# mmp/pbrt-v3

Hardware: NVIDIA H100
Metric: Msamples/sec (higher is better)
Workload: dtype f32

## Files before the change

### include/pb2.h

```cpp
#ifndef PB2_H
#define PB2_H

#include <stddef.h>
#include <stdint.h>

#ifdef __cplusplus
extern "C" {
#endif

#define PB2_ABI_VERSION 10

typedef enum pb2_status {
    PB2_OK = 0,
    PB2_ERR_NO_DEVICE = 1,
    PB2_ERR_CUDA = 2,
    PB2_ERR_INVALID = 3,
    PB2_ERR_UNSUPPORTED = 4,
    PB2_ERR_NCCL = 5
} pb2_status;


typedef struct pb2_bvh_node {
    float bmin[3];
    float bmax[3];
// ... 95 lines not shown
} pb2_bvh;

typedef struct pb2_instance {
    float instance_to_world[16];
    float world_to_instance[16];
    int32_t bvh;
    int32_t lone_prim;
    int32_t pad[2];
} pb2_instance;

typedef struct pb2_scene_desc {
    int64_t n_vertices;
    const float *P;
    const float *N;
    const float *UV;
    const float *S;
    int64_t n_tris;
    const int32_t *tri_index;
    const int32_t *tri_mesh;
    int32_t n_meshes;
    const pb2_mesh *meshes;
    int32_t n_spheres;
    const pb2_sphere *spheres;

    int64_t n_prims;
    const uint8_t *prim_type;
    const int32_t *prim_index;
    const int32_t *prim_material;
    const int32_t *prim_light;

    int64_t n_nodes;
    const pb2_bvh_node *nodes;
    const int32_t *bvh_prims;

    int32_t n_materials;
    const pb2_material *materials;
    int32_t n_lights;
    const pb2_light *lights;

    int32_t light_strategy;
    int32_t spatial_max_voxels;

    int32_t n_instances;
    int32_t n_bvhs;
    const pb2_instance *instances;
    const pb2_bvh *bvhs;
    int64_t n_bvh_prims;
    const pb2_delta_light *delta_lights;
    int32_t n_textures;
    int32_t pad_textures;
    const pb2_texture *textures;
} pb2_scene_desc;

typedef struct pb2_camera {
    float camera_to_world[16];
    float world_to_camera[16];
    float screen_window[4];
    float fov;
    float lens_radius, focal_distance;
    float shutter_open, shutter_close;
    float raster_to_camera[16];
    float dx_camera[3], dy_camera[3];
} pb2_camera;

typedef struct pb2_film_desc {
    int32_t full_resolution[2];
    int32_t cropped_pixel_bounds[4];
    float filter_radius[2];
    float max_sample_luminance;
    float scale;
    int32_t filter_type;
    float filter_param[2];
    int32_t pad;
} pb2_film_desc;

typedef struct pb2_path_params {
    int32_t samples_per_pixel;
    int32_t sample_at_pixel_center;
    int32_t max_depth;
    float rr_threshold;
    int32_t pixel_bounds[4];
    int32_t tile_rank, tile_count;
    int32_t flags;
    int32_t sampler;
} pb2_path_params;

enum { PB2_SAMPLER_HALTON = 0, PB2_SAMPLER_SOBOL = 1 };

#define PB2_FLAG_COUNT_TRAVERSAL 1
#define PB2_FLAG_LINEAR_NODES 2
#define PB2_FLAG_WIDE4 4
#define PB2_FLAG_PLAIN_TRACE 8
#define PB2_FLAG_SMALL_STACK 16
#define PB2_FLAG_LD128 32
#define PB2_FLAG_LEAF_TMA 64
#define PB2_FLAG_POOL 128
#define PB2_FLAG_CHAIN 256

typedef struct pb2_ray {
    float o[3];
    float d[3];
    float t_max;
} pb2_ray;

typedef struct pb2_hit {
    int32_t prim;
    float t;
    float b[3];
    float p[3];
    float p_error[3];
    float n[3];
    float ns[3];
    float dpdu[3];
    float uv[2];
} pb2_hit;

typedef struct pb2_stats {
    uint64_t camera_rays;
    uint64_t regular_rays;
    uint64_t shadow_rays;
    uint64_t node_visits;
    uint64_t prim_tests;
    uint64_t kernel_launches;
    double render_ms;
    double h2d_ms, d2h_ms;
    double trace_ms;
} pb2_stats;

typedef struct pb2_scene pb2_scene;


int pb2_abi_version(void);
const char *pb2_last_error(void);

int pb2_init(int device_id);
int pb2_init_devices(int n_devices, const int *device_ids);
int pb2_device_count(void);
int pb2_shutdown(void);

#define PB2_DIST_ID_BYTES 128
int pb2_dist_unique_id(void *id);
int pb2_dist_init(int rank, int world, const void *id);
int pb2_dist_info(int *rank, int *world);
int pb2_dist_shutdown(void);

int pb2_work_items(const pb2_film_desc *film, const pb2_path_params *params, int64_t first, int64_t n, int32_t *out,
                   int64_t *n_items);

int pb2_host_alloc(size_t bytes, void **out);
int pb2_host_free(void *p);

int pb2_scene_create(const pb2_scene_desc *desc, pb2_scene **out);
int pb2_scene_destroy(pb2_scene *scene);

int pb2_intersect(pb2_scene *scene, const pb2_ray *rays, int64_t n, pb2_hit *hits);
int pb2_intersect_p(pb2_scene *scene, const pb2_ray *rays, int64_t n, uint8_t *occluded);

int pb2_render_path(pb2_scene *scene, const pb2_camera *camera, const pb2_film_desc *film,
                    const pb2_path_params *params, float *film_rgbw, pb2_stats *stats);

int pb2_render_path_device(pb2_scene *scene, const pb2_camera *camera, const pb2_film_desc *film,
                           const pb2_path_params *params, float *film_rgbw_device, int clear,
                           void *stream, pb2_stats *stats);

typedef struct pb2_wf_hit {
    int32_t found;
    int32_t leaf;
    int32_t prim;
    float t;
    float b[3];
    int32_t listed;
} pb2_wf_hit;
int pb2_trace_wavefront(pb2_scene *scene, const pb2_ray *rays, const uint8_t *any_hit, int64_t n, int32_t flags,
                        pb2_wf_hit *out);

int pb2_li_samples(pb2_scene *scene, const pb2_camera *camera, const pb2_film_desc *film,
                   const pb2_path_params *params, const int32_t *pixel_xy, const int64_t *sample_num,
                   int64_t n, float *out_rgb, float *out_pfilm);

int pb2_halton_samples(const pb2_film_desc *film, const pb2_path_params *params,
                       const int32_t *pixel_xy, const int64_t *sample_num, const int32_t *dim,
                       int64_t n, float *out);

int pb2_sobol_samples_host(const pb2_film_desc *film, const pb2_path_params *params, const int32_t *pixel_xy,
                           const int64_t *sample_num, const int32_t *dim, int64_t n, float *out, uint64_t *tables);

int pb2_light_distribution(pb2_scene *scene, const float *points_xyz, int64_t n, float *out);

int pb2_texture_pyramid(const pb2_texture *texture, int32_t level, int32_t *n_levels, int32_t *w, int32_t *h, float *out);

int pb2_texture_eval_host(const pb2_texture *textures, int32_t n_textures, int32_t id, int64_t n, const float *uv, const float *duv,
                          float *out);

int pb2_bsdf_eval_host(const pb2_material *material, int64_t n, const float *in, float *out);

int pb2_camera_differentials_host(const pb2_camera *camera, const pb2_film_desc *film, const pb2_path_params *params, int64_t n,
                                  const float *in, float *out);
int pb2_uv_differentials_host(int64_t n, const float *in, float *out);

int pb2_env_distribution(const pb2_texture *texture, int32_t *nu, int32_t *nv, float *out);

int pb2_texture_lookup(const pb2_texture *texture, int64_t n, const float *st, const float *dst, float *out);

typedef struct pb2_build_node {
    float bmin[3], bmax[3];
    int32_t child[2];
    int32_t split_axis;
    int32_t first_prim_offset;
    int32_t n_primitives;
} pb2_build_node;
int pb2_hlbvh_treelets(const float *prim_bounds, int64_t n, int32_t max_prims_in_node, pb2_build_node *pool,
                       int32_t *ordered_prims, int32_t *treelet_roots, int32_t *n_treelets, double *device_ms);

int pb2_hlbvh_build(const float *prim_bounds, int64_t n, int32_t max_prims_in_node, pb2_bvh_node *nodes, int64_t *n_nodes,
                    int32_t *ordered_prims, double *device_ms);

#ifdef __cplusplus
}
#endif
#endif
```

### pbrt_v3_b200/csrc/device/pb2_path.cuh

```cuda
#ifndef PB2_PATH_CUH
#define PB2_PATH_CUH

#include "pb2_shade.cuh"

namespace pb2 {

enum { LS_IDLE = 0, LS_PATH = 1, LS_SHADOW = 2, LS_MIS = 3, LS_DEFER = 4 };

struct DLane {
    int state;
    DRay ray;
    V3 L, beta;
    DSampler smp;
    int bounces;
    bool specularBounce;
    bool camRay;
    float etaScale;
    bool doNEE, hasMis, hasNext;
    int lightNum;
    float pick;
    V3 ldSum, ldLight, misTerm;
    V3 misO, misD;
    V3 nextO, nextD;
    V3 betaNext;
};

PB2_HD void laneStartPath(DLane &ln, const DRay &ray, const DSampler &smp) {
    ln.state = LS_PATH;
    ln.ray = ray;
    ln.L = mk3(0, 0, 0);
    ln.beta = mk3(1, 1, 1);
    ln.smp = smp;
    ln.bounces = 0;
    ln.specularBounce = false;
    ln.camRay = true;
    ln.etaScale = 1;
    ln.doNEE = ln.hasMis = ln.hasNext = false;
}

PB2_HD void finishVertex(DLane &ln) {
    if (ln.doNEE) {
        V3 Ld = mk3(0, 0, 0);
        if (ln.pick != 0) Ld = mk3(ln.ldSum.x / ln.pick, ln.ldSum.y / ln.pick, ln.ldSum.z / ln.pick);
        ln.L = ln.L + ln.beta * Ld;
    }
    if (ln.hasNext) {
        ln.beta = ln.betaNext;
        ln.ray.o = ln.nextO;
        ln.ray.d = ln.nextD;
        ln.ray.tMax = PB2_INFINITY;
        ln.bounces++;
        ln.state = LS_PATH;
    } else
        ln.state = LS_IDLE;
}

PB2_HD void startMisOrFinish(DLane &ln) {
    if (ln.hasMis) {
        ln.ray.o = ln.misO;
        ln.ray.d = ln.misD;
        ln.ray.tMax = PB2_INFINITY;
        ln.state = LS_MIS;
    } else
        finishVertex(ln);
}

struct DTexCtx {
    const DCamera *cam;
    V2 pFilm;
    float diffScale;
};

template <bool SPH, bool SPEC = true, bool LAZY = true, bool TEX = false>
PB2_HD void shadeVertex(const DScene &sc, const DHalton &h, const DPathParams &pp, DLane &ln, bool found, const DHit &hit,
                        float tMax, float *u, const DTexCtx *tc = nullptr) {
    const int dim0 = ln.smp.dim;
    if (found && ln.bounces < pp.maxDepth) haltonSampleBatch<TEX>(h, ln.smp.index, dim0, kSampleBatch, u);
    DInteraction isect;
    int li = -1;
    DTexGeom tg;
    DUvDiff uvDiff;
    uvDiff.dudx = uvDiff.dvdx = uvDiff.dudy = uvDiff.dvdy = 0;
    if (found) isect = hitInteraction<SPH>(sc, hit, ln.ray, tMax, &li, (TEX && tc) ? &tg : nullptr);
    if (TEX && tc && sc.textures) {
        if (found && ln.camRay) {
            V2 uLens = mk2(0, 0);
            if (tc->cam->lensRadius > 0) {
                DSampler ls = ln.smp;
                ls.dim = 3;
                uLens = get2D<TEX>(h, ls);
            }
            const DRayDiff rd = cameraRayDifferentials(*tc->cam, tc->pFilm, uLens, tc->diffScale, ln.ray.o, ln.ray.d);
            uvDiff = computeUvDifferentials(isect.p, isect.n, tg.dpdu, tg.dpdv, rd);
        }
        if (found && ln.bounces < pp.maxDepth) {
            const int m = sc.primMaterial[isect.prim];
            const int bump = m >= 0 ? sc.materials[m].tex[PB2_TEX_BUMP] : 0;
            if (bump) bumpShading(sc, bump - 1, tg, uvDiff, &isect);
        }
    }
    const float *lazyDistrib = nullptr;
    if (LAZY && sc.lightDist.slots && found && ln.bounces < pp.maxDepth) {
        lazyDistrib = lightDistLookup(sc.lightDist, isect.p);
        if (!lazyDistrib) {
            ln.state = LS_DEFER;
            return;
        }
    }
    if (ln.bounces == 0 || ln.specularBounce) {
        if (found) {
            if (li >= 0) ln.L = ln.L + ln.beta * lightL(sc.lights[li], isect.n, -ln.ray.d);
        } else {
            for (int k = 0; k < sc.nInfinite; ++k)
                ln.L = ln.L + ln.beta * infiniteLe(sc, sc.lights[sc.infinite[k]], sc.deltaLights[sc.infinite[k]], ln.ray.d);
        }
    }
    if (!found || ln.bounces >= pp.maxDepth) {
        ln.state = LS_IDLE;
        return;
    }
    if (TEX) ln.camRay = false;
    DBsdf bsdf;
    if (!makeBsdf<SPEC, TEX>(sc, isect, &bsdf, TEX ? &uvDiff : nullptr)) {
        ln.ray = spawnRay(isect, ln.ray.d);
        return;
    }
    const float *distrib = (LAZY && lazyDistrib) ? lazyDistrib : lightDistLookup(sc.lightDist, isect.p);
    DSampler &smp = ln.smp;

    ln.doNEE = bsdf.nLobes > 0;
    ln.hasMis = false;
    ln.pick = 0;
    ln.ldSum = mk3(0, 0, 0);
    bool hasShadow = false;
    DRay shadow;
    shadow.o = shadow.d = mk3(0, 0, 0);
    shadow.tMax = 0;
    if (ln.doNEE && sc.nLights > 0) {
        float lightPickPdf;
        int lightNum = sampleDiscrete(distrib, sc.nLights, get1D<TEX>(h, smp, u, dim0), &lightPickPdf);
        if (lightPickPdf != 0) {
            ln.pick = lightPickPdf;
            ln.lightNum = lightNum;
            const pb2_light light = sc.lights[lightNum];
            const TriRec lightRec = loadTriRec(sc.lightRecs, (size_t)lightNum);
            V2 uLight = get2D<TEX>(h, smp, u, dim0);
            V2 uScattering = get2D<TEX>(h, smp, u, dim0);
            DLightSample ls = sampleLight<SPH>(sc, lightNum, light, lightRec, isect, uLight);
            float lightPdf = ls.pdf, scatteringPdf = 0;
            if (lightPdf > 0 && !isBlack(ls.Li)) {
                V3 f = bsdfF<SPEC>(bsdf, isect.wo, ls.wi) * absDot(ls.wi, isect.ns);
                scatteringPdf = bsdfPdf<SPEC>(bsdf, isect.wo, ls.wi);
                if (!isBlack(f)) {
                    shadow = spawnRayTo(isect, ls.p, ls.pError, ls.n);
                    hasShadow = true;
                    float weight = ls.delta ? 1.f : powerHeuristic(lightPdf, scatteringPdf);
                    V3 fl = f * ls.Li * weight;
                    ln.ldLight = mk3(fl.x / lightPdf, fl.y / lightPdf, fl.z / lightPdf);
                }
            }
            V3 wi;
            V3 f = mk3(0, 0, 0);
            if (!ls.delta) {
                f = bsdfSampleF<SPEC>(bsdf, isect.wo, &wi, uScattering, &scatteringPdf, nullptr, true);
                if (scatteringPdf != 0) f = f * absDot(wi, isect.ns);
                else f = mk3(0, 0, 0);
            }
            if (!isBlack(f) && scatteringPdf > 0) {
                lightPdf = lightPdfLi<SPH>(sc, light, lightRec, isect, wi, lightNum);
                if (lightPdf != 0) {
                    float weight = powerHeuristic(scatteringPdf, lightPdf);
                    V3 Lmis = mk3(light.L[0], light.L[1], light.L[2]);
                    if (sc.deltaLights && light.type == PB2_LIGHT_INFINITE) Lmis = infiniteLe(sc, light, sc.deltaLights[lightNum], wi);
                    V3 fl = f * Lmis * weight;
                    ln.misTerm = mk3(fl.x / scatteringPdf, fl.y / scatteringPdf, fl.z / scatteringPdf);
                    DRay mr = spawnRay(isect, wi);
                    ln.misO = mr.o;
                    ln.misD = mr.d;
                    ln.hasMis = true;
                }
            }
        }
    }

    ln.hasNext = false;
    {
        V3 wo = -ln.ray.d, wi;
        float pdf;
        int sampled = 0;
        V3 f = bsdfSampleF<SPEC>(bsdf, wo, &wi, get2D<TEX>(h, smp, u, dim0), &pdf, &sampled);
        if (!(isBlack(f) || pdf == 0.f)) {
            V3 s = f * absDot(wi, isect.ns);
            V3 beta = ln.beta * mk3(s.x / pdf, s.y / pdf, s.z / pdf);
            ln.specularBounce = (sampled & BSDF_SAMPLED_SPECULAR) != 0;
            if ((sampled & BSDF_SAMPLED_SPECULAR) && (sampled & BSDF_SAMPLED_TRANSMISSION)) {
                float eta = bsdf.eta;
                ln.etaScale *= (dot(wo, isect.n) > 0) ? (eta * eta) : 1 / (eta * eta);
            }
            DRay nr = spawnRay(isect, wi);
            bool survive = true;
            V3 rrBeta = beta * ln.etaScale;
            if (maxComponentValue(rrBeta) < pp.rrThreshold && ln.bounces > 3) {
                float q = pmax(.05f, 1 - maxComponentValue(rrBeta));
                if (get1D<TEX>(h, smp, u, dim0) < q) survive = false;
                else {
                    float d = 1 - q;
                    beta = mk3(beta.x / d, beta.y / d, beta.z / d);
                }
            }
            if (survive) {
                ln.hasNext = true;
                ln.nextO = nr.o;
                ln.nextD = nr.d;
                ln.betaNext = beta;
            }
        }
    }

    if (hasShadow) {
        ln.ray = shadow;
        ln.state = LS_SHADOW;
    } else
        startMisOrFinish(ln);
}

template <bool SPH>
PB2_HD void lightAdvance(const DScene &sc, DLane &ln, bool found, const DHit &hit, float tMax) {
    if (ln.state == LS_SHADOW) {
        if (!found) ln.ldSum = ln.ldSum + ln.ldLight;
        startMisOrFinish(ln);
    } else {
        if (!found) {
            if (sc.deltaLights && sc.lights[ln.lightNum].type == PB2_LIGHT_INFINITE) ln.ldSum = ln.ldSum + ln.misTerm;
        } else if (!(sc.deltaLights && sc.lights[ln.lightNum].type == PB2_LIGHT_INFINITE)) {
            float4 b = ldg4(&sc.leafPrims[3 * (size_t)hit.leaf + 1]), c = ldg4(&sc.leafPrims[3 * (size_t)hit.leaf + 2]);
            int hitLight = asInt(c.w);
            if (SPH && (floatBits(b.w) & LEAF_SPHERE)) hitLight = sc.primLight[asInt(ldg4(&sc.leafPrims[3 * (size_t)hit.leaf]).w)];
            if (hitLight == ln.lightNum) {
                const pb2_light light = sc.lights[ln.lightNum];
                if (light.two_sided) ln.ldSum = ln.ldSum + ln.misTerm;
                else {
                    DInteraction lightIsect = hitInteraction<SPH>(sc, hit, ln.ray, tMax);
                    if (dot(lightIsect.n, -ln.ray.d) > 0) ln.ldSum = ln.ldSum + ln.misTerm;
                }
            }
        }
        finishVertex(ln);
    }
}

template <bool SPH, bool SPEC = true, bool TEX = false>
PB2_HD bool laneAdvance(const DScene &sc, const DHalton &h, const DPathParams &pp, DLane &ln, bool found, const DHit &hit,
                        float tMax, const DTexCtx *tc = nullptr) {
    if (ln.state == LS_PATH) {
        float u[kSampleBatch];
        shadeVertex<SPH, SPEC, true, TEX>(sc, h, pp, ln, found, hit, tMax, u, tc);
    } else
        lightAdvance<SPH>(sc, ln, found, hit, tMax);
    return ln.state == LS_IDLE;
}

PB2_HD bool traceLane(const DScene &sc, const DLane &ln, float *tMax, DHit *hit, DCounters *ctr) {
    *tMax = ln.ray.tMax;
    hit->leaf = -1;
    hit->b0 = hit->b1 = hit->b2 = 0;
    hit->inst = -1;
    return traverseAnyOrClosest(sc, ln.ray, ln.state == LS_SHADOW, tMax, hit, ctr);
}

}
#endif
```

### pbrt_v3_b200/csrc/device/pb2_shade.cuh

```cuda
#ifndef PB2_SHADE_CUH
#define PB2_SHADE_CUH

#include "pb2_sampler.cuh"
#include "pb2_scene.cuh"

namespace pb2 {

struct DInteraction {
    V3 p, pError, n;
    V3 wo;
    V3 ns;
    V3 dpdus;
    V2 uv;
    int prim;
};

struct DTexGeom { V3 dpdu, dpdv, dpdvs, dndus, dndvs; };

struct TriVerts { V3 p0, p1, p2; };

PB2_HD V3 ld3(const float *a, int64_t i) { return mk3(a[3 * i], a[3 * i + 1], a[3 * i + 2]); }

PB2_HD TriVerts triVerts(const DScene &sc, int tri) {
    TriVerts t;
// ... 69 lines not shown
        mesh = sc.meshes[sc.triMesh[tri]];
    }
    V2 uv[3];
    triUVs(sc, tri, mesh, uv);
    V3 dpdu, dpdv;
    triPartials(tv.p0, tv.p1, tv.p2, uv, &dpdu, &dpdv);
    if (tg) {
        tg->dpdu = dpdu;
        tg->dpdv = dpdv;
        tg->dpdvs = dpdv;
        tg->dndus = tg->dndvs = mk3(0, 0, 0);
    }
    float xAbsSum = (fabsf(b0 * tv.p0.x) + fabsf(b1 * tv.p1.x) + fabsf(b2 * tv.p2.x));
    float yAbsSum = (fabsf(b0 * tv.p0.y) + fabsf(b1 * tv.p1.y) + fabsf(b2 * tv.p2.y));
    float zAbsSum = (fabsf(b0 * tv.p0.z) + fabsf(b1 * tv.p1.z) + fabsf(b2 * tv.p2.z));
    it.pError = kGamma7 * mk3(xAbsSum, yAbsSum, zAbsSum);
    it.p = b0 * tv.p0 + b1 * tv.p1 + b2 * tv.p2;
    it.uv = mk2(b0 * uv[0].x + b1 * uv[1].x + b2 * uv[2].x, b0 * uv[0].y + b1 * uv[1].y + b2 * uv[2].y);
    it.wo = normalize(-rayD);
    it.prim = prim;
    V3 dp02 = tv.p0 - tv.p2, dp12 = tv.p1 - tv.p2;
    it.n = it.ns = normalize(cross(dp02, dp12));
    if ((mesh.reverse_orientation != 0) ^ (mesh.transform_swaps_handedness != 0)) it.n = it.ns = -it.n;
    it.dpdus = dpdu;
    if (mesh.has_n || mesh.has_s) {
        int64_t v0 = sc.triIndex[3 * (int64_t)tri], v1 = sc.triIndex[3 * (int64_t)tri + 1], v2 = sc.triIndex[3 * (int64_t)tri + 2];
        V3 ns;
        if (mesh.has_n) {
            ns = (b0 * ld3(sc.N, v0) + b1 * ld3(sc.N, v1) + b2 * ld3(sc.N, v2));
            if (lengthSquared(ns) > 0) ns = normalize(ns);
            else ns = it.n;
        } else
            ns = it.n;
        V3 ss;
        if (mesh.has_s) {
            ss = (b0 * ld3(sc.S, v0) + b1 * ld3(sc.S, v1) + b2 * ld3(sc.S, v2));
            if (lengthSquared(ss) > 0) ss = normalize(ss);
            else ss = normalize(dpdu);
        } else
            ss = normalize(dpdu);
        V3 ts = cross(ss, ns);
        if (lengthSquared(ts) > 0.f) {
            ts = normalize(ts);
            ss = cross(ts, ns);
        } else
            coordinateSystem(ns, &ss, &ts);
        if (mesh.reverse_orientation) ts = -ts;
        it.ns = normalize(cross(ss, ts));
        it.n = faceforward(it.n, it.ns);
        it.dpdus = ss;
        if (tg) {
            tg->dpdvs = ts;
            if (mesh.has_n) {
                const float duv02x = uv[0].x - uv[2].x, duv02y = uv[0].y - uv[2].y;
                const float duv12x = uv[1].x - uv[2].x, duv12y = uv[1].y - uv[2].y;
                const V3 n0 = ld3(sc.N, v0), n1 = ld3(sc.N, v1), n2 = ld3(sc.N, v2);
                const V3 dn1 = n0 - n2, dn2 = n1 - n2;
                const float determinant = duv02x * duv12y - duv02y * duv12x;
                if ((double)fabsf(determinant) < 1e-8) {
                    const V3 dn = cross(n2 - n0, n1 - n0);
                    if (lengthSquared(dn) == 0) tg->dndus = tg->dndvs = mk3(0, 0, 0);
                    else coordinateSystem(dn, &tg->dndus, &tg->dndvs);
                } else {
                    const float invDet = 1 / determinant;
                    tg->dndus = (duv12y * dn1 - duv02y * dn2) * invDet;
                    tg->dndvs = (-duv12x * dn1 + duv02x * dn2) * invDet;
                }
            }
        }
    }
    return it;
}

}

#include "pb2_sphere.cuh"

namespace pb2 {

template <bool SPH = true>
PB2_HD DInteraction hitInteraction(const DScene &sc, const DHit &hit, const DRay &ray, float tHit, int *light = nullptr, DTexGeom *tg = nullptr) {
    TriRec rec = loadTriRec(sc.leafPrims, (size_t)hit.leaf);
    const DInstance *inst = nullptr;
    DRay r = ray;
    if (hit.inst >= 0 && sc.instances) {
        inst = &sc.instances[hit.inst];
        r = xfRay(inst->w2i, ray, ray.tMax);
    }
    DInteraction it;
    if (SPH && (rec.flags & LEAF_SPHERE)) {
        if (light) *light = sc.primLight[rec.prim];
        it = sphereInteraction(sc, rec.prim, r, tHit, hit.b0, tg);
    } else {
        if (light) *light = rec.light;
        it = triangleInteraction(sc, rec, hit.b0, hit.b1, hit.b2, r.d, tg);
    }
    if (inst && !inst->identity) {
        V3 pError;
        it.p = xfPointErrIn(inst->i2w, it.p, it.pError, &pError);
        it.pError = pError;
        it.n = normalize(xfNormalInv(inst->w2i, it.n));
        it.wo = normalize(xfVector(inst->i2w, it.wo));
        it.ns = normalize(xfNormalInv(inst->w2i, it.ns));
        it.dpdus = xfVector(inst->i2w, it.dpdus);
        it.ns = faceforward(it.ns, it.n);
        if (tg) {
            tg->dpdu = xfVector(inst->i2w, tg->dpdu);
            tg->dpdv = xfVector(inst->i2w, tg->dpdv);
            tg->dpdvs = xfVector(inst->i2w, tg->dpdvs);
            tg->dndus = xfNormalInv(inst->w2i, tg->dndus);
            tg->dndvs = xfNormalInv(inst->w2i, tg->dndvs);
        }
    }
    return it;
}

PB2_HD DRay spawnRay(const DInteraction &it, V3 d) {
    DRay r;
    r.o = offsetRayOrigin(it.p, it.pError, it.n, d);
    r.d = d;
    r.tMax = PB2_INFINITY;
    return r;
}
PB2_HD DRay spawnRayTo(const DInteraction &from, V3 toP, V3 toPError, V3 toN) {
    DRay r;
    r.o = offsetRayOrigin(from.p, from.pError, from.n, toP - from.p);
    V3 target = offsetRayOrigin(toP, toPError, toN, r.o - toP);
    r.d = target - r.o;
    r.tMax = 1 - kShadowEpsilon;
    return r;
}

struct DBsdf {
    V3 ns, ng, ss, ts;
    int nLobes;
    int diffuseKind;
    V3 R;
    float A, B;
    int hasMicrofacet;
    V3 Ks;
    float alpha;
    int specKind;
    V3 specR, specT;
    float eta;
    int blend;
    float alphaX, alphaY;
    int general;
    int conductor;
    V3 T0;
    V3 condEta, condK;
    float e;
};
enum { BSDF_SAMPLED_SPECULAR = 1, BSDF_SAMPLED_TRANSMISSION = 2 };
enum { GEN_OPACITY = 1, GEN_LAMBERT = 2, GEN_MICROFACET = 4, GEN_SPEC_REFLECTION = 8, GEN_SPEC_TRANSMISSION = 16,
       GEN_MICRO_TRANSMISSION = 32,
       GEN_LOBES = 6, GEN_NON_SPECULAR = GEN_LAMBERT | GEN_MICROFACET | GEN_MICRO_TRANSMISSION };

PB2_HD V3 clampSpectrum(const float c[3]) {
    return mk3(clampf(c[0], 0.f, PB2_INFINITY), clampf(c[1], 0.f, PB2_INFINITY), clampf(c[2], 0.f, PB2_INFINITY));
}

PB2_HD float roughnessToAlpha(float roughness) {
    roughness = pmax(roughness, (float)1e-3);
    float x = plogf(roughness);
    return 1.62142f + 0.819955f * x + 0.1734f * x * x + 0.0171201f * x * x * x + 0.000640711f * x * x * x * x;
}

PB2_HDN void applyTextures(const DScene &sc, V2 uv, const DUvDiff &d, pb2_material *mat) {
    for (int k = 0; k < PB2_TEX_SLOTS; ++k) {
        const int id = mat->tex[k];
        if (!id) continue;
        const V3 v = texEvaluateNode(sc.textures, sc.texels, id - 1, uv, d);
        float *dst3 = nullptr;
        switch (k) {
        case PB2_TEX_KD: dst3 = mat->kd; break;
        case PB2_TEX_KS: dst3 = mat->ks; break;
        case PB2_TEX_KR: dst3 = mat->kr; break;
        case PB2_TEX_KT: dst3 = mat->kt; break;
        case PB2_TEX_OPACITY: dst3 = mat->opacity; break;
        case PB2_TEX_METAL_ETA: dst3 = mat->metal_eta; break;
        case PB2_TEX_METAL_K: dst3 = mat->metal_k; break;
        case PB2_TEX_SIGMA: mat->sigma = v.x; break;
        case PB2_TEX_ROUGHNESS: mat->roughness = v.x; break;
        case PB2_TEX_UROUGHNESS: mat->uroughness = v.x; break;
        case PB2_TEX_VROUGHNESS: mat->vroughness = v.x; break;
        case PB2_TEX_ETA: mat->eta = v.x; break;
        }
        if (dst3) {
            dst3[0] = v.x;
            dst3[1] = v.y;
            dst3[2] = v.z;
        }
    }
}

PB2_HDN void bumpShading(const DScene &sc, int tex, const DTexGeom &tg, const DUvDiff &d, DInteraction *it) {
    float du = .5f * (fabsf(d.dudx) + fabsf(d.dudy));
    if (du == 0) du = .0005f;
    const float uDisplace = texEvaluateNode(sc.textures, sc.texels, tex, mk2(it->uv.x + du, it->uv.y + 0.f), d).x;
    float dv = .5f * (fabsf(d.dvdx) + fabsf(d.dvdy));
    if (dv == 0) dv = .0005f;
    const float vDisplace = texEvaluateNode(sc.textures, sc.texels, tex, mk2(it->uv.x + 0.f, it->uv.y + dv), d).x;
    const float displace = texEvaluateNode(sc.textures, sc.texels, tex, it->uv, d).x;
    const V3 dpdu = it->dpdus + ((uDisplace - displace) / du) * it->ns + displace * tg.dndus;
    const V3 dpdv = tg.dpdvs + ((vDisplace - displace) / dv) * it->ns + displace * tg.dndvs;
    it->ns = faceforward(normalize(cross(dpdu, dpdv)), it->n);
    it->dpdus = dpdu;
}

template <bool SPEC = true, bool TEX = false>
PB2_HD bool makeBsdf(const DScene &sc, const DInteraction &it, DBsdf *bsdf, const DUvDiff *uvDiff = nullptr) {
    int m = sc.primMaterial[it.prim];
    if (m < 0) return false;
    pb2_material mat = sc.materials[m];
    if (mat.type == PB2_MAT_NONE) return false;
    if (TEX && sc.textures && uvDiff) applyTextures(sc, it.uv, *uvDiff, &mat);
    bsdf->ns = it.ns;
    bsdf->ng = it.n;
    bsdf->ss = normalize(it.dpdus);
    bsdf->ts = cross(bsdf->ns, bsdf->ss);
    bsdf->nLobes = 0;
    bsdf->diffuseKind = 0;
    bsdf->hasMicrofacet = 0;
    bsdf->R = mk3(0, 0, 0);
    bsdf->Ks = mk3(0, 0, 0);
    bsdf->A = bsdf->B = 0;
    bsdf->alpha = 0;
    bsdf->specKind = 0;
    bsdf->specR = bsdf->specT = mk3(0, 0, 0);
    bsdf->eta = 1;
    bsdf->blend = 0;
    bsdf->alphaX = bsdf->alphaY = 0;
    bsdf->general = 0;
    bsdf->conductor = 0;
    bsdf->T0 = bsdf->condEta = bsdf->condK = mk3(0, 0, 0);
    bsdf->e = 1;
    if (SPEC && mat.type == PB2_MAT_METAL) {
        float uRough = mat.uroughness, vRough = mat.vroughness;
        if (mat.remap_roughness) {
            uRough = roughnessToAlpha(uRough);
            vRough = roughnessToAlpha(vRough);
        }
        bsdf->Ks = mk3(1, 1, 1);
        bsdf->alphaX = pmax(0.001f, uRough);
        bsdf->alphaY = pmax(0.001f, vRough);
        bsdf->conductor = 1;
        bsdf->condEta = mk3(mat.metal_eta[0], mat.metal_eta[1], mat.metal_eta[2]);
        bsdf->condK = mk3(mat.metal_k[0], mat.metal_k[1], mat.metal_k[2]);
        bsdf->general = GEN_MICROFACET;
        bsdf->nLobes = 1;
        return true;
    }
    if (SPEC && mat.type == PB2_MAT_UBER) {
        const float e = mat.eta;
        V3 op = clampSpectrum(mat.opacity);
        V3 t = mk3(clampf(-op.x + 1.f, 0.f, PB2_INFINITY), clampf(-op.y + 1.f, 0.f, PB2_INFINITY), clampf(-op.z + 1.f, 0.f, PB2_INFINITY));
        bsdf->e = e;
        if (!isBlack(t)) {
            bsdf->T0 = t;
            bsdf->general |= GEN_OPACITY;
        } else
            bsdf->eta = e;
        V3 kd = op * clampSpectrum(mat.kd);
        if (!isBlack(kd)) {
            bsdf->R = kd;
            bsdf->diffuseKind = 1;
            bsdf->general |= GEN_LAMBERT;
            bsdf->nLobes++;
        }
        V3 ks = op * clampSpectrum(mat.ks);
        if (!isBlack(ks)) {
            float roughu = mat.uroughness, roughv = mat.vroughness;
            if (mat.remap_roughness) {
                roughu = roughnessToAlpha(roughu);
                roughv = roughnessToAlpha(roughv);
            }
            bsdf->Ks = ks;
            bsdf->alphaX = pmax(0.001f, roughu);
            bsdf->alphaY = pmax(0.001f, roughv);
            bsdf->general |= GEN_MICROFACET;
            bsdf->nLobes++;
        }
        V3 kr = op * clampSpectrum(mat.kr);
        if (!isBlack(kr)) {
            bsdf->specR = kr;
            bsdf->general |= GEN_SPEC_REFLECTION;
        }
        V3 kt = op * clampSpectrum(mat.kt);
        if (!isBlack(kt)) {
            bsdf->specT = kt;
            bsdf->general |= GEN_SPEC_TRANSMISSION;
        }
        return true;
    }
    if (SPEC && mat.type == PB2_MAT_SUBSTRATE) {
        V3 d = clampSpectrum(mat.kd), sp = clampSpectrum(mat.ks);
        if (!isBlack(d) || !isBlack(sp)) {
            float roughu = mat.uroughness, roughv = mat.vroughness;
            if (mat.remap_roughness) {
                roughu = roughnessToAlpha(roughu);
                roughv = roughnessToAlpha(roughv);
            }
            bsdf->R = d;
            bsdf->Ks = sp;
            bsdf->alphaX = pmax(0.001f, roughu);
            bsdf->alphaY = pmax(0.001f, roughv);
            bsdf->blend = 1;
            bsdf->nLobes = 1;
        }
        return true;
    }
    if (SPEC && mat.type == PB2_MAT_MIRROR) {
        V3 r = clampSpectrum(mat.kr);
        if (!isBlack(r)) {
            bsdf->specKind = 1;
            bsdf->specR = r;
        }
        return true;
    }
    if (SPEC && mat.type == PB2_MAT_GLASS && !(mat.uroughness == 0 && mat.vroughness == 0)) {
        V3 r = clampSpectrum(mat.kr), t = clampSpectrum(mat.kt);
        bsdf->eta = mat.eta;
        bsdf->e = mat.eta;
        if (isBlack(r) && isBlack(t)) return true;
        float urough = mat.uroughness, vrough = mat.vroughness;
        if (mat.remap_roughness) {
            urough = roughnessToAlpha(urough);
            vrough = roughnessToAlpha(vrough);
        }
        bsdf->alphaX = pmax(0.001f, urough);
        bsdf->alphaY = pmax(0.001f, vrough);
        if (!isBlack(r)) {
            bsdf->Ks = r;
            bsdf->general |= GEN_MICROFACET;
            bsdf->nLobes++;
        }
        if (!isBlack(t)) {
            bsdf->specT = t;
            bsdf->general |= GEN_MICRO_TRANSMISSION;
            bsdf->nLobes++;
        }
        return true;
    }
    if (SPEC && mat.type == PB2_MAT_GLASS) {
        V3 r = clampSpectrum(mat.kr), t = clampSpectrum(mat.kt);
        bsdf->eta = mat.eta;
        if (!(isBlack(r) && isBlack(t))) {
            bsdf->specKind = 2;
            bsdf->specR = r;
            bsdf->specT = t;
        }
        return true;
    }
    V3 kd = clampSpectrum(mat.kd);
    if (mat.type == PB2_MAT_MATTE) {
        float sig = clampf(mat.sigma, 0.f, 90.f);
        if (!isBlack(kd)) {
            bsdf->R = kd;
            if (sig == 0)
                bsdf->diffuseKind = 1;
            else {
                bsdf->diffuseKind = 2;
                float sigma = (kPi / 180) * sig;
                float sigma2 = sigma * sigma;
                bsdf->A = 1.f - (sigma2 / (2.f * (sigma2 + 0.33f)));
                bsdf->B = 0.45f * sigma2 / (sigma2 + 0.09f);
            }
            bsdf->nLobes = 1;
        }
    } else {
        if (!isBlack(kd)) {
            bsdf->R = kd;
            bsdf->diffuseKind = 1;
            bsdf->nLobes++;
        }
        V3 ks = clampSpectrum(mat.ks);
        if (!isBlack(ks)) {
            float rough = mat.roughness;
            if (mat.remap_roughness) rough = roughnessToAlpha(rough);
            bsdf->Ks = ks;
            bsdf->alpha = pmax(0.001f, rough);
            bsdf->hasMicrofacet = 1;
            bsdf->nLobes++;
        }
    }
    return true;
}

PB2_HD V3 worldToLocal(const DBsdf &b, V3 v) { return mk3(dot(v, b.ss), dot(v, b.ts), dot(v, b.ns)); }
PB2_HD V3 localToWorld(const DBsdf &b, V3 v) {
    return mk3(b.ss.x * v.x + b.ts.x * v.y + b.ns.x * v.z, b.ss.y * v.x + b.ts.y * v.y + b.ns.y * v.z,
               b.ss.z * v.x + b.ts.z * v.y + b.ns.z * v.z);
}

PB2_HD float cosTheta(V3 w) { return w.z; }
PB2_HD float cos2Theta(V3 w) { return w.z * w.z; }
PB2_HD float absCosTheta(V3 w) { return fabsf(w.z); }
PB2_HD float sin2Theta(V3 w) { return pmax(0.f, 1.f - cos2Theta(w)); }
PB2_HD float sinTheta(V3 w) { return sqrtf(sin2Theta(w)); }
PB2_HD float tanTheta(V3 w) { return sinTheta(w) / cosTheta(w); }
PB2_HD float tan2Theta(V3 w) { return sin2Theta(w) / cos2Theta(w); }
PB2_HD float cosPhi(V3 w) { float s = sinTheta(w); return (s == 0) ? 1 : clampf(w.x / s, -1.f, 1.f); }
PB2_HD float sinPhi(V3 w) { float s = sinTheta(w); return (s == 0) ? 0 : clampf(w.y / s, -1.f, 1.f); }
PB2_HD float cos2Phi(V3 w) { return cosPhi(w) * cosPhi(w); }
PB2_HD float sin2Phi(V3 w) { return sinPhi(w) * sinPhi(w); }
PB2_HD bool sameHemisphere(V3 w, V3 wp) { return w.z * wp.z > 0; }

PB2_HD float frDielectric(float cosThetaI, float etaI, float etaT) {
    cosThetaI = clampf(cosThetaI, -1.f, 1.f);
    bool entering = cosThetaI > 0.f;
    if (!entering) {
        float t = etaI; etaI = etaT; etaT = t;
        cosThetaI = fabsf(cosThetaI);
    }
    float sinThetaI = sqrtf(pmax(0.f, 1 - cosThetaI * cosThetaI));
    float sinThetaT = etaI / etaT * sinThetaI;
    if (sinThetaT >= 1) return 1;
    float cosThetaT = sqrtf(pmax(0.f, 1 - sinThetaT * sinThetaT));
    float Rparl = ((etaT * cosThetaI) - (etaI * cosThetaT)) / ((etaT * cosThetaI) + (etaI * cosThetaT));
    float Rperp = ((etaI * cosThetaI) - (etaT * cosThetaT)) / ((etaI * cosThetaI) + (etaT * cosThetaT));
    return (Rparl * Rparl + Rperp * Rperp) / 2;
}

PB2_HD float trD(float alpha, V3 wh) {
    float t2 = tan2Theta(wh);
    if (isinf(t2)) return 0.;
    const float cos4Theta = cos2Theta(wh) * cos2Theta(wh);
    float e = (cos2Phi(wh) / (alpha * alpha) + sin2Phi(wh) / (alpha * alpha)) * t2;
    return 1 / (kPi * alpha * alpha * cos4Theta * (1 + e) * (1 + e));
}
PB2_HD float trLambda(float alpha, V3 w) {
    float absTanTheta = fabsf(tanTheta(w));
    if (isinf(absTanTheta)) return 0.;
    float a = sqrtf(cos2Phi(w) * alpha * alpha + sin2Phi(w) * alpha * alpha);
    float alpha2Tan2Theta = (a * absTanTheta) * (a * absTanTheta);
    return (-1 + sqrtf(1.f + alpha2Tan2Theta)) / 2;
}
PB2_HD float trG1(float alpha, V3 w) { return 1 / (1 + trLambda(alpha, w)); }
PB2_HD float trG(float alpha, V3 wo, V3 wi) { return 1 / (1 + trLambda(alpha, wo) + trLambda(alpha, wi)); }
PB2_HD float trPdf(float alpha, V3 wo, V3 wh) {
    return trD(alpha, wh) * trG1(alpha, wo) * absDot(wo, wh) / absCosTheta(wo);
}

PB2_HDN void trSample11(float cosThetaV, float U1, float U2, float *slope_x, float *slope_y) {
    if ((double)cosThetaV > .9999) {
        float r = (float)sqrt((double)(U1 / (1 - U1)));
        float phi = (float)(6.28318530718 * (double)U2);
        double sPhi, cPhi;
        sincos((double)phi, &sPhi, &cPhi);
        *slope_x = (float)((double)r * cPhi);
        *slope_y = (float)((double)r * sPhi);
        return;
    }
    float sinThetaV = sqrtf(pmax(0.f, 1.f - cosThetaV * cosThetaV));
    float tanThetaV = sinThetaV / cosThetaV;
    float a = 1 / tanThetaV;
    float G1 = 2 / (1 + sqrtf(1.f + 1.f / (a * a)));
    float A = 2 * U1 / G1 - 1;
    float tmp = 1.f / (A * A - 1.f);
    if (tmp > 1e10) tmp = 1e10;
    float B = tanThetaV;
    float D = sqrtf(pmax((float)(B * B * tmp * tmp - (A * A - B * B) * tmp), 0.f));
    float slope_x_1 = B * tmp - D;
    float slope_x_2 = B * tmp + D;
    *slope_x = (A < 0 || slope_x_2 > 1.f / tanThetaV) ? slope_x_1 : slope_x_2;
    float S;
    if (U2 > 0.5f) {
        S = 1.f;
        U2 = 2.f * (U2 - .5f);
    } else {
        S = -1.f;
        U2 = 2.f * (.5f - U2);
    }
    float z = (U2 * (U2 * (U2 * 0.27385f - 0.73369f) + 0.46341f)) /
              (U2 * (U2 * (U2 * 0.093073f + 0.309420f) - 1.000000f) + 0.597999f);
    *slope_y = S * z * sqrtf(1.f + *slope_x * *slope_x);
}
PB2_HD V3 trSampleWh(float alpha, V3 wo, V2 u) {
    bool flip = wo.z < 0;
    V3 wi = flip ? -wo : wo;
    V3 wiStretched = normalize(mk3(alpha * wi.x, alpha * wi.y, wi.z));
    float slope_x, slope_y;
    trSample11(cosTheta(wiStretched), u.x, u.y, &slope_x, &slope_y);
    float tmp = cosPhi(wiStretched) * slope_x - sinPhi(wiStretched) * slope_y;
    slope_y = sinPhi(wiStretched) * slope_x + cosPhi(wiStretched) * slope_y;
    slope_x = tmp;
    slope_x = alpha * slope_x;
    slope_y = alpha * slope_y;
    V3 wh = normalize(mk3(-slope_x, -slope_y, 1.f));
    if (flip) wh = -wh;
    return wh;
}

PB2_HD float trD2(float ax, float ay, V3 wh) {
    float t2 = tan2Theta(wh);
    if (isinf(t2)) return 0.;
    const float cos4Theta = cos2Theta(wh) * cos2Theta(wh);
    float e = (cos2Phi(wh) / (ax * ax) + sin2Phi(wh) / (ay * ay)) * t2;
    return 1 / (kPi * ax * ay * cos4Theta * (1 + e) * (1 + e));
}
PB2_HD float trLambda2(float ax, float ay, V3 w) {
    float absTanTheta = fabsf(tanTheta(w));
    if (isinf(absTanTheta)) return 0.;
    float a = sqrtf(cos2Phi(w) * ax * ax + sin2Phi(w) * ay * ay);
    float alpha2Tan2Theta = (a * absTanTheta) * (a * absTanTheta);
    return (-1 + sqrtf(1.f + alpha2Tan2Theta)) / 2;
}
PB2_HD float trPdf2(float ax, float ay, V3 wo, V3 wh) {
    return trD2(ax, ay, wh) * (1 / (1 + trLambda2(ax, ay, wo))) * absDot(wo, wh) / absCosTheta(wo);
}
PB2_HD V3 trSampleWh2(float ax, float ay, V3 wo, V2 u) {
    bool flip = wo.z < 0;
    V3 wi = flip ? -wo : wo;
    V3 wiStretched = normalize(mk3(ax * wi.x, ay * wi.y, wi.z));
    float slope_x, slope_y;
    trSample11(cosTheta(wiStretched), u.x, u.y, &slope_x, &slope_y);
    float tmp = cosPhi(wiStretched) * slope_x - sinPhi(wiStretched) * slope_y;
    slope_y = sinPhi(wiStretched) * slope_x + cosPhi(wiStretched) * slope_y;
    slope_x = tmp;
    slope_x = ax * slope_x;
    slope_y = ay * slope_y;
    V3 wh = normalize(mk3(-slope_x, -slope_y, 1.f));
    if (flip) wh = -wh;
    return wh;
}
PB2_HD float pow5f(float v) { return (v * v) * (v * v) * v; }
PB2_HD V3 blendF(const DBsdf &b, V3 wo, V3 wi) {
    V3 one = mk3(1, 1, 1);
    V3 diffuse = (28.f / (23.f * kPi)) * b.R * (one - b.Ks) * (1 - pow5f(1 - .5f * absCosTheta(wi))) * (1 - pow5f(1 - .5f * absCosTheta(wo)));
    V3 wh = wi + wo;
    if (wh.x == 0 && wh.y == 0 && wh.z == 0) return mk3(0, 0, 0);
    wh = normalize(wh);
    float cosT = dot(wi, wh);
    V3 schlick = b.Ks + pow5f(1 - cosT) * (one - b.Ks);
    V3 specular = (trD2(b.alphaX, b.alphaY, wh) / (4 * absDot(wi, wh) * pmax(absCosTheta(wi), absCosTheta(wo)))) * schlick;
    return diffuse + specular;
}
PB2_HD float blendPdf(const DBsdf &b, V3 wo, V3 wi) {
    if (!sameHemisphere(wo, wi)) return 0;
    V3 wh = normalize(wo + wi);
    float pdf_wh = trPdf2(b.alphaX, b.alphaY, wo, wh);
    return .5f * (absCosTheta(wi) * kInvPi + pdf_wh / (4 * dot(wo, wh)));
}

PB2_HD V3 diffuseF(const DBsdf &b, V3 wo, V3 wi) {
    if (b.diffuseKind == 1) return b.R * kInvPi;
    float sinThetaI = sinTheta(wi), sinThetaO = sinTheta(wo);
    float maxCos = 0;
    if ((double)sinThetaI > 1e-4 && (double)sinThetaO > 1e-4) {
        float sinPhiI = sinPhi(wi), cosPhiI = cosPhi(wi);
        float sinPhiO = sinPhi(wo), cosPhiO = cosPhi(wo);
        float dCos = cosPhiI * cosPhiO + sinPhiI * sinPhiO;
        maxCos = pmax(0.f, dCos);
    }
    float sinAlpha, tanBeta;
    if (absCosTheta(wi) > absCosTheta(wo)) {
        sinAlpha = sinThetaO;
        tanBeta = sinThetaI / absCosTheta(wi);
    } else {
        sinAlpha = sinThetaI;
        tanBeta = sinThetaO / absCosTheta(wo);
    }
    return b.R * kInvPi * (b.A + b.B * maxCos * sinAlpha * tanBeta);
}
PB2_HD float diffusePdf(V3 wo, V3 wi) { return sameHemisphere(wo, wi) ? absCosTheta(wi) * kInvPi : 0; }

PB2_HD V3 microfacetF(const DBsdf &b, V3 wo, V3 wi) {
    float cosThetaO = absCosTheta(wo), cosThetaI = absCosTheta(wi);
    V3 wh = wi + wo;
    if (cosThetaI == 0 || cosThetaO == 0) return mk3(0, 0, 0);
    if (wh.x == 0 && wh.y == 0 && wh.z == 0) return mk3(0, 0, 0);
    wh = normalize(wh);
    float F = frDielectric(dot(wi, faceforward(wh, mk3(0, 0, 1))), 1.5f, 1.f);
    V3 num = b.Ks * trD(b.alpha, wh) * trG(b.alpha, wo, wi) * mk3(F, F, F);
    float den = (4 * cosThetaI * cosThetaO);
    return mk3(num.x / den, num.y / den, num.z / den);
}
PB2_HD float microfacetPdf(const DBsdf &b, V3 wo, V3 wi) {
    if (!sameHemisphere(wo, wi)) return 0;
    V3 wh = normalize(wo + wi);
    return trPdf(b.alpha, wo, wh) / (4 * dot(wo, wh));
}

PB2_HD float frConductor1(float cosThetaI, float cosThetaI2, float sinThetaI2, float etat, float k) {
    float eta = etat / 1.f, etak = k / 1.f;
    float eta2 = eta * eta, etak2 = etak * etak;
    float t0 = eta2 - etak2 - sinThetaI2;
    float a2plusb2 = sqrtf(t0 * t0 + 4 * eta2 * etak2);
    float t1 = a2plusb2 + cosThetaI2;
    float a = sqrtf(0.5f * (a2plusb2 + t0));
    float t2 = (2 * cosThetaI) * a;
    float Rs = (t1 - t2) / (t1 + t2);
    float t3 = cosThetaI2 * a2plusb2 + sinThetaI2 * sinThetaI2;
    float t4 = t2 * sinThetaI2;
    float Rp = Rs * (t3 - t4) / (t3 + t4);
    return 0.5f * (Rp + Rs);
}
PB2_HD V3 frConductor(float cosThetaI, V3 etat, V3 k) {
    cosThetaI = clampf(cosThetaI, -1.f, 1.f);
    float cosThetaI2 = cosThetaI * cosThetaI;
    float sinThetaI2 = (float)(1. - (double)cosThetaI2);
    return mk3(frConductor1(cosThetaI, cosThetaI2, sinThetaI2, etat.x, k.x), frConductor1(cosThetaI, cosThetaI2, sinThetaI2, etat.y, k.y),
               frConductor1(cosThetaI, cosThetaI2, sinThetaI2, etat.z, k.z));
}
PB2_HD V3 microfacetFGen(const DBsdf &b, V3 wo, V3 wi) {
    float cosThetaO = absCosTheta(wo), cosThetaI = absCosTheta(wi);
    V3 wh = wi + wo;
    if (cosThetaI == 0 || cosThetaO == 0) return mk3(0, 0, 0);
    if (wh.x == 0 && wh.y == 0 && wh.z == 0) return mk3(0, 0, 0);
    wh = normalize(wh);
    float c = dot(wi, faceforward(wh, mk3(0, 0, 1)));
    V3 F;
    if (b.conductor) F = frConductor(fabsf(c), b.condEta, b.condK);
    else {
        float Fd = frDielectric(c, 1.f, b.e);
        F = mk3(Fd, Fd, Fd);
    }
    float G = 1 / (1 + trLambda2(b.alphaX, b.alphaY, wo) + trLambda2(b.alphaX, b.alphaY, wi));
    V3 num = b.Ks * trD2(b.alphaX, b.alphaY, wh) * G * F;
    float den = (4 * cosThetaI * cosThetaO);
    return mk3(num.x / den, num.y / den, num.z / den);
}
PB2_HD float microfacetPdfGen(const DBsdf &b, V3 wo, V3 wi) {
    if (!sameHemisphere(wo, wi)) return 0;
    V3 wh = normalize(wo + wi);
    return trPdf2(b.alphaX, b.alphaY, wo, wh) / (4 * dot(wo, wh));
}
PB2_HD V3 microTransF(const DBsdf &b, V3 wo, V3 wi) {
    if (sameHemisphere(wo, wi)) return mk3(0, 0, 0);
    float cosThetaO = cosTheta(wo), cosThetaI = cosTheta(wi);
    if (cosThetaI == 0 || cosThetaO == 0) return mk3(0, 0, 0);
    float eta = cosTheta(wo) > 0 ? (b.e / 1.f) : (1.f / b.e);
    V3 wh = normalize(wo + wi * eta);
    if (wh.z < 0) wh = -wh;
    if (dot(wo, wh) * dot(wi, wh) > 0) return mk3(0, 0, 0);
    float F = frDielectric(dot(wo, wh), 1.f, b.e);
    float sqrtDenom = dot(wo, wh) + eta * dot(wi, wh);
    float factor = 1 / eta;
    float G = 1 / (1 + trLambda2(b.alphaX, b.alphaY, wo) + trLambda2(b.alphaX, b.alphaY, wi));
    float v = fabsf(trD2(b.alphaX, b.alphaY, wh) * G * eta * eta * absDot(wi, wh) * absDot(wo, wh) * factor * factor /
                    (cosThetaI * cosThetaO * sqrtDenom * sqrtDenom));
    return mk3(1.f - F, 1.f - F, 1.f - F) * b.specT * v;
}
PB2_HD float microTransPdf(const DBsdf &b, V3 wo, V3 wi) {
    if (sameHemisphere(wo, wi)) return 0;
    float eta = cosTheta(wo) > 0 ? (b.e / 1.f) : (1.f / b.e);
    V3 wh = normalize(wo + wi * eta);
    if (dot(wo, wh) * dot(wi, wh) > 0) return 0;
    float sqrtDenom = dot(wo, wh) + eta * dot(wi, wh);
    float dwh_dwi = fabsf((eta * eta * dot(wi, wh)) / (sqrtDenom * sqrtDenom));
    return trPdf2(b.alphaX, b.alphaY, wo, wh) * dwh_dwi;
}
PB2_HD V3 genF(const DBsdf &b, V3 wo, V3 wi, bool reflect) {
    V3 f = mk3(0, 0, 0);
    if (reflect) {
        if (b.general & GEN_LAMBERT) f = f + b.R * kInvPi;
        if (b.general & GEN_MICROFACET) f = f + microfacetFGen(b, wo, wi);
    } else if (b.general & GEN_MICRO_TRANSMISSION)
        f = f + microTransF(b, wo, wi);
    return f;
}

template <bool SPEC = true>
PB2_HD V3 bsdfF(const DBsdf &b, V3 woW, V3 wiW) {
    V3 wi = worldToLocal(b, wiW), wo = worldToLocal(b, woW);
    if (wo.z == 0) return mk3(0, 0, 0);
    bool reflect = dot(wiW, b.ng) * dot(woW, b.ng) > 0;
    V3 f = mk3(0, 0, 0);
    if (SPEC && b.blend) return reflect ? blendF(b, wo, wi) : f;
    if (SPEC && b.general) return genF(b, wo, wi, reflect);
    if (reflect) {
        if (b.diffuseKind) f = f + diffuseF(b, wo, wi);
        if (b.hasMicrofacet) f = f + microfacetF(b, wo, wi);
    }
    return f;
}
template <bool SPEC = true>
PB2_HD float bsdfPdf(const DBsdf &b, V3 woW, V3 wiW) {
    if (b.nLobes == 0) return 0.f;
    V3 wo = worldToLocal(b, woW), wi = worldToLocal(b, wiW);
    if (wo.z == 0) return 0.;
    if (SPEC && b.blend) return blendPdf(b, wo, wi);
    if (SPEC && b.general) {
        float pdf = 0.f;
        if (b.general & GEN_LAMBERT) pdf += diffusePdf(wo, wi);
        if (b.general & GEN_MICROFACET) pdf += microfacetPdfGen(b, wo, wi);
        if (b.general & GEN_MICRO_TRANSMISSION) pdf += microTransPdf(b, wo, wi);
        return pdf / b.nLobes;
    }
    float pdf = 0.f;
    if (b.diffuseKind) pdf += diffusePdf(wo, wi);
    if (b.hasMicrofacet) pdf += microfacetPdf(b, wo, wi);
    return pdf / b.nLobes;
}
PB2_HD bool refract(V3 wi, V3 n, float eta, V3 *wt) {
    float cosThetaI = dot(n, wi);
    float sin2ThetaI = pmax(0.f, 1 - cosThetaI * cosThetaI);
    float sin2ThetaT = eta * eta * sin2ThetaI;
    if (sin2ThetaT >= 1) return false;
    float cosThetaT = sqrtf(1 - sin2ThetaT);
    *wt = eta * (-wi) + (eta * cosThetaI - cosThetaT) * n;
    return true;
}

PB2_HDN V3 genSampleF(const DBsdf &b, V3 woW, V3 *wiW, V2 u, float *pdf, int *sampledFlags, bool nonSpecularOnly) {
    const int mask = nonSpecularOnly ? (b.general & GEN_NON_SPECULAR) : b.general;
    int matching = 0;
    for (int i = 0; i < GEN_LOBES; ++i) matching += (mask >> i) & 1;
    if (matching == 0) return mk3(0, 0, 0);
    int comp = (int)floorf(u.x * matching);
    if (comp > matching - 1) comp = matching - 1;
    int lobe = 0, count = comp;
    for (int i = 0; i < GEN_LOBES; ++i)
        if ((mask >> i) & 1) {
            if (count-- == 0) {
                lobe = 1 << i;
                break;
            }
        }
    V2 uRemapped = mk2(pmin(u.x * matching - comp, kOneMinusEpsilon), u.y);
    V3 wo = worldToLocal(b, woW), wi = mk3(0, 0, 0);
    if (wo.z == 0) return mk3(0, 0, 0);
    V3 f = mk3(0, 0, 0);
    int flags = 0;
    if (lobe == GEN_LAMBERT) {
        wi = cosineSampleHemisphere(uRemapped);
        if (wo.z < 0) wi.z *= -1;
        *pdf = diffusePdf(wo, wi);
    } else if (lobe == GEN_MICROFACET) {
        V3 wh = trSampleWh2(b.alphaX, b.alphaY, wo, uRemapped);
        if (dot(wo, wh) < 0) return mk3(0, 0, 0);
        wi = -wo + 2 * dot(wo, wh) * wh;
        if (!sameHemisphere(wo, wi)) return mk3(0, 0, 0);
        *pdf = trPdf2(b.alphaX, b.alphaY, wo, wh) / (4 * dot(wo, wh));
    } else if (lobe == GEN_MICRO_TRANSMISSION) {
        V3 wh = trSampleWh2(b.alphaX, b.alphaY, wo, uRemapped);
        if (dot(wo, wh) < 0) return mk3(0, 0, 0);
        float eta = cosTheta(wo) > 0 ? (1.f / b.e) : (b.e / 1.f);
        if (!refract(wo, wh, eta, &wi)) return mk3(0, 0, 0);
        *pdf = microTransPdf(b, wo, wi);
        flags = BSDF_SAMPLED_TRANSMISSION;
    } else if (lobe == GEN_SPEC_REFLECTION) {
        wi = mk3(-wo.x, -wo.y, wo.z);
        *pdf = 1;
        float F = frDielectric(cosTheta(wi), 1.f, b.e);
        V3 fr = mk3(F, F, F) * b.specR;
        f = mk3(fr.x / absCosTheta(wi), fr.y / absCosTheta(wi), fr.z / absCosTheta(wi));
        flags = BSDF_SAMPLED_SPECULAR;
    } else {
        const float etaA = 1.f, etaB = (lobe == GEN_OPACITY) ? 1.f : b.e;
        const V3 T = (lobe == GEN_OPACITY) ? b.T0 : b.specT;
        bool entering = cosTheta(wo) > 0;
        float etaI = entering ? etaA : etaB;
        float etaT = entering ? etaB : etaA;
        V3 nn = mk3(0, 0, 1);
        if (dot(nn, wo) < 0) nn = -nn;
        if (!refract(wo, nn, etaI / etaT, &wi)) return mk3(0, 0, 0);
        *pdf = 1;
        float F = frDielectric(cosTheta(wi), etaA, etaB);
        V3 ft = T * mk3(1.f - F, 1.f - F, 1.f - F);
        ft = ft * ((etaI * etaI) / (etaT * etaT));
        f = mk3(ft.x / absCosTheta(wi), ft.y / absCosTheta(wi), ft.z / absCosTheta(wi));
        flags = BSDF_SAMPLED_SPECULAR | BSDF_SAMPLED_TRANSMISSION;
    }
    if (*pdf == 0) return mk3(0, 0, 0);
    *wiW = localToWorld(b, wi);
    const bool specular = (lobe & GEN_NON_SPECULAR) == 0;
    if (!specular && matching > 1) {
        if (lobe != GEN_LAMBERT && (mask & GEN_LAMBERT)) *pdf += diffusePdf(wo, wi);
        if (lobe != GEN_MICROFACET && (mask & GEN_MICROFACET)) *pdf += microfacetPdfGen(b, wo, wi);
        if (lobe != GEN_MICRO_TRANSMISSION && (mask & GEN_MICRO_TRANSMISSION)) *pdf += microTransPdf(b, wo, wi);
    }
    if (matching > 1) *pdf /= matching;
    if (!specular) {
        bool reflect = dot(*wiW, b.ng) * dot(woW, b.ng) > 0;
        f = genF(b, wo, wi, reflect);
    }
    if (sampledFlags) *sampledFlags = flags;
    return f;
}

template <bool SPEC = true>
PB2_HD V3 bsdfSampleF(const DBsdf &b, V3 woW, V3 *wiW, V2 u, float *pdf, int *sampledFlags = nullptr, bool nonSpecularOnly = false) {
    *pdf = 0;
    if (sampledFlags) *sampledFlags = 0;
    if (SPEC && b.general) return genSampleF(b, woW, wiW, u, pdf, sampledFlags, nonSpecularOnly);
    if (SPEC && b.specKind) {
        V3 wo = worldToLocal(b, woW), wi;
        if (wo.z == 0) return mk3(0, 0, 0);
        V3 f;
        int flags = BSDF_SAMPLED_SPECULAR;
        if (b.specKind == 1) {
            wi = mk3(-wo.x, -wo.y, wo.z);
            *pdf = 1;
            f = mk3(b.specR.x / absCosTheta(wi), b.specR.y / absCosTheta(wi), b.specR.z / absCosTheta(wi));
        } else {
            float u0 = pmin(u.x, kOneMinusEpsilon);
            float F = frDielectric(cosTheta(wo), 1.f, b.eta);
            if (u0 < F) {
                wi = mk3(-wo.x, -wo.y, wo.z);
                *pdf = F;
                V3 fr = F * b.specR;
                f = mk3(fr.x / absCosTheta(wi), fr.y / absCosTheta(wi), fr.z / absCosTheta(wi));
            } else {
                bool entering = cosTheta(wo) > 0;
                float etaI = entering ? 1.f : b.eta;
                float etaT = entering ? b.eta : 1.f;
                V3 nn = mk3(0, 0, 1);
                if (dot(nn, wo) < 0) nn = -nn;
                if (!refract(wo, nn, etaI / etaT, &wi)) return mk3(0, 0, 0);
                V3 ft = b.specT * (1 - F);
                ft = ft * ((etaI * etaI) / (etaT * etaT));
                flags |= BSDF_SAMPLED_TRANSMISSION;
                *pdf = 1 - F;
                f = mk3(ft.x / absCosTheta(wi), ft.y / absCosTheta(wi), ft.z / absCosTheta(wi));
            }
        }
        if (*pdf == 0) return mk3(0, 0, 0);
        *wiW = localToWorld(b, wi);
        if (sampledFlags) *sampledFlags = flags;
        return f;
    }
    int matching = b.nLobes;
    if (matching == 0) return mk3(0, 0, 0);
    if (SPEC && b.blend) {
        V3 wo = worldToLocal(b, woW), wi;
        if (wo.z == 0) return mk3(0, 0, 0);
        V2 uu = mk2(pmin(u.x, kOneMinusEpsilon), u.y);
        if ((double)uu.x < .5) {
            uu.x = pmin(2 * uu.x, kOneMinusEpsilon);
            wi = cosineSampleHemisphere(uu);
            if (wo.z < 0) wi.z *= -1;
        } else {
            uu.x = pmin(2 * (uu.x - .5f), kOneMinusEpsilon);
            V3 wh = trSampleWh2(b.alphaX, b.alphaY, wo, uu);
            wi = -wo + 2 * dot(wo, wh) * wh;
            if (!sameHemisphere(wo, wi)) return mk3(0, 0, 0);
        }
        *pdf = blendPdf(b, wo, wi);
        if (*pdf == 0) return mk3(0, 0, 0);
        *wiW = localToWorld(b, wi);
        bool reflect = dot(*wiW, b.ng) * dot(woW, b.ng) > 0;
        return reflect ? blendF(b, wo, wi) : mk3(0, 0, 0);
    }
    int comp = (int)floorf(u.x * matching);
    if (comp > matching - 1) comp = matching - 1;
    bool sampleMicro = b.hasMicrofacet && (comp == matching - 1) && !(b.diffuseKind && comp == 0);
    V2 uRemapped = mk2(pmin(u.x * matching - comp, kOneMinusEpsilon), u.y);
    V3 wo = worldToLocal(b, woW), wi;
    if (wo.z == 0) return mk3(0, 0, 0);
    V3 f;
    if (!sampleMicro) {
        wi = cosineSampleHemisphere(uRemapped);
        if (wo.z < 0) wi.z *= -1;
        *pdf = diffusePdf(wo, wi);
        f = diffuseF(b, wo, wi);
    } else {
        V3 wh = trSampleWh(b.alpha, wo, uRemapped);
        if (dot(wo, wh) < 0) return mk3(0, 0, 0);
        wi = -wo + 2 * dot(wo, wh) * wh;
        if (!sameHemisphere(wo, wi)) return mk3(0, 0, 0);
        *pdf = trPdf(b.alpha, wo, wh) / (4 * dot(wo, wh));
        f = microfacetF(b, wo, wi);
    }
    if (*pdf == 0) return mk3(0, 0, 0);
    *wiW = localToWorld(b, wi);
    if (matching > 1) {
        if (sampleMicro) *pdf += diffusePdf(wo, wi);
        else *pdf += microfacetPdf(b, wo, wi);
        *pdf /= matching;
    }
    bool reflect = dot(*wiW, b.ng) * dot(woW, b.ng) > 0;
    f = mk3(0, 0, 0);
    if (reflect) {
        if (b.diffuseKind) f = f + diffuseF(b, wo, wi);
        if (b.hasMicrofacet) f = f + microfacetF(b, wo, wi);
    }
    return f;
}

struct DLightSample {
    V3 p, pError, n;
    V3 wi;
    V3 Li;
    float pdf;
    bool delta;
};

PB2_HD float triangleArea(const TriVerts &t) { return (float)(0.5 * (double)length(cross(t.p1 - t.p0, t.p2 - t.p0))); }

PB2_HD V3 lightL(const pb2_light &l, V3 n, V3 w) {
    return (l.two_sided || dot(n, w) > 0) ? mk3(l.L[0], l.L[1], l.L[2]) : mk3(0, 0, 0);
}

PB2_HD void sphereSampleArea(const pb2_sphere &s, V2 u, V3 *p, V3 *pError, V3 *n, float *pdf) {
    M44 o2w = loadM44(s.object_to_world), w2o = loadM44(s.world_to_object);
    V3 pObj = mk3(0, 0, 0) + s.radius * uniformSampleSphere(u);
    *n = normalize(xfNormalInv(w2o, pObj));
    if (s.reverse_orientation) *n = *n * -1.f;
    pObj = pObj * (s.radius / length(pObj));
    V3 pObjError = kGamma5 * vabs(pObj);
    *p = xfPointErrIn(o2w, pObj, pObjError, pError);
    *pdf = 1 / (s.phi_max * s.radius * (s.z_max - s.z_min));
}

PB2_HDN DLightSample sampleSphereLight(const DScene &sc, const pb2_light &l, const DInteraction &ref, V2 u) {
    DLightSample ls;
    const pb2_sphere s = sc.spheres[sc.primIndex[l.prim]];
    M44 o2w = loadM44(s.object_to_world);
    V3 pCenter = xfPoint(o2w, mk3(0, 0, 0));
    V3 pOrigin = offsetRayOrigin(ref.p, ref.pError, ref.n, pCenter - ref.p);
    if (lengthSquared(pOrigin - pCenter) <= s.radius * s.radius) {
        sphereSampleArea(s, u, &ls.p, &ls.pError, &ls.n, &ls.pdf);
        V3 wi = ls.p - ref.p;
        if (lengthSquared(wi) == 0)
            ls.pdf = 0;
        else {
            wi = normalize(wi);
            ls.pdf *= lengthSquared(ref.p - ls.p) / absDot(ls.n, -wi);
        }
        if (isinf(ls.pdf)) ls.pdf = 0.f;
    } else {
        float dc = length(ref.p - pCenter);
        float invDc = 1 / dc;
        V3 wc = (pCenter - ref.p) * invDc;
        V3 wcX, wcY;
        coordinateSystem(wc, &wcX, &wcY);
        float sinThetaMax = s.radius * invDc;
        float sinThetaMax2 = sinThetaMax * sinThetaMax;
        float invSinThetaMax = 1 / sinThetaMax;
        float cosThetaMax = sqrtf(pmax(0.f, 1 - sinThetaMax2));
        float cosThetaV = (cosThetaMax - 1) * u.x + 1;
        float sinTheta2 = 1 - cosThetaV * cosThetaV;
        if (sinThetaMax2 < 0.00068523f) {
            sinTheta2 = sinThetaMax2 * u.x;
            cosThetaV = sqrtf(1 - sinTheta2);
        }
        float cosAlpha = sinTheta2 * invSinThetaMax +
                         cosThetaV * sqrtf(pmax(0.f, 1.f - sinTheta2 * invSinThetaMax * invSinThetaMax));
        float sinAlpha = sqrtf(pmax(0.f, 1.f - cosAlpha * cosAlpha));
        float phi = u.y * 2 * kPi;
        float sinPhiS, cosPhiS;
        psincosf(phi, &sinPhiS, &cosPhiS);
        V3 nWorld = sinAlpha * cosPhiS * (-wcX) + sinAlpha * sinPhiS * (-wcY) + cosAlpha * (-wc);
        V3 pWorld = pCenter + s.radius * nWorld;
        ls.p = pWorld;
        ls.pError = kGamma5 * vabs(pWorld);
        ls.n = nWorld;
        if (s.reverse_orientation) ls.n = ls.n * -1.f;
        ls.pdf = 1 / (2 * kPi * (1 - cosThetaMax));
    }
    if (ls.pdf == 0 || lengthSquared(ls.p - ref.p) == 0) {
        ls.pdf = 0;
        ls.Li = mk3(0, 0, 0);
        ls.wi = mk3(0, 0, 0);
        return ls;
    }
    ls.wi = normalize(ls.p - ref.p);
    ls.Li = lightL(l, ls.n, -ls.wi);
    return ls;
}

PB2_HDN float sphereLightPdf(const DScene &sc, const pb2_light &l, const DInteraction &ref, V3 wi) {
    const pb2_sphere s = sc.spheres[sc.primIndex[l.prim]];
    M44 o2w = loadM44(s.object_to_world);
    V3 pCenter = xfPoint(o2w, mk3(0, 0, 0));
    V3 pOrigin = offsetRayOrigin(ref.p, ref.pError, ref.n, pCenter - ref.p);
    if (lengthSquared(pOrigin - pCenter) <= s.radius * s.radius) {
        DRay ray;
        ray.o = offsetRayOrigin(ref.p, ref.pError, ref.n, wi);
        ray.d = wi;
        ray.tMax = PB2_INFINITY;
        SphereRayHit h;
        if (!sphereTest(s, ray, ray.tMax, &h)) return 0;
        DInteraction li = sphereInteraction(sc, l.prim, ray, h.tHit, h.phi);
        float pdf = lengthSquared(ref.p - li.p) / (absDot(li.n, -wi) * (s.phi_max * s.radius * (s.z_max - s.z_min)));
        if (isinf(pdf)) pdf = 0.f;
        return pdf;
    }
    float sinThetaMax2 = s.radius * s.radius / lengthSquared(ref.p - pCenter);
    float cosThetaMax = sqrtf(pmax(0.f, 1 - sinThetaMax2));
    return 1 / (2 * kPi * (1 - cosThetaMax));
}

PB2_HD DLightSample sampleTriangleLight(const DScene &sc, const pb2_light &l, const TriRec &rec, V3 refP, V2 u) {
    DLightSample s;
    const TriVerts t = rec.tv;
    V2 b = uniformSampleTriangle(u);
    float b2 = (1 - b.x - b.y);
    s.p = b.x * t.p0 + b.y * t.p1 + b2 * t.p2;
    s.n = normalize(cross(t.p1 - t.p0, t.p2 - t.p0));
    bool hasN = false;
    if (rec.flags & LEAF_ATTR) {
        int tri = sc.primIndex[rec.prim];
        if (sc.meshes[sc.triMesh[tri]].has_n) {
            hasN = true;
            int64_t v0 = sc.triIndex[3 * (int64_t)tri], v1 = sc.triIndex[3 * (int64_t)tri + 1], v2 = sc.triIndex[3 * (int64_t)tri + 2];
            V3 ns = b.x * ld3(sc.N, v0) + b.y * ld3(sc.N, v1) + b2 * ld3(sc.N, v2);
            s.n = faceforward(s.n, ns);
        }
    }
    if (!hasN && (rec.flags & LEAF_FLIP)) s.n = s.n * -1.f;
    V3 pAbsSum = vabs(b.x * t.p0) + vabs(b.y * t.p1) + vabs(b2 * t.p2);
    s.pError = kGamma6 * pAbsSum;
    s.pdf = 1 / triangleArea(t);
    V3 wi = s.p - refP;
    if (lengthSquared(wi) == 0)
        s.pdf = 0;
    else {
        wi = normalize(wi);
        s.pdf *= lengthSquared(refP - s.p) / absDot(s.n, -wi);
        if (isinf(s.pdf)) s.pdf = 0.f;
    }
    if (s.pdf == 0 || lengthSquared(s.p - refP) == 0) {
        s.pdf = 0;
        s.Li = mk3(0, 0, 0);
        s.wi = mk3(0, 0, 0);
        return s;
    }
    s.wi = normalize(s.p - refP);
    s.Li = lightL(l, s.n, -s.wi);
    return s;
}

PB2_HDN DLightSample sampleDeltaLight(const pb2_light &l, const DDeltaLight &dl, V3 refP) {
    DLightSample s;
    s.delta = true;
    s.pError = s.n = mk3(0, 0, 0);
    s.pdf = 1.f;
    const V3 I = mk3(l.L[0], l.L[1], l.L[2]);
    if (l.type == PB2_LIGHT_DISTANT) {
        V3 wLight = mk3(dl.p[0], dl.p[1], dl.p[2]);
        s.wi = wLight;
        s.p = refP + wLight * (2 * dl.worldRadius);
        s.Li = I;
        return s;
    }
    V3 pLight = mk3(dl.p[0], dl.p[1], dl.p[2]);
    s.p = pLight;
    s.wi = normalize(pLight - refP);
    float d2 = lengthSquared(pLight - refP);
    if (l.type == PB2_LIGHT_POINT) {
        s.Li = mk3(I.x / d2, I.y / d2, I.z / d2);
        return s;
    }
    V3 w = -s.wi;
    const float *m = dl.worldToLight;
    V3 wl = normalize(mk3(m[0] * w.x + m[1] * w.y + m[2] * w.z, m[3] * w.x + m[4] * w.y + m[5] * w.z, m[6] * w.x + m[7] * w.y + m[8] * w.z));
    float cosT = wl.z, falloff;
    if (cosT < dl.cosTotalWidth) falloff = 0;
    else if (cosT >= dl.cosFalloffStart) falloff = 1;
    else {
        float delta = (cosT - dl.cosTotalWidth) / (dl.cosFalloffStart - dl.cosTotalWidth);
        falloff = (delta * delta) * (delta * delta);
    }
    V3 If = I * falloff;
    s.Li = mk3(If.x / d2, If.y / d2, If.z / d2);
    return s;
}

PB2_HD V3 infiniteLookup(const pb2_light &l, V2 st) {
    const V3 T = mk3(l.L[0], l.L[1], l.L[2]);
    const float s = st.x * 1 - 0.5f, t = st.y * 1 - 0.5f;
    const float s0 = floorf(s), t0 = floorf(t);
    const float ds = s - (float)(int)s0, dt = t - (float)(int)t0;
    return ((1 - ds) * (1 - dt)) * T + ((1 - ds) * dt) * T + (ds * (1 - dt)) * T + (ds * dt) * T;
}
PB2_HD float sampleContinuous1D(const float *rec, int n, float u, float *pdf, int *off) {
    const float *func = rec, *cdf = rec + n;
    const float funcInt = rec[2 * n + 1];
    int first = 0, len = n + 1;
    while (len > 0) {
        int half = len >> 1, middle = first + half;
        if (cdf[middle] <= u) {
            first = middle + 1;
            len -= half + 1;
        } else
            len = half;
    }
    int offset = first - 1;
    offset = offset < 0 ? 0 : (offset > n - 1 ? n - 1 : offset);
    *off = offset;
    float du = u - cdf[offset];
    if ((cdf[offset + 1] - cdf[offset]) > 0) du /= (cdf[offset + 1] - cdf[offset]);
    *pdf = (funcInt > 0) ? func[offset] / funcInt : 0;
    return (offset + du) / n;
}
PB2_HD V3 envLookup(const DScene &sc, const pb2_light &l, const DDeltaLight &dl, V2 st) {
    if (dl.envTex) return texTriangle(sc.textures[dl.envTex - 1], sc.texels, 0, st);
    return infiniteLookup(l, st);
}
PB2_HDN V3 infiniteLe(const DScene &sc, const pb2_light &l, const DDeltaLight &dl, V3 d) {
    const float *m = dl.worldToLight;
    const V3 w = normalize(mk3(m[0] * d.x + m[1] * d.y + m[2] * d.z, m[3] * d.x + m[4] * d.y + m[5] * d.z, m[6] * d.x + m[7] * d.y + m[8] * d.z));
    float phi = patan2f(w.y, w.x);
    if (phi < 0) phi = phi + 2 * kPi;
    const float theta = pacosf(clampf(w.z, -1.f, 1.f));
    return envLookup(sc, l, dl, mk2(phi * (0.5f * kInvPi), theta * kInvPi));
}
PB2_HDN DLightSample sampleInfiniteLight(const DScene &sc, const pb2_light &l, const DDeltaLight &dl, V3 refP, V2 u) {
    DLightSample s;
    s.delta = false;
    s.pError = s.n = mk3(0, 0, 0);
    s.p = refP;
    s.wi = mk3(0, 0, 1);
    s.pdf = 0;
    s.Li = mk3(0, 0, 0);
    float pdf1, pdf0;
    int v, uo;
    float d0, d1;
    if (dl.envTex) {
        const int nu = dl.envNu, nv = dl.envNv;
        d1 = sampleContinuous1D(dl.envDist + (size_t)nv * (2 * nu + 2), nv, u.y, &pdf1, &v);
        d0 = sampleContinuous1D(dl.envDist + (size_t)v * (2 * nu + 2), nu, u.x, &pdf0, &uo);
    } else {
        d1 = sampleContinuous1D(dl.dist + 12, 2, u.y, &pdf1, &v);
        d0 = sampleContinuous1D(dl.dist + 6 * v, 2, u.x, &pdf0, &uo);
    }
    const float mapPdf = pdf0 * pdf1;
    if (mapPdf == 0) return s;
    const float theta = d1 * kPi, phi = d0 * 2 * kPi;
    const float cosTheta = pcosf(theta), sinTheta = psinf(theta);
    const float sinPhi = psinf(phi), cosPhi = pcosf(phi);
    const V3 vl = mk3(sinTheta * cosPhi, sinTheta * sinPhi, cosTheta);
    const float *m = dl.lightToWorld;
    s.wi = mk3(m[0] * vl.x + m[1] * vl.y + m[2] * vl.z, m[3] * vl.x + m[4] * vl.y + m[5] * vl.z, m[6] * vl.x + m[7] * vl.y + m[8] * vl.z);
    s.pdf = mapPdf / (2 * kPi * kPi * sinTheta);
    if (sinTheta == 0) s.pdf = 0;
    s.p = refP + s.wi * (2 * dl.worldRadius);
    s.Li = envLookup(sc, l, dl, mk2(d0, d1));
    return s;
}
PB2_HDN float infinitePdfLi(const DDeltaLight &dl, V3 w) {
    const float *m = dl.worldToLight;
    const V3 wi = mk3(m[0] * w.x + m[1] * w.y + m[2] * w.z, m[3] * w.x + m[4] * w.y + m[5] * w.z, m[6] * w.x + m[7] * w.y + m[8] * w.z);
    const float theta = pacosf(clampf(wi.z, -1.f, 1.f));
    float phi = patan2f(wi.y, wi.x);
    if (phi < 0) phi = phi + 2 * kPi;
    const float sinTheta = psinf(theta);
    if (sinTheta == 0) return 0;
    const float px = phi * (0.5f * kInvPi), py = theta * kInvPi;
    if (dl.envTex) {
        const int nu = dl.envNu, nv = dl.envNv;
        int iu = (int)(px * nu), iv = (int)(py * nv);
        iu = iu < 0 ? 0 : (iu > nu - 1 ? nu - 1 : iu);
        iv = iv < 0 ? 0 : (iv > nv - 1 ? nv - 1 : iv);
        const float marginalInt = dl.envDist[(size_t)nv * (2 * nu + 2) + 2 * nv + 1];
        return (dl.envDist[(size_t)iv * (2 * nu + 2) + iu] / marginalInt) / (2 * kPi * kPi * sinTheta);
    }
    int iu = (int)(px * 2), iv = (int)(py * 2);
    iu = iu < 0 ? 0 : (iu > 1 ? 1 : iu);
    iv = iv < 0 ? 0 : (iv > 1 ? 1 : iv);
    return (dl.dist[6 * iv + iu] / dl.dist[12 + 5]) / (2 * kPi * kPi * sinTheta);
}

template <bool SPH = true>
PB2_HD DLightSample sampleLight(const DScene &sc, int lightNum, const pb2_light &l, const TriRec &rec, const DInteraction &ref, V2 u) {
    if (sc.deltaLights && l.type == PB2_LIGHT_INFINITE) return sampleInfiniteLight(sc, l, sc.deltaLights[lightNum], ref.p, u);
    if (sc.deltaLights && l.type != PB2_LIGHT_AREA) return sampleDeltaLight(l, sc.deltaLights[lightNum], ref.p);
    DLightSample s;
    if (SPH && (rec.flags & LEAF_SPHERE)) s = sampleSphereLight(sc, l, ref, u);
    else s = sampleTriangleLight(sc, l, rec, ref.p, u);
    s.delta = false;
    return s;
}

template <bool SPH = true>
PB2_HD float lightPdfLi(const DScene &sc, const pb2_light &l, const TriRec &rec, const DInteraction &ref, V3 wi, int lightNum = -1) {
    if (sc.deltaLights && l.type == PB2_LIGHT_INFINITE) return infinitePdfLi(sc.deltaLights[lightNum], wi);
    if (SPH && (rec.flags & LEAF_SPHERE)) return sphereLightPdf(sc, l, ref, wi);
    DRay ray = spawnRay(ref, wi);
    const TriVerts t = rec.tv;
    DRaySetup rs = setupRay(ray.o, ray.d);
    float tHit, b0, b1, b2;
    if (!triangleTest(t.p0, t.p1, t.p2, rs, ray.tMax, &tHit, &b0, &b1, &b2)) return 0;
    if (rec.flags & LEAF_DEGENERATE) return 0;
    DInteraction li = triangleInteraction(sc, rec, b0, b1, b2, ray.d);
    float pdf = lengthSquared(ref.p - li.p) / (absDot(li.n, -wi) * triangleArea(t));
    if (isinf(pdf)) pdf = 0.f;
    return pdf;
}

PB2_HD const float *lightDistLookup(const DLightDist &ld, V3 p) {
    if (ld.strategy != PB2_LIGHTDIST_SPATIAL) return ld.table;
    V3 o = p - ld.boundsMin;
    if (ld.boundsMax.x > ld.boundsMin.x) o.x /= ld.boundsMax.x - ld.boundsMin.x;
    if (ld.boundsMax.y > ld.boundsMin.y) o.y /= ld.boundsMax.y - ld.boundsMin.y;
    if (ld.boundsMax.z > ld.boundsMin.z) o.z /= ld.boundsMax.z - ld.boundsMin.z;
    int pi[3];
    float of[3] = {o.x, o.y, o.z};
    for (int i = 0; i < 3; ++i) {
        float v = of[i] * ld.nVoxels[i];
        int iv = (v != v) ? 0 : (v >= 2147483648.f ? ld.nVoxels[i] - 1 : (v <= -2147483648.f ? 0 : (int)v));
        pi[i] = iv < 0 ? 0 : (iv > ld.nVoxels[i] - 1 ? ld.nVoxels[i] - 1 : iv);
    }
    int64_t voxel = ((int64_t)pi[0] * ld.nVoxels[1] + pi[1]) * ld.nVoxels[2] + pi[2];
    if (!ld.slots) return ld.table + voxel * ld.stride;
#if defined(__CUDA_ARCH__)
    int s = ld.slots[voxel];
    if (s >= 0) return ld.table + (size_t)s * ld.stride;
    if (s == LD_ABSENT && atomicCAS(&ld.slots[voxel], (int)LD_ABSENT, (int)LD_REQUESTED) == LD_ABSENT)
        ld.requests[atomicAdd(&ld.counters[0], 1)] = (int)voxel;
#endif
    return nullptr;
}

struct DVoxelBounds { V3 vMin, vMax; };
PB2_HD DVoxelBounds voxelBounds(const DLightDist &ld, int px, int py, int pz) {
    V3 p0 = mk3((float)px / (float)ld.nVoxels[0], (float)py / (float)ld.nVoxels[1], (float)pz / (float)ld.nVoxels[2]);
    V3 p1 = mk3((float)(px + 1) / (float)ld.nVoxels[0], (float)(py + 1) / (float)ld.nVoxels[1], (float)(pz + 1) / (float)ld.nVoxels[2]);
    V3 a = mk3(lerpf(p0.x, ld.boundsMin.x, ld.boundsMax.x), lerpf(p0.y, ld.boundsMin.y, ld.boundsMax.y), lerpf(p0.z, ld.boundsMin.z, ld.boundsMax.z));
    V3 b = mk3(lerpf(p1.x, ld.boundsMin.x, ld.boundsMax.x), lerpf(p1.y, ld.boundsMin.y, ld.boundsMax.y), lerpf(p1.z, ld.boundsMin.z, ld.boundsMax.z));
    DVoxelBounds vb;
    vb.vMin = mk3(pmin(a.x, b.x), pmin(a.y, b.y), pmin(a.z, b.z));
    vb.vMax = mk3(pmax(a.x, b.x), pmax(a.y, b.y), pmax(a.z, b.z));
    return vb;
}
constexpr int kVoxelSamples = 128;
PB2_HD float voxelLightContribution(const DScene &sc, const DHalton &h, const DVoxelBounds &vb, int j) {
    const pb2_light light = sc.lights[j];
    const TriRec rec = loadTriRec(sc.lightRecs, (size_t)j);
    float contrib = 0;
    for (int i = 0; i < kVoxelSamples; ++i) {
        V3 t = mk3(radicalInverse(h, 0, i), radicalInverse(h, 1, i), radicalInverse(h, 2, i));
        DInteraction intr;
        intr.p = mk3(lerpf(t.x, vb.vMin.x, vb.vMax.x), lerpf(t.y, vb.vMin.y, vb.vMax.y), lerpf(t.z, vb.vMin.z, vb.vMax.z));
        intr.pError = mk3(0, 0, 0);
        intr.n = mk3(0, 0, 0);
        intr.wo = mk3(1, 0, 0);
        intr.ns = mk3(0, 0, 0);
        intr.dpdus = mk3(0, 0, 0);
        intr.uv = mk2(0, 0);
        intr.prim = -1;
        V2 u = mk2(radicalInverse(h, 3, i), radicalInverse(h, 4, i));
        DLightSample ls = sampleLight(sc, j, light, rec, intr, u);
        if (ls.pdf > 0) contrib += luminance(ls.Li) / ls.pdf;
    }
    return contrib;
}
PB2_HD void finishVoxelDistribution(int n, float *rec) {
    float sumContrib = 0;
    for (int j = 0; j < n; ++j) sumContrib += rec[j];
    float avgContrib = sumContrib / (kVoxelSamples * n);
    float minContrib = (avgContrib > 0) ? (float)(.001 * (double)avgContrib) : 1;
    for (int j = 0; j < n; ++j) rec[j] = pmax(rec[j], minContrib);
    float *cdf = rec + n;
    cdf[0] = 0;
    for (int i = 1; i < n + 1; ++i) cdf[i] = cdf[i - 1] + rec[i - 1] / n;
    float funcInt = cdf[n];
    if (funcInt == 0) {
        for (int i = 1; i < n + 1; ++i) cdf[i] = (float)i / (float)n;
    } else {
        for (int i = 1; i < n + 1; ++i) cdf[i] /= funcInt;
    }
    rec[2 * n + 1] = funcInt;
}
PB2_HD void computeVoxelDistribution(const DScene &sc, const DHalton &h, const DLightDist &ld, int px, int py, int pz,
                                     float *rec) {
    const DVoxelBounds vb = voxelBounds(ld, px, py, pz);
    for (int j = 0; j < sc.nLights; ++j) rec[j] = voxelLightContribution(sc, h, vb, j);
    finishVoxelDistribution(sc.nLights, rec);
}

struct DCamera {
    M44 rasterToCamera, cameraToWorld;
    float lensRadius, focalDistance;
    V3 dxCamera, dyCamera;
};

struct DRayDiff { V3 rxo, rxd, ryo, ryd; };

PB2_HD DRayDiff cameraRayDifferentials(const DCamera &cam, V2 pFilm, V2 uLens, float scale, V3 o, V3 d) {
    V3 pCamera = xfPoint(cam.rasterToCamera, mk3(pFilm.x, pFilm.y, 0));
    V3 rxo = mk3(0, 0, 0), ryo = mk3(0, 0, 0), rxd, ryd;
    if (cam.lensRadius > 0) {
        V2 dsk = concentricSampleDisk(uLens);
        V2 pLens = mk2(cam.lensRadius * dsk.x, cam.lensRadius * dsk.y);
        V3 dx = normalize(pCamera + cam.dxCamera);
        float ft = cam.focalDistance / dx.z;
        V3 pFocus = mk3(0, 0, 0) + (ft * dx);
        rxo = mk3(pLens.x, pLens.y, 0);
        rxd = normalize(pFocus - rxo);
        V3 dy = normalize(pCamera + cam.dyCamera);
        ft = cam.focalDistance / dy.z;
        pFocus = mk3(0, 0, 0) + (ft * dy);
        ryo = mk3(pLens.x, pLens.y, 0);
        ryd = normalize(pFocus - ryo);
    } else {
        rxd = normalize(pCamera + cam.dxCamera);
        ryd = normalize(pCamera + cam.dyCamera);
    }
    DRayDiff r;
    r.rxo = xfPoint(cam.cameraToWorld, rxo);
    r.ryo = xfPoint(cam.cameraToWorld, ryo);
    r.rxd = xfVector(cam.cameraToWorld, rxd);
    r.ryd = xfVector(cam.cameraToWorld, ryd);
    r.rxo = o + (r.rxo - o) * scale;
    r.ryo = o + (r.ryo - o) * scale;
    r.rxd = d + (r.rxd - d) * scale;
    r.ryd = d + (r.ryd - d) * scale;
    return r;
}

PB2_HD DUvDiff computeUvDifferentials(V3 p, V3 n, V3 dpdu, V3 dpdv, const DRayDiff &rd) {
    DUvDiff z;
    z.dudx = z.dvdx = z.dudy = z.dvdy = 0;
    float dd = dot(n, p);
    float tx = -(dot(n, rd.rxo) - dd) / dot(n, rd.rxd);
    if (isinf(tx) || tx != tx) return z;
    V3 px = rd.rxo + tx * rd.rxd;
    float ty = -(dot(n, rd.ryo) - dd) / dot(n, rd.ryd);
    if (isinf(ty) || ty != ty) return z;
    V3 py = rd.ryo + ty * rd.ryd;
    int d0, d1;
    if (fabsf(n.x) > fabsf(n.y) && fabsf(n.x) > fabsf(n.z)) {
        d0 = 1;
        d1 = 2;
    } else if (fabsf(n.y) > fabsf(n.z)) {
        d0 = 0;
        d1 = 2;
    } else {
        d0 = 0;
// ... 78 lines not shown
```

### pbrt_v3_b200/csrc/pb2_cuda.cu

```cuda
#include <cuda_runtime.h>
#include <cub/device/device_radix_sort.cuh>
#include <dlfcn.h>
#include <nccl.h>

#include <algorithm>
#include <mutex>
#include <chrono>
#include <cstddef>
#include <cstdio>
#include <cstdlib>
#include <cstring>
#include <string>
#include <thread>
#include <vector>

#include "device/pb2_path.cuh"
#include "device/pb2_wide4.cuh"
#include "host/core.h"
#include "pb2.h"

using namespace pb2;

static thread_local std::string g_lastError;
static int setError(int code, const std::string &msg) {
// ... 172 lines not shown
    extendedGCD(b, a % b, &xp, &yp);
    *x = yp;
    *y = xp - (d * yp);
}
static uint64_t multiplicativeInverse(int64_t a, int64_t n) {
    int64_t x, y;
    extendedGCD(a, n, &x, &y);
    int64_t r = x - (x / n) * n;
    return (uint64_t)(r < 0 ? r + n : r);
}

struct SampleBounds { int x0, y0, x1, y1; };
static SampleBounds filmSampleBounds(const pb2_film_desc *f) {
    SampleBounds b;
    b.x0 = (int)std::floor((float)f->cropped_pixel_bounds[0] + 0.5f - f->filter_radius[0]);
    b.y0 = (int)std::floor((float)f->cropped_pixel_bounds[1] + 0.5f - f->filter_radius[1]);
    b.x1 = (int)std::ceil((float)f->cropped_pixel_bounds[2] - 0.5f + f->filter_radius[0]);
    b.y1 = (int)std::ceil((float)f->cropped_pixel_bounds[3] - 0.5f + f->filter_radius[1]);
    return b;
}

static DHalton makeHalton(const pb2_film_desc *film, const pb2_path_params *pp) {
    DHalton h;
    SampleBounds sb = filmSampleBounds(film);
    int res[2] = {sb.x1 - sb.x0, sb.y1 - sb.y0};
    for (int i = 0; i < 2; ++i) {
        int base = (i == 0) ? 2 : 3;
        int scale = 1, exp = 0;
        while (scale < std::min(res[i], kMaxResolution)) {
            scale *= base;
            ++exp;
        }
        h.baseScales[i] = scale;
        h.baseExponents[i] = exp;
    }
    h.sampleStride = h.baseScales[0] * h.baseScales[1];
    h.multInverse[0] = (int)multiplicativeInverse(h.baseScales[1], h.baseScales[0]);
    h.multInverse[1] = (int)multiplicativeInverse(h.baseScales[0], h.baseScales[1]);
    h.sampleAtPixelCenter = pp->sample_at_pixel_center;
    h.samplesPerPixel = pp->samples_per_pixel;
    h.perms = cur().perms;
    h.primes = cur().primes;
    h.primeSums = cur().primeSums;
    h.dimRecs = cur().dimRecs;
    h.dimTabs = envInt("PB2_HALTON_LOOP", 0) ? nullptr : cur().dimTabs;
    h.digitTab = cur().digitTab;
    h.sobol = nullptr;
    h.sobolVdc = nullptr;
    h.sobolLog2Res = h.sobolRes = 0;
    h.sbx0 = sb.x0;
    h.sby0 = sb.y0;
    return h;
}

static std::vector<uint32_t> g_sobolMatrices;
static std::mutex g_sobolMutex;
static int loadSobolMatrices() {
    std::lock_guard<std::mutex> lock(g_sobolMutex);
    if (!g_sobolMatrices.empty()) return PB2_OK;
    Dl_info info;
    std::string dir = ".";
    if (dladdr((void *)&loadSobolMatrices, &info) && info.dli_fname) {
        dir = info.dli_fname;
        size_t slash = dir.find_last_of('/');
        dir = slash == std::string::npos ? "." : dir.substr(0, slash);
    }
    const std::string path = dir + "/sobol_matrices32.bin";
    FILE *f = fopen(path.c_str(), "rb");
    std::vector<uint32_t> m((size_t)kSobolDims * kSobolMatrixSize);
    if (!f || fread(m.data(), sizeof(uint32_t), m.size(), f) != m.size()) {
        if (f) fclose(f);
        return setError(PB2_ERR_UNSUPPORTED, "SobolSampler: cannot read " + path + " (run tools/make_sobol_tables.py or __graft_entry__.build())");
    }
    fclose(f);
    for (int k = 0; k < 32; ++k)
        if (m[k] != (0x80000000u >> k) || !(m[kSobolMatrixSize + k] & 0x80000000u))
            return setError(PB2_ERR_INVALID, "SobolSampler: " + path + " does not hold Sobol' generator matrices");
    g_sobolMatrices.swap(m);
    return PB2_OK;
}
static uint64_t sobolPixelColumn(int k, int m) {
    const uint64_t c0 = g_sobolMatrices[k], c1 = g_sobolMatrices[kSobolMatrixSize + k];
    return ((c0 >> (32 - m)) << m) | (c1 >> (32 - m));
}
static void sobolIntervalTables(int m, uint64_t out[2 * kSobolMatrixSize]) {
    memset(out, 0, 2 * kSobolMatrixSize * sizeof(uint64_t));
    if (m <= 0) return;
    const int n = 2 * m;
    for (int c = 0; c + n < kSobolMatrixSize; ++c) out[c] = sobolPixelColumn(n + c, m);
    std::vector<uint64_t> a((size_t)n, 0), id((size_t)n);
    for (int r = 0; r < n; ++r) {
        for (int k = 0; k < n; ++k)
            if ((sobolPixelColumn(k, m) >> r) & 1) a[r] |= 1ull << k;
        id[r] = 1ull << r;
    }
    for (int k = 0, rr = 0; k < n; ++k, ++rr) {
        int p = rr;
        while (p < n && !((a[p] >> k) & 1)) ++p;
        if (p == n) return;
        std::swap(a[rr], a[p]);
        std::swap(id[rr], id[p]);
        for (int r = 0; r < n; ++r)
            if (r != rr && ((a[r] >> k) & 1)) {
                a[r] ^= a[rr];
                id[r] ^= id[rr];
            }
    }
    for (int c = 0; c < n; ++c) {
        uint64_t v = 0;
        for (int k = 0; k < n; ++k)
            if ((id[k] >> c) & 1) v |= 1ull << k;
        out[kSobolMatrixSize + c] = v;
    }
}
static int attachSobol(DHalton *h, const pb2_film_desc *film) {
    int rc = loadSobolMatrices();
    if (rc) return rc;
    DeviceState &dev = cur();
    if (!dev.sobol) {
        CUDA_TRY(cudaMalloc((void **)&dev.sobol, g_sobolMatrices.size() * sizeof(uint32_t)));
        CUDA_TRY(cudaMemcpy(dev.sobol, g_sobolMatrices.data(), g_sobolMatrices.size() * sizeof(uint32_t), cudaMemcpyHostToDevice));
    }
    if (!dev.sobolVdc) CUDA_TRY(cudaMalloc((void **)&dev.sobolVdc, 2 * kSobolMatrixSize * sizeof(uint64_t)));
    SampleBounds sb = filmSampleBounds(film);
    int extent = std::max(sb.x1 - sb.x0, sb.y1 - sb.y0), res = 1, log2Res = 0;
    while (res < extent) {
        res <<= 1;
        ++log2Res;
    }
    if (log2Res > 26) return setError(PB2_ERR_UNSUPPORTED, "SobolSampler: sample bounds beyond 2^26 pixels in one direction");
    uint64_t tables[2 * kSobolMatrixSize];
    sobolIntervalTables(log2Res, tables);
    CUDA_TRY(cudaMemcpy(dev.sobolVdc, tables, sizeof(tables), cudaMemcpyHostToDevice));
    h->sobol = dev.sobol;
    h->sobolVdc = dev.sobolVdc;
    h->sobolLog2Res = log2Res;
    h->sobolRes = res;
    h->sampleAtPixelCenter = 0;
    return PB2_OK;
}

struct pb2_scene {
    DScene d;
    std::vector<void *> allocations;
    float *film = nullptr;
    float *filterTable = nullptr;
    size_t filmFloats = 0;
    unsigned long long *counters = nullptr;
    int64_t nPrims = 0;
    int nLights = 0;
    int bvhDepth = 0;
    int instDepth = 0;
    bool hasSpecular = false;
    int devIndex = 0;
    std::vector<pb2_scene *> replicas;
    bool lazyLightDist = false;
    int *ldHostCounters = nullptr;
    void *wfCtx = nullptr;
    int *wfQueues = nullptr;
    unsigned *wfCounts = nullptr;
    unsigned *wfHostCounts = nullptr;
    int wfCapacity = 0;
    std::vector<cudaEvent_t> traceEvents;
    int2 *wfSpill = nullptr;
    void *paramBuf = nullptr;
    cudaStream_t pipeStreams[4] = {nullptr, nullptr, nullptr, nullptr};
    cudaEvent_t forkEvent = nullptr, joinEvents[4] = {nullptr, nullptr, nullptr, nullptr};
};

template <typename T>
static int upload(pb2_scene *s, const T *host, size_t count, const T **dev) {
    *dev = nullptr;
    if (count == 0 || host == nullptr) return PB2_OK;
    void *p = nullptr;
    CUDA_TRY(cudaMalloc(&p, count * sizeof(T)));
    s->allocations.push_back(p);
    CUDA_TRY(cudaMemcpy(p, host, count * sizeof(T), cudaMemcpyHostToDevice));
    *dev = (const T *)p;
    return PB2_OK;
}
template <typename T>
static int allocate(pb2_scene *s, size_t count, T **dev) {
    void *p = nullptr;
    CUDA_TRY(cudaMalloc(&p, std::max<size_t>(count, 1) * sizeof(T)));
    s->allocations.push_back(p);
    *dev = (T *)p;
    return PB2_OK;
}

__global__ void k_build_leaf_records(DScene sc, const int32_t *prims, int64_t n, float4 *out) {
    int64_t j = blockIdx.x * (int64_t)blockDim.x + threadIdx.x;
    if (j >= n) return;
    int prim = prims[j];
    float4 a, b, c;
    if (sc.primType[prim] == PB2_PRIM_SPHERE) {
        a = make_float4(0, 0, 0, __int_as_float(prim));
        b = make_float4(0, 0, 0, __uint_as_float(LEAF_SPHERE));
        c = make_float4(0, 0, 0, __int_as_float(sc.primIndex[prim]));
    } else if (sc.primType[prim] == PB2_PRIM_INSTANCE) {
        a = make_float4(0, 0, 0, __int_as_float(prim));
        b = make_float4(0, 0, 0, __uint_as_float(LEAF_INSTANCE));
        c = make_float4(0, 0, 0, __int_as_float(sc.primIndex[prim]));
    } else {
        int tri = sc.primIndex[prim];
        TriVerts t = triVerts(sc, tri);
        uint32_t flags = 0;
        V2 uv[3];
        const pb2_mesh mesh = sc.meshes[sc.triMesh[tri]];
        triUVs(sc, tri, mesh, uv);
        V3 dpdu, dpdv;
        if (!triPartials(t.p0, t.p1, t.p2, uv, &dpdu, &dpdv)) flags |= LEAF_DEGENERATE;
        if ((mesh.reverse_orientation != 0) ^ (mesh.transform_swaps_handedness != 0)) flags |= LEAF_FLIP;
        if (mesh.has_n || mesh.has_s || mesh.has_uv) flags |= LEAF_ATTR;
        if (mesh.alpha_tex || mesh.shadow_alpha_tex) flags |= LEAF_ALPHA;
        a = make_float4(t.p0.x, t.p0.y, t.p0.z, __int_as_float(prim));
        b = make_float4(t.p1.x, t.p1.y, t.p1.z, __uint_as_float(flags));
        c = make_float4(t.p2.x, t.p2.y, t.p2.z, __int_as_float(sc.primLight[prim]));
    }
    out[3 * j] = a;
    out[3 * j + 1] = b;
    out[3 * j + 2] = c;
}

__global__ void k_spatial_light_dist(DScene sc, DHalton h, float *table) {
    int64_t v = blockIdx.x * (int64_t)blockDim.x + threadIdx.x;
    const DLightDist &ld = sc.lightDist;
    int64_t total = (int64_t)ld.nVoxels[0] * ld.nVoxels[1] * ld.nVoxels[2];
    if (v >= total) return;
    int pz = (int)(v % ld.nVoxels[2]);
    int py = (int)((v / ld.nVoxels[2]) % ld.nVoxels[1]);
    int px = (int)(v / ((int64_t)ld.nVoxels[2] * ld.nVoxels[1]));
    computeVoxelDistribution(sc, h, ld, px, py, pz, table + v * ld.stride);
}

__global__ void k_intersect(DScene sc, const pb2_ray *rays, int64_t n, pb2_hit *hits) {
    int64_t i = blockIdx.x * (int64_t)blockDim.x + threadIdx.x;
    if (i >= n) return;
    DRay r;
    r.o = mk3(rays[i].o[0], rays[i].o[1], rays[i].o[2]);
    r.d = mk3(rays[i].d[0], rays[i].d[1], rays[i].d[2]);
    r.tMax = rays[i].t_max;
    DHit h;
    h.leaf = -1;
    h.b0 = h.b1 = h.b2 = 0;
    h.inst = -1;
    float tMax = r.tMax;
    bool found = traverse<false>(sc, r, &tMax, &h, nullptr);
    pb2_hit out;
    memset(&out, 0, sizeof(out));
    out.prim = -1;
    out.t = tMax;
    if (found) {
        DInteraction it = hitInteraction<true>(sc, h, r, tMax);
        out.prim = it.prim;
        out.b[0] = h.b0; out.b[1] = h.b1; out.b[2] = h.b2;
        out.p[0] = it.p.x; out.p[1] = it.p.y; out.p[2] = it.p.z;
        out.p_error[0] = it.pError.x; out.p_error[1] = it.pError.y; out.p_error[2] = it.pError.z;
        out.n[0] = it.n.x; out.n[1] = it.n.y; out.n[2] = it.n.z;
        out.ns[0] = it.ns.x; out.ns[1] = it.ns.y; out.ns[2] = it.ns.z;
        out.dpdu[0] = it.dpdus.x; out.dpdu[1] = it.dpdus.y; out.dpdu[2] = it.dpdus.z;
        out.uv[0] = it.uv.x; out.uv[1] = it.uv.y;
    }
    hits[i] = out;
}

__global__ void k_intersect_p(DScene sc, const pb2_ray *rays, int64_t n, uint8_t *occluded) {
    int64_t i = blockIdx.x * (int64_t)blockDim.x + threadIdx.x;
    if (i >= n) return;
    DRay r;
    r.o = mk3(rays[i].o[0], rays[i].o[1], rays[i].o[2]);
    r.d = mk3(rays[i].d[0], rays[i].d[1], rays[i].d[2]);
    r.tMax = rays[i].t_max;
    DHit h;
    h.leaf = -1;
    h.inst = -1;
    float tMax = r.tMax;
    occluded[i] = traverse<true>(sc, r, &tMax, &h, nullptr) ? 1 : 0;
}

struct DRenderParams {
    DCamera cam;
    DHalton halton;
    DPathParams path;
    int sbx0, sby0, sbx1, sby1;
    int pbx0, pby0, pbx1, pby1;
    int cx0, cy0, cx1, cy1;
    float filterRadiusX, filterRadiusY;
    float invFilterRadiusX, invFilterRadiusY;
    const float *filterTable;
    float maxSampleLuminance;
    int nTilesX, nTilesY;
    int tileRank, tileCount;
    long long nOwnedTiles;
    long long nWorkItems;
    int spp;
    float diffScale;
};

enum { CTR_WORK = 0, CTR_CAMERA = 1, CTR_REGULAR = 2, CTR_SHADOW = 3, CTR_NODES = 4, CTR_PRIMS = 5, CTR_COUNT = 8 };

PB2_HD int compact1by1(unsigned x) {
    x &= 0x55555555u;
    x = (x ^ (x >> 1)) & 0x33333333u;
    x = (x ^ (x >> 2)) & 0x0f0f0f0fu;
    x = (x ^ (x >> 4)) & 0x00ff00ffu;
    return (int)x;
// ... 272 lines not shown
    rp.maxSampleLuminance = film->max_sample_luminance;
    rp.nTilesX = (sb.x1 - sb.x0 + 15) / 16;
    rp.nTilesY = (sb.y1 - sb.y0 + 15) / 16;
    rp.tileCount = std::max(1, pp->tile_count);
    rp.tileRank = pp->tile_rank;
    long long nTiles = (long long)std::max(0, rp.nTilesX) * std::max(0, rp.nTilesY);
    rp.nOwnedTiles = nTiles > rp.tileRank ? (nTiles - rp.tileRank + rp.tileCount - 1) / rp.tileCount : 0;
    rp.spp = pp->samples_per_pixel;
    rp.nWorkItems = rp.nOwnedTiles * 256LL * rp.spp;
    return rp;
}

static int validateRenderArgs(const pb2_scene *scene, const pb2_camera *cam, const pb2_film_desc *film, const pb2_path_params *pp) {
    if (!scene || !cam || !film || !pp) return setError(PB2_ERR_INVALID, "null argument");
    if (pp->samples_per_pixel <= 0 || pp->max_depth < 0) return setError(PB2_ERR_INVALID, "bad samples_per_pixel / max_depth");
    if (5 + 8 * ((long long)pp->max_depth + 1) > kMaxHaltonDims)
        return setError(PB2_ERR_UNSUPPORTED, "maxdepth above 123: HaltonSampler can only sample 1000 dimensions");
    if (pp->tile_count < 0 || pp->tile_rank < 0 || (pp->tile_count > 0 && pp->tile_rank >= pp->tile_count))
        return setError(PB2_ERR_INVALID, "bad tile_rank / tile_count");
    if (pp->sampler != PB2_SAMPLER_HALTON && pp->sampler != PB2_SAMPLER_SOBOL) return setError(PB2_ERR_INVALID, "unknown sampler");
    if (pp->sampler == PB2_SAMPLER_SOBOL && (pp->samples_per_pixel & (pp->samples_per_pixel - 1)))
        return setError(PB2_ERR_INVALID, "SobolSampler: samples_per_pixel must be the power of two its constructor rounds up to (sobol.h:52)");
    if (film->cropped_pixel_bounds[2] < film->cropped_pixel_bounds[0] || film->cropped_pixel_bounds[3] < film->cropped_pixel_bounds[1])
        return setError(PB2_ERR_INVALID, "bad cropped pixel bounds");
    if (!(film->filter_radius[0] > 0) || !(film->filter_radius[1] > 0)) return setError(PB2_ERR_INVALID, "bad filter radius");
    if (film->filter_type < PB2_FILTER_BOX || film->filter_type > PB2_FILTER_TRIANGLE) return setError(PB2_ERR_INVALID, "unknown filter type");
    return PB2_OK;
}

enum { kMaxPipes = 4 };
typedef void (*TraceKernel)(DScene, WfPool, int, WfChain);
typedef void (*AdvanceKernel)(const DScene *, const DRenderParams *, WfPool, int, int, int, float4 *, unsigned long long *);

struct TraceLaunch {
    TraceKernel fn = nullptr;
    int block = 128;
    size_t smem = 0;
    int grid = 0;
    bool chain = false;
    const char *name = "";
};

static int selectTraceKernel(pb2_scene *scene, int flags, TraceLaunch *out, bool allowChain = false) {
    TraceLaunch t;
    const bool wantChain = allowChain && (flags & PB2_FLAG_CHAIN) != 0;
    const bool spheres = scene->d.spheres != nullptr;
    const bool instanced = scene->d.instances != nullptr;
    const bool records = scene->d.wide4 != nullptr && !(flags & PB2_FLAG_LINEAR_NODES);
    const bool small = (flags & PB2_FLAG_SMALL_STACK) != 0;
    const bool linearFits = !instanced || scene->bvhDepth + 3 + scene->instDepth <= 64;
    if (flags & PB2_FLAG_COUNT_TRAVERSAL) { t.fn = k_wf_trace_plain<true>; t.name = "k_wf_trace_plain<count>"; }
    else if ((flags & PB2_FLAG_PLAIN_TRACE) || (!records && !linearFits)) { t.fn = k_wf_trace_plain<false>; t.name = "k_wf_trace_plain"; }
    else if (scene->d.hasAlpha) {
        if (!records) { t.fn = k_wf_trace_plain<false>; t.name = "k_wf_trace_plain"; }
        else {
            t.name = "k_wf_trace_w<2,alpha>";
            if (instanced) t.fn = k_wf_trace_w<2, 1, 8, 4, 16, 6, true, true, true, false, true>;
            else if (spheres) t.fn = k_wf_trace_w<2, 1, 8, 4, 16, 6, true, false, true, false, true>;
            else t.fn = k_wf_trace_w<2, 1, 8, 4, 16, 6, false, false, true, false, true>;
        }
    } else if (records && (flags & PB2_FLAG_POOL) && !spheres && !instanced) {
        t.name = "k_wf_trace_pool";
        if (!scene->wfSpill)
            CUDA_TRY(cudaMalloc((void **)&scene->wfSpill, (size_t)kMaxPipes * g_numSMs * 8 * 4 * PL_R * PL_SPILL * sizeof(int2)));
        t.fn = k_wf_trace_pool<4, 8, 16, 12, 48, 8>;
        t.smem = 4 * sizeof(PoolWarp<48, 8>);
        CUDA_TRY(cudaFuncSetAttribute(t.fn, cudaFuncAttributeMaxDynamicSharedMemorySize, (int)t.smem));
    } else if (records && (flags & PB2_FLAG_WIDE4)) {
        t.name = "k_wf_trace_w<4>";
        if (flags & PB2_FLAG_LD128) {
            if (instanced) t.fn = small ? k_wf_trace_w<4, 1, 8, 4, 4, 5, true, true> : k_wf_trace_w<4, 1, 8, 4, 16, 5, true, true>;
            else if (spheres) t.fn = small ? k_wf_trace_w<4, 1, 8, 4, 4, 5, true> : k_wf_trace_w<4, 1, 8, 4, 16, 5, true>;
            else t.fn = small ? k_wf_trace_w<4, 1, 8, 4, 4, 7> : k_wf_trace_w<4, 1, 8, 4, 16, 7>;
        } else {
            if (instanced) t.fn = small ? k_wf_trace_w<4, 1, 8, 4, 4, 5, true, true, true> : k_wf_trace_w<4, 1, 8, 4, 16, 5, true, true, true>;
            else if (spheres) t.fn = small ? k_wf_trace_w<4, 1, 8, 4, 4, 5, true, false, true> : k_wf_trace_w<4, 1, 8, 4, 16, 5, true, false, true>;
            else t.fn = small ? k_wf_trace_w<4, 1, 8, 4, 4, 7, false, false, true> : k_wf_trace_w<4, 1, 8, 4, 16, 7, false, false, true>;
        }
    } else if (records) {
        t.name = "k_wf_trace_w<2>";
        if (flags & PB2_FLAG_LD128) {
            if (instanced) t.fn = small ? k_wf_trace_w<2, 1, 8, 4, 4, 6, true, true> : k_wf_trace_w<2, 1, 8, 4, 16, 6, true, true>;
            else if (spheres) t.fn = small ? k_wf_trace_w<2, 1, 8, 4, 4, 6, true> : k_wf_trace_w<2, 1, 8, 4, 16, 6, true>;
            else t.fn = small ? k_wf_trace_w<2, 1, 8, 4, 4, 9> : k_wf_trace_w<2, 1, 8, 4, 16, 9>;
        } else {
            if (instanced) t.fn = small ? k_wf_trace_w<2, 1, 8, 4, 4, 6, true, true, true> : k_wf_trace_w<2, 1, 8, 4, 16, 6, true, true, true>;
            else if (spheres) t.fn = small ? k_wf_trace_w<2, 1, 8, 4, 4, 6, true, false, true> : k_wf_trace_w<2, 1, 8, 4, 16, 6, true, false, true>;
            else if (flags & PB2_FLAG_LEAF_TMA) t.fn = k_wf_trace_w<2, 1, 8, 4, 16, 5, false, false, true, true>;
            else t.fn = small ? k_wf_trace_w<2, 1, 8, 4, 4, 9, false, false, true> : k_wf_trace_w<2, 1, 8, 4, 16, 9, false, false, true>;
            if (wantChain && !small && !(flags & PB2_FLAG_LEAF_TMA)) {
                t.chain = true;
                t.name = "k_wf_trace_w<2,chain>";
                if (instanced) t.fn = k_wf_trace_w<2, 1, 8, 4, 16, 6, true, true, true, false, false, true>;
                else if (spheres) t.fn = k_wf_trace_w<2, 1, 8, 4, 16, 6, true, false, true, false, false, true>;
                else t.fn = k_wf_trace_w<2, 1, 8, 4, 16, 9, false, false, true, false, false, true>;
            }
        }
    } else {
        t.name = "k_wf_trace";
        if (instanced) t.fn = k_wf_trace<8, 8, 2, 32, true, true, 6, true>;
        else if (spheres) t.fn = k_wf_trace<8, 8, 2, 32, true, true, 6>;
        else if (scene->bvhDepth > 32) t.fn = k_wf_trace<12, 8, 4, 32, true, false, 8>;
        else t.fn = k_wf_trace<12, 8, 4, 32, false, false, 8>;
    }
    if (t.name[10] == 'p') {
        *out = t;
        return PB2_OK;
    }
    int blocksPerSM = 1;
    CUDA_TRY(cudaOccupancyMaxActiveBlocksPerMultiprocessor(&blocksPerSM, t.fn, t.block, t.smem));
    blocksPerSM = std::max(1, std::min(blocksPerSM, 8));
    cudaFuncAttributes fa;
    CUDA_TRY(cudaFuncGetAttributes(&fa, t.fn));
    size_t need = (size_t)blocksPerSM * (fa.sharedSizeBytes + t.smem + 1024);
    int pct = (int)std::min<size_t>(100, (need * 100 + 233471) / 233472);
    CUDA_TRY(cudaFuncSetAttribute(t.fn, cudaFuncAttributePreferredSharedMemoryCarveout, pct));
    static const int verbose = envInt("PB2_VERBOSE", 0);
    if (verbose)
        fprintf(stderr, "pb2: trace kernel %s: %d regs, %zu B smem, %d blocks/SM, carve-out %d %%, BVH depth %d\n", t.name, fa.numRegs,
                fa.sharedSizeBytes + t.smem, blocksPerSM, pct, scene->bvhDepth);
    t.grid = g_numSMs * blocksPerSM;
    *out = t;
    return PB2_OK;
}

static int ensurePool(pb2_scene *scene, int capacity) {
    if (scene->wfCapacity < capacity) {
        if (scene->wfCtx) cudaFree(scene->wfCtx);
        if (scene->wfQueues) cudaFree(scene->wfQueues);
        scene->wfCtx = nullptr;
        scene->wfQueues = nullptr;
        scene->wfCapacity = 0;
        CUDA_TRY(cudaMalloc(&scene->wfCtx, (size_t)capacity * sizeof(WfCtx)));
        CUDA_TRY(cudaMalloc((void **)&scene->wfQueues, (size_t)capacity * WQ_COUNT * sizeof(int)));
        scene->wfCapacity = capacity;
    }
    if (!scene->wfCounts) CUDA_TRY(cudaMalloc((void **)&scene->wfCounts, kMaxPipes * WQ_COUNT * sizeof(unsigned)));
    if (!scene->wfHostCounts) CUDA_TRY(cudaMallocHost((void **)&scene->wfHostCounts, (kMaxPipes * WQ_COUNT + 2) * sizeof(unsigned long long)));
    return PB2_OK;
}

static WfPool poolOf(const pb2_scene *scene, int capacity, int pipe = 0, int nPipes = 1) {
    WfPool pool;
    const int cap = capacity / nPipes;
    pool.capacity = cap;
    pool.ctx = (WfCtx *)scene->wfCtx + (size_t)pipe * cap;
    for (int q = 0; q < WQ_COUNT; ++q) pool.queue[q] = scene->wfQueues + ((size_t)pipe * WQ_COUNT + q) * cap;
    pool.counts = scene->wfCounts + (size_t)pipe * WQ_COUNT;
    pool.ctr = scene->counters;
    pool.spill = scene->wfSpill ? scene->wfSpill + (size_t)pipe * g_numSMs * 8 * 4 * PL_R * PL_SPILL : nullptr;
    return pool;
}

static int renderWavefront(pb2_scene *scene, const DRenderParams &rp, float4 *film, cudaStream_t stream, int flags,
                           bool timeTrace, unsigned long long *launches, double *traceMs) {
    const bool lazyLights = scene->lazyLightDist;
    static const int maxCapacity = envInt("PB2_POOL", 1 << 22);
    long long want = std::min<long long>(maxCapacity, std::max<long long>(rp.nWorkItems, 1024));
    int capacity = (int)((want + 255) / 256 * 256);
    int rc = ensurePool(scene, capacity);
    if (rc) return rc;
    TraceLaunch trace;
    if ((rc = selectTraceKernel(scene, flags, &trace, true))) return rc;
    if (!scene->paramBuf) CUDA_TRY(cudaMalloc(&scene->paramBuf, sizeof(DScene) + sizeof(DRenderParams)));
    const DScene *dSc = reinterpret_cast<const DScene *>(scene->paramBuf);
    const DRenderParams *dRp = reinterpret_cast<const DRenderParams *>((char *)scene->paramBuf + sizeof(DScene));
    CUDA_TRY(cudaMemcpyAsync((void *)dSc, &scene->d, sizeof(DScene), cudaMemcpyHostToDevice, stream));
    CUDA_TRY(cudaMemcpyAsync((void *)dRp, &rp, sizeof(DRenderParams), cudaMemcpyHostToDevice, stream));
    WfChain chain;
    memset(&chain, 0, sizeof(chain));
    if (trace.chain) {
        chain.sc = dSc;
        chain.rp = dRp;
        chain.film = film;
    }
    const bool spheres = scene->d.spheres != nullptr;
    AdvanceKernel advLight = spheres ? k_wf_advance<false, true, 7> : k_wf_advance<false, false, 7>;
    AdvanceKernel advShade = scene->hasSpecular ? (spheres ? k_wf_advance<true, true, 4, true> : k_wf_advance<true, false, 4, true>)
                             : spheres ? k_wf_advance<true, true, 4>
                                       : k_wf_advance<true, false, 4>;
    if (scene->lazyLightDist)
        advShade = scene->hasSpecular ? (spheres ? k_wf_advance<true, true, 4, true, true> : k_wf_advance<true, false, 4, true, true>)
                   : spheres ? k_wf_advance<true, true, 4, false, true>
                             : k_wf_advance<true, false, 4, false, true>;
    const bool sobol = rp.halton.sobol != nullptr;
    const bool textured = scene->d.nTextures > 0 || sobol;
    if (textured) advShade = k_wf_advance<true, true, 3, true, true, true>;
    typedef void (*FinishKernel)(const DScene *, const DRenderParams *, WfPool, int, unsigned, float4 *);
    FinishKernel finish = scene->hasSpecular ? (spheres ? k_wf_finish<true, true> : k_wf_finish<false, true>)
                                             : (spheres ? k_wf_finish<true, false> : k_wf_finish<false, false>);
    static const int finishPerSM = envInt("PB2_FINISH", 256);
    const unsigned finishThreshold = ((flags & PB2_FLAG_COUNT_TRAVERSAL) || lazyLights || textured) ? 0u : (unsigned)(g_numSMs * std::max(0, finishPerSM));
    const int finishBlocks = std::max(1, (int)((finishThreshold + 127) / 128));
    static const int syncEvery = std::max(1, envInt("PB2_SYNC_EVERY", 8));
    static const int pipesEnv = envInt("PB2_PIPES", 0);
    const int pipesWanted = std::min((int)kMaxPipes, pipesEnv > 0 ? pipesEnv : 2);
    const int nPipes = (lazyLights || capacity < 65536) ? 1 : pipesWanted;
    cudaStream_t streams[kMaxPipes] = {stream, stream, stream, stream};
    if (nPipes > 1) {
        if (!scene->forkEvent) CUDA_TRY(cudaEventCreateWithFlags(&scene->forkEvent, cudaEventDisableTiming));
        CUDA_TRY(cudaEventRecord(scene->forkEvent, stream));
        for (int p = 1; p < nPipes; ++p) {
            if (!scene->pipeStreams[p]) CUDA_TRY(cudaStreamCreateWithFlags(&scene->pipeStreams[p], cudaStreamNonBlocking));
            if (!scene->joinEvents[p]) CUDA_TRY(cudaEventCreateWithFlags(&scene->joinEvents[p], cudaEventDisableTiming));
            streams[p] = scene->pipeStreams[p];
            CUDA_TRY(cudaStreamWaitEvent(streams[p], scene->forkEvent, 0));
        }
    }
    WfPool pools[kMaxPipes];
    for (int p = 0; p < nPipes; ++p) pools[p] = poolOf(scene, capacity / nPipes * nPipes, p, nPipes);
    const int capP = pools[0].capacity;
    const int blocks128 = std::min((capP + 127) / 128, g_numSMs * 32);
    for (int p = 0; p < nPipes; ++p) k_wf_init<<<(capP + 255) / 256, 256, 0, streams[p]>>>(pools[p]);
    unsigned long long nLaunch = nPipes;
    size_t nEvents = 0;
    int cur = 0;
    volatile unsigned *hc = scene->wfHostCounts;
    unsigned long long *hWork = reinterpret_cast<unsigned long long *>(scene->wfHostCounts + kMaxPipes * WQ_COUNT);
    for (long long round = 0;; ++round) {
        int next = 1 - cur;
        for (int p = 0; p < nPipes; ++p) {
            const WfPool &pool = pools[p];
            cudaStream_t st = streams[p];
            if (sobol) k_wf_gen<true><<<blocks128, 128, 0, st>>>(dRp, pool, WQ_FREE0 + cur, WQ_TRACE0 + cur);
            else k_wf_gen<false><<<blocks128, 128, 0, st>>>(dRp, pool, WQ_FREE0 + cur, WQ_TRACE0 + cur);
            if (timeTrace) {
                if (scene->traceEvents.size() < nEvents + 2) {
                    cudaEvent_t e0, e1;
                    CUDA_TRY(cudaEventCreate(&e0));
                    CUDA_TRY(cudaEventCreate(&e1));
                    scene->traceEvents.push_back(e0);
                    scene->traceEvents.push_back(e1);
                }
                CUDA_TRY(cudaEventRecord(scene->traceEvents[nEvents], st));
            }
            chain.freeQ = WQ_FREE0 + next;
            trace.fn<<<trace.grid ? trace.grid : blocks128, trace.block, trace.smem, st>>>(scene->d, pool, WQ_TRACE0 + cur, chain);
            if (timeTrace) {
                CUDA_TRY(cudaEventRecord(scene->traceEvents[nEvents + 1], st));
                nEvents += 2;
            }
            if (!trace.chain) advLight<<<blocks128, 128, 0, st>>>(dSc, dRp, pool, WQ_LIGHT, WQ_TRACE0 + next, WQ_FREE0 + next, film, scene->counters);
            else --nLaunch;
            advShade<<<blocks128, 128, 0, st>>>(dSc, dRp, pool, WQ_SHADE, WQ_TRACE0 + next, WQ_FREE0 + next, film, scene->counters);
            if (lazyLights) {
                launchLightDistBuild(scene, st);
                advShade<<<blocks128, 128, 0, st>>>(dSc, dRp, pool, WQ_RETRY, WQ_TRACE0 + next, WQ_FREE0 + next, film, scene->counters);
                nLaunch += 3;
            }
            if (finishThreshold) finish<<<finishBlocks, 128, 0, st>>>(dSc, dRp, pool, WQ_TRACE0 + next, finishThreshold, film);
            k_wf_reset<<<1, 32, 0, st>>>(pool, WQ_FREE0 + cur, WQ_TRACE0 + cur, WQ_TRACE0 + next, finishThreshold);
            nLaunch += finishThreshold ? 6 : 5;
        }
        cur = next;
        if ((round + 1) % syncEvery != 0) continue;
        for (int p = 0; p < nPipes; ++p)
            CUDA_TRY(cudaMemcpyAsync((void *)(scene->wfHostCounts + p * WQ_COUNT), pools[p].counts, WQ_COUNT * sizeof(unsigned), cudaMemcpyDeviceToHost, streams[p]));
        for (int p = 1; p < nPipes; ++p) CUDA_TRY(cudaStreamSynchronize(streams[p]));
        CUDA_TRY(cudaMemcpyAsync(hWork, &scene->counters[CTR_WORK], sizeof(unsigned long long), cudaMemcpyDeviceToHost, stream));
        CUDA_TRY(cudaStreamSynchronize(stream));
        bool overflowed = false;
        if ((rc = lightDistOverflowed(scene, stream, &overflowed))) return rc;
        if (overflowed) return lightDistOverflowError();
        const bool workLeft = (long long)*hWork < rp.nWorkItems;
        bool done = true;
        for (int p = 0; p < nPipes; ++p) {
            const unsigned traceNext = hc[p * WQ_COUNT + WQ_TRACE0 + cur], freeNext = hc[p * WQ_COUNT + WQ_FREE0 + cur];
            if (!(traceNext == 0 && !(workLeft && freeNext > 0))) done = false;
        }
        if (done) break;
        if (round > 100000000LL) return setError(PB2_ERR_CUDA, "wavefront did not terminate");
    }
    if (nPipes > 1) {
        for (int p = 1; p < nPipes; ++p) {
            CUDA_TRY(cudaEventRecord(scene->joinEvents[p], streams[p]));
            CUDA_TRY(cudaStreamWaitEvent(stream, scene->joinEvents[p], 0));
        }
    }
    CUDA_TRY(cudaGetLastError());
    *launches = nLaunch;
    *traceMs = 0;
    for (size_t e = 0; e + 1 < nEvents; e += 2) {
        float ms = 0;
        CUDA_TRY(cudaEventElapsedTime(&ms, scene->traceEvents[e], scene->traceEvents[e + 1]));
        *traceMs += ms;
    }
    return PB2_OK;
}

extern "C" {

int pb2_abi_version(void) { return PB2_ABI_VERSION; }
const char *pb2_last_error(void) { return g_lastError.c_str(); }

static void freeDeviceTables() {
    for (DeviceState &d : g_devs) {
        cudaSetDevice(d.id);
        cudaFree(d.primes);
        cudaFree(d.primeSums);
        cudaFree(d.perms);
        cudaFree(d.dimRecs);
        cudaFree(d.dimTabs);
        cudaFree(d.digitTab);
        cudaFree(d.sobol);
        cudaFree(d.sobolVdc);
    }
    g_devs.clear();
    g_initialised = false;
}

int pb2_init_devices(int n, const int *device_ids) {
    int count = 0;
    cudaError_t e = cudaGetDeviceCount(&count);
    if (e != cudaSuccess || count == 0) {
        cudaGetLastError();
        return setError(PB2_ERR_NO_DEVICE, std::string("no CUDA device available (") +
                                               (e != cudaSuccess ? cudaGetErrorString(e) : "device count is 0") +
                                               "); the path-tracing hot path has no CPU fallback");
    }
    std::vector<int> ids;
    if (n <= 0) for (int i = 0; i < count; ++i) ids.push_back(i);
    else {
        if (!device_ids) return setError(PB2_ERR_INVALID, "null device list");
        ids.assign(device_ids, device_ids + n);
    }
    for (size_t i = 0; i < ids.size(); ++i) {
        if (ids[i] < 0 || ids[i] >= count) return setError(PB2_ERR_INVALID, "device id out of range");
        for (size_t j = 0; j < i; ++j)
            if (ids[j] == ids[i]) return setError(PB2_ERR_INVALID, "device listed twice");
    }
    if (g_initialised && g_devs.size() == ids.size()) {
        bool same = true;
        for (size_t i = 0; i < ids.size(); ++i) same &= g_devs[i].id == ids[i];
        if (same) return PB2_OK;
    }
    if (g_dist.comm) return setError(PB2_ERR_INVALID, "pb2_init: shut the communicator down (pb2_dist_shutdown) before rebinding devices");
    freeDeviceTables();
    buildHaltonHostTables();
    t_dev = 0;
    for (int id : ids) {
        CUDA_TRY(cudaSetDevice(id));
        cudaDeviceProp prop;
        CUDA_TRY(cudaGetDeviceProperties(&prop, id));
// ... 91 lines not shown
        if (dim0[i] < 0 || dim0[i] + kSampleBatch > kMaxHaltonDims) return setError(PB2_ERR_INVALID, "dimension out of range");
    DHalton h = makeHalton(film, pp);
    if (pp->sampler == PB2_SAMPLER_SOBOL && (rc = attachSobol(&h, film))) return rc;
    int32_t *dXY = nullptr, *dDim = nullptr;
    int64_t *dS = nullptr;
    float *dOut = nullptr;
    cudaError_t e = cudaMalloc((void **)&dXY, n * 2 * sizeof(int32_t));
    if (e == cudaSuccess) e = cudaMalloc((void **)&dS, n * sizeof(int64_t));
    if (e == cudaSuccess) e = cudaMalloc((void **)&dDim, n * sizeof(int32_t));
    if (e == cudaSuccess) e = cudaMalloc((void **)&dOut, n * kSampleBatch * sizeof(float));
    if (e == cudaSuccess) e = cudaMemcpy(dXY, pixel_xy, n * 2 * sizeof(int32_t), cudaMemcpyHostToDevice);
    if (e == cudaSuccess) e = cudaMemcpy(dS, sample_num, n * sizeof(int64_t), cudaMemcpyHostToDevice);
    if (e == cudaSuccess) e = cudaMemcpy(dDim, dim0, n * sizeof(int32_t), cudaMemcpyHostToDevice);
    if (e == cudaSuccess) {
        k_halton_batch<<<(unsigned)((n + 127) / 128), 128>>>(h, dXY, dS, dDim, n, dOut);
        e = cudaGetLastError();
    }
    if (e == cudaSuccess) e = cudaMemcpy(out, dOut, n * kSampleBatch * sizeof(float), cudaMemcpyDeviceToHost);
    cudaFree(dXY);
    cudaFree(dS);
    cudaFree(dDim);
    cudaFree(dOut);
    if (e != cudaSuccess) return setError(PB2_ERR_CUDA, std::string("pb2_debug_halton_batch_device: ") + cudaGetErrorString(e));
    return PB2_OK;
}

int pb2_work_items(const pb2_film_desc *film, const pb2_path_params *pp, int64_t first, int64_t n, int32_t *out, int64_t *n_items) {
    if (!film || !pp) return setError(PB2_ERR_INVALID, "null argument");
    if (pp->samples_per_pixel <= 0 || pp->tile_count < 0 || pp->tile_rank < 0 || (pp->tile_count > 0 && pp->tile_rank >= pp->tile_count))
        return setError(PB2_ERR_INVALID, "bad samples_per_pixel / tile_rank / tile_count");
    pb2_camera cam;
    memset(&cam, 0, sizeof(cam));
    const DRenderParams rp = makeRenderParams(&cam, film, pp);
    if (n_items) *n_items = rp.nWorkItems;
    for (int64_t i = 0; i < n && out; ++i) {
        int px = -1, py = -1, sample = -1;
        const bool inside = first + i >= 0 && first + i < rp.nWorkItems && decodeWork(rp, first + i, &px, &py, &sample);
        out[3 * i] = inside ? px : -1;
        out[3 * i + 1] = inside ? py : -1;
        out[3 * i + 2] = inside ? sample : -1;
    }
    return PB2_OK;
}

int pb2_dist_unique_id(void *id128) {
    if (!id128) return setError(PB2_ERR_INVALID, "null argument");
    int rc = loadNccl();
    if (rc) return rc;
    static_assert(sizeof(ncclUniqueId) == PB2_DIST_ID_BYTES, "ncclUniqueId is 128 bytes");
    ncclUniqueId id;
    NCCL_TRY(g_nccl.GetUniqueId(&id));
    memcpy(id128, &id, sizeof(id));
    return PB2_OK;
}

int pb2_dist_init(int rank, int world, const void *id128) {
    int rc = requireDevice();
    if (rc) return rc;
    if (world < 1 || rank < 0 || rank >= world || (world > 1 && !id128)) return setError(PB2_ERR_INVALID, "bad rank / world / id");
    if (g_dist.comm) return setError(PB2_ERR_INVALID, "pb2_dist_init: a communicator already exists (call pb2_dist_shutdown first)");
    g_dist.rank = rank;
    g_dist.world = world;
    if (world == 1) return PB2_OK;
    if ((rc = loadNccl())) return rc;
    ncclUniqueId id;
    memcpy(&id, id128, sizeof(id));
    if (g_devs.size() != 1) return setError(PB2_ERR_INVALID, "pb2_dist_init: one device per process (pb2_init), not a local device group");
    CUDA_TRY(cudaSetDevice(g_devs[0].id));
    NCCL_TRY(g_nccl.CommInitRank(&g_dist.comm, world, id, rank));
    return PB2_OK;
}

int pb2_dist_info(int *rank, int *world) {
    if (rank) *rank = g_dist.rank;
    if (world) *world = g_dist.world;
    return PB2_OK;
}

int pb2_dist_shutdown(void) {
    if (g_dist.comm) g_nccl.CommDestroy(g_dist.comm);
    g_dist.comm = nullptr;
    g_dist.rank = 0;
    g_dist.world = 1;
    return PB2_OK;
}

int pb2_host_alloc(size_t bytes, void **out) {
    if (!out) return setError(PB2_ERR_INVALID, "null argument");
    *out = nullptr;
    int rc = requireDevice();
    if (rc) return rc;
    CUDA_TRY(cudaMallocHost(out, std::max<size_t>(bytes, 1)));
    return PB2_OK;
}

int pb2_host_free(void *p) {
    if (p) cudaFreeHost(p);
    return PB2_OK;
}

int pb2_scene_destroy(pb2_scene *s) {
    if (!s) return PB2_OK;
    for (pb2_scene *r : s->replicas) pb2_scene_destroy(r);
    s->replicas.clear();
    if (g_initialised && (size_t)s->devIndex < g_devs.size()) cudaSetDevice(g_devs[(size_t)s->devIndex].id);
    for (void *p : s->allocations) cudaFree(p);
    if (s->film) cudaFree(s->film);
    if (s->filterTable) cudaFree(s->filterTable);
    if (s->wfCtx) cudaFree(s->wfCtx);
    if (s->wfQueues) cudaFree(s->wfQueues);
    if (s->wfCounts) cudaFree(s->wfCounts);
    if (s->wfHostCounts) cudaFreeHost(s->wfHostCounts);
    if (s->ldHostCounters) cudaFreeHost(s->ldHostCounters);
    for (cudaEvent_t e : s->traceEvents) cudaEventDestroy(e);
    if (s->wfSpill) cudaFree(s->wfSpill);
    if (s->paramBuf) cudaFree(s->paramBuf);
    for (int p = 0; p < 4; ++p) {
        if (s->pipeStreams[p]) cudaStreamDestroy(s->pipeStreams[p]);
        if (s->joinEvents[p]) cudaEventDestroy(s->joinEvents[p]);
    }
    if (s->forkEvent) cudaEventDestroy(s->forkEvent);
    delete s;
    if (g_initialised) cudaSetDevice(g_devs[0].id);
    return PB2_OK;
}

static int createSceneOnCurrentDevice(const pb2_scene_desc *d, pb2_scene **out);

int pb2_scene_create(const pb2_scene_desc *d, pb2_scene **out) {
    if (!d || !out) return setError(PB2_ERR_INVALID, "null argument");
    *out = nullptr;
    int rc = requireDevice();
    if (rc) return rc;
    t_dev = 0;
    CUDA_TRY(cudaSetDevice(g_devs[0].id));
    pb2_scene *primary = nullptr;
    if ((rc = createSceneOnCurrentDevice(d, &primary))) return rc;
    for (size_t i = 1; i < g_devs.size() && rc == PB2_OK; ++i) {
        t_dev = (int)i;
        pb2_scene *rep = nullptr;
        if (cudaSetDevice(g_devs[i].id) != cudaSuccess) rc = setError(PB2_ERR_CUDA, "cudaSetDevice failed");
        else if ((rc = createSceneOnCurrentDevice(d, &rep)) == PB2_OK) {
            rep->devIndex = (int)i;
            primary->replicas.push_back(rep);
        }
    }
    t_dev = 0;
    cudaSetDevice(g_devs[0].id);
    if (rc) {
        pb2_scene_destroy(primary);
        return rc;
    }
    *out = primary;
    return PB2_OK;
}

static float texLanczos(float x) {
    const float tau = 2;
    x = std::abs(x);
    if (x < 1e-5f) return 1;
    if (x > 1.f) return 0;
    x *= 3.14159265358979323846f;
    float sv = std::sin(x * tau) / (x * tau);
    float lanczos = std::sin(x) / x;
    return sv * lanczos;
}
struct TexResampleWeight {
    int firstTexel;
    float weight[4];
};
static std::vector<TexResampleWeight> texResampleWeights(int oldRes, int newRes) {
    std::vector<TexResampleWeight> wt((size_t)newRes);
    const float filterwidth = 2.f;
    for (int i = 0; i < newRes; ++i) {
        float center = (i + .5f) * oldRes / newRes;
        wt[i].firstTexel = (int)std::floor((center - filterwidth) + 0.5f);
        for (int j = 0; j < 4; ++j) {
            float pos = wt[i].firstTexel + j + .5f;
            wt[i].weight[j] = texLanczos((pos - center) / filterwidth);
        }
        float invSumWts = 1 / (wt[i].weight[0] + wt[i].weight[1] + wt[i].weight[2] + wt[i].weight[3]);
        for (int j = 0; j < 4; ++j) wt[i].weight[j] *= invSumWts;
    }
    return wt;
}
static int texWrapIndex(int i, int n, int wrap) {
    if (wrap == PB2_WRAP_REPEAT) return texMod(i, n);
    if (wrap == PB2_WRAP_CLAMP) return i < 0 ? 0 : (i > n - 1 ? n - 1 : i);
    return (i >= 0 && i < n) ? i : -1;
}
static int buildTexturePyramid(const pb2_texture &in, std::vector<float> &pool, DTexture *out) {
    if (in.kind != PB2_TEXKIND_IMAGE) return setError(PB2_ERR_INVALID, "texture: not an image (a constant or a combinator has no pyramid)");
    if ((in.channels != 1 && in.channels != 3) || in.width <= 0 || in.height <= 0 || !in.texels)
        return setError(PB2_ERR_INVALID, "texture: channels must be 1 or 3, the resolution positive, texels not null");
    if (in.wrap < PB2_WRAP_REPEAT || in.wrap > PB2_WRAP_CLAMP) return setError(PB2_ERR_INVALID, "texture: unknown wrap mode");
    if (in.width > 32768 || in.height > 32768) return setError(PB2_ERR_UNSUPPORTED, "texture larger than 32768 in one direction");
    const int C = in.channels;
    int rw = in.width, rh = in.height;
    std::vector<float> level0;
    auto isPow2 = [](int v) { return v && !(v & (v - 1)); };
    auto roundUpPow2 = [](int v) { int p = 1; while (p < v) p <<= 1; return p; };
    if (!isPow2(rw) || !isPow2(rh)) {
        const int pw = roundUpPow2(rw), ph = roundUpPow2(rh);
        std::vector<float> img((size_t)pw * ph * C, 0.f);
        std::vector<TexResampleWeight> sW = texResampleWeights(rw, pw);
        for (int t = 0; t < rh; ++t)
            for (int sx = 0; sx < pw; ++sx)
                for (int c = 0; c < C; ++c) {
                    float v = 0.f;
                    for (int j = 0; j < 4; ++j) {
                        int origS = texWrapIndex(sW[sx].firstTexel + j, rw, in.wrap);
                        if (origS >= 0 && origS < rw) v += sW[sx].weight[j] * in.texels[((size_t)t * rw + origS) * C + c];
                    }
                    img[((size_t)t * pw + sx) * C + c] = v;
                }
        std::vector<TexResampleWeight> tW = texResampleWeights(rh, ph);
        std::vector<float> work((size_t)ph);
        for (int sx = 0; sx < pw; ++sx)
            for (int c = 0; c < C; ++c) {
                for (int t = 0; t < ph; ++t) {
                    float v = 0.f;
                    for (int j = 0; j < 4; ++j) {
                        int offset = texWrapIndex(tW[t].firstTexel + j, rh, in.wrap);
                        if (offset >= 0 && offset < rh) v += tW[t].weight[j] * img[((size_t)offset * pw + sx) * C + c];
                    }
                    work[t] = v;
                }
                for (int t = 0; t < ph; ++t) img[((size_t)t * pw + sx) * C + c] = work[t] < 0.f ? 0.f : work[t];
            }
        level0.swap(img);
        rw = pw;
        rh = ph;
    } else
        level0.assign(in.texels, in.texels + (size_t)rw * rh * C);
    int nLevels = 1;
    for (int m = std::max(rw, rh); m > 1; m >>= 1) ++nLevels;
    memset(out, 0, sizeof(*out));
    out->channels = C;
    out->nLevels = nLevels;
    out->w = rw;
    out->h = rh;
    out->wrap = in.wrap;
    out->doTrilinear = in.do_trilinear != 0;
    out->maxAniso = in.max_anisotropy;
    out->su = in.su; out->sv = in.sv; out->du = in.du; out->dv = in.dv;
    out->levelOfs[0] = (long long)pool.size();
    pool.insert(pool.end(), level0.begin(), level0.end());
    int pw = rw, ph = rh;
    for (int i = 1; i < nLevels; ++i) {
        const int sRes = std::max(1, pw / 2), tRes = std::max(1, ph / 2);
        const size_t prev = (size_t)out->levelOfs[i - 1];
        out->levelOfs[i] = (long long)pool.size();
        pool.resize(pool.size() + (size_t)sRes * tRes * C);
        float *dst = pool.data() + out->levelOfs[i];
        const float *src = pool.data() + prev;
        auto texel = [&](int sx, int t, int c) -> float {
            sx = texWrapIndex(sx, pw, in.wrap);
            t = texWrapIndex(t, ph, in.wrap);
            if (sx < 0 || t < 0) return 0.f;
            return src[((size_t)t * pw + sx) * C + c];
        };
        for (int t = 0; t < tRes; ++t)
            for (int sx = 0; sx < sRes; ++sx)
                for (int c = 0; c < C; ++c)
                    dst[((size_t)t * sRes + sx) * C + c] =
                        .25f * (texel(2 * sx, 2 * t, c) + texel(2 * sx + 1, 2 * t, c) + texel(2 * sx, 2 * t + 1, c) + texel(2 * sx + 1, 2 * t + 1, c));
        pw = sRes;
        ph = tRes;
    }
    return PB2_OK;
}

static void texWeightLut(std::vector<float> &pool);
struct HostTextures {
    std::vector<float> pool;
    std::vector<DTexture> tex;
};
static int buildHostTextures(const pb2_scene_desc *d, HostTextures *host);
static int uploadTextures(pb2_scene *s, const pb2_scene_desc *d, HostTextures *host) {
    DScene &sc = s->d;
    if (d->n_textures <= 0) return PB2_OK;
    int rc = buildHostTextures(d, host);
    if (rc) return rc;
    if ((rc = upload(s, host->tex.data(), host->tex.size(), &sc.textures))) return rc;
    if ((rc = upload(s, host->pool.data(), host->pool.size(), &sc.texels))) return rc;
    sc.nTextures = d->n_textures;
    return PB2_OK;
}
static int buildHostTextures(const pb2_scene_desc *d, HostTextures *host) {
    if (!d->textures) return setError(PB2_ERR_INVALID, "n_textures > 0 but textures is null");
    std::vector<float> &pool = host->pool;
    texWeightLut(pool);
    std::vector<DTexture> &tex = host->tex;
    tex.resize((size_t)d->n_textures);
    std::vector<int> depth((size_t)d->n_textures, 0);
    for (int i = 0; i < d->n_textures; ++i) {
        const pb2_texture &in = d->textures[i];
        if (in.kind == PB2_TEXKIND_IMAGE) {
            int rc = buildTexturePyramid(in, pool, &tex[i]);
            if (rc) return rc;
            continue;
        }
        DTexture &t = tex[i];
        memset(&t, 0, sizeof(t));
        if (in.channels != 1 && in.channels != 3) return setError(PB2_ERR_INVALID, "texture: channels must be 1 or 3");
        t.channels = in.channels;
        t.kind = in.kind;
        for (int c = 0; c < 3; ++c) t.value[c] = in.value[in.channels == 3 ? c : 0];
        if (in.kind == PB2_TEXKIND_CONSTANT) continue;
        t.su = in.su; t.sv = in.sv; t.du = in.du; t.dv = in.dv;
        if (in.kind == PB2_TEXKIND_UV) {
            if (in.channels != 3) return setError(PB2_ERR_INVALID, "texture: a uv texture has three channels");
            continue;
        }
        if (in.kind == PB2_TEXKIND_CHECKERBOARD) t.value[0] = in.value[0];
        else if (in.kind != PB2_TEXKIND_SCALE && in.kind != PB2_TEXKIND_MIX) return setError(PB2_ERR_INVALID, "texture: unknown kind");
        const int nChildren = in.kind == PB2_TEXKIND_MIX ? 3 : 2;
        for (int c = 0; c < nChildren; ++c) {
            const int id = in.child[c];
            if (id < 1 || id > i) return setError(PB2_ERR_INVALID, "texture combinator: a child must precede its parent in the texture array");
            const int want = (in.kind == PB2_TEXKIND_MIX && c == 2) ? 1 : in.channels;
            if (d->textures[id - 1].channels != want) return setError(PB2_ERR_INVALID, "texture combinator: child with the wrong number of channels");
            t.child[c] = id;
            depth[i] = std::max(depth[i], depth[(size_t)id - 1] + 1);
        }
        if (depth[i] > TEX_MAX_DEPTH) return setError(PB2_ERR_UNSUPPORTED, "texture combinators nested more than three levels deep");
    }
    return PB2_OK;
}

extern "C" int pb2_texture_eval_host(const pb2_texture *textures, int32_t n_textures, int32_t id, int64_t n, const float *uv,
                                     const float *duv, float *out) {
    if (!textures || n_textures <= 0 || id < 0 || id >= n_textures || (n > 0 && (!uv || !duv || !out))) return setError(PB2_ERR_INVALID, "bad argument");
    pb2_scene_desc d;
    memset(&d, 0, sizeof(d));
    d.n_textures = n_textures;
    d.textures = textures;
    HostTextures host;
    int rc = buildHostTextures(&d, &host);
    if (rc) return rc;
    for (int64_t i = 0; i < n; ++i) {
        DUvDiff dd;
        dd.dudx = duv[4 * i];
        dd.dvdx = duv[4 * i + 1];
        dd.dudy = duv[4 * i + 2];
        dd.dvdy = duv[4 * i + 3];
        const V3 v = texEvaluateNode(host.tex.data(), host.pool.data(), id, mk2(uv[2 * i], uv[2 * i + 1]), dd);
        out[3 * i] = v.x;
        out[3 * i + 1] = v.y;
        out[3 * i + 2] = v.z;
    }
    return PB2_OK;
}

static void texWeightLut(std::vector<float> &pool) {
    pool.assign((size_t)TEX_LUT_SIZE, 0.f);
    for (int i = 0; i < TEX_LUT_SIZE; ++i) {
        float alpha = 2;
        float r2 = float(i) / float(TEX_LUT_SIZE - 1);
        pool[i] = std::exp(-alpha * r2) - std::exp(-alpha);
    }
}

extern "C" int pb2_texture_pyramid(const pb2_texture *texture, int32_t level, int32_t *n_levels, int32_t *w, int32_t *h, float *out) {
    if (!texture || !n_levels || !w || !h) return setError(PB2_ERR_INVALID, "null argument");
    std::vector<float> pool;
    DTexture t;
    int rc = buildTexturePyramid(*texture, pool, &t);
    if (rc) return rc;
    if (level < 0 || level >= t.nLevels) return setError(PB2_ERR_INVALID, "texture level out of range");
    *n_levels = t.nLevels;
    *w = std::max(1, t.w >> level);
    *h = std::max(1, t.h >> level);
    if (out) memcpy(out, pool.data() + t.levelOfs[level], (size_t)*w * *h * t.channels * sizeof(float));
    return PB2_OK;
}

__global__ void k_texture_lookup(DTexture tx, const float *pool, int64_t n, const float *st, const float *dst, float *out) {
    int64_t i = blockIdx.x * (int64_t)blockDim.x + threadIdx.x;
    if (i >= n) return;
    V3 v = texLookup(tx, pool, mk2(st[2 * i], st[2 * i + 1]), mk2(dst[4 * i], dst[4 * i + 1]), mk2(dst[4 * i + 2], dst[4 * i + 3]));
    out[3 * i] = v.x;
    out[3 * i + 1] = v.y;
    out[3 * i + 2] = v.z;
}

extern "C" int pb2_texture_lookup(const pb2_texture *texture, int64_t n, const float *st, const float *dst, float *out) {
    if (!g_initialised) return setError(PB2_ERR_NO_DEVICE, "pb2_init was not called or failed (no CUDA device: this library has no CPU fallback)");
    if (!texture || n < 0 || (n > 0 && (!st || !dst || !out))) return setError(PB2_ERR_INVALID, "null argument");
    std::vector<float> pool;
    texWeightLut(pool);
    DTexture t;
    int rc = buildTexturePyramid(*texture, pool, &t);
    if (rc || n == 0) return rc;
    float *dPool = nullptr, *dSt = nullptr, *dDst = nullptr, *dOut = nullptr;
    cudaError_t e = cudaMalloc((void **)&dPool, pool.size() * sizeof(float));
    if (e == cudaSuccess) e = cudaMalloc((void **)&dSt, (size_t)n * 2 * sizeof(float));
    if (e == cudaSuccess) e = cudaMalloc((void **)&dDst, (size_t)n * 4 * sizeof(float));
    if (e == cudaSuccess) e = cudaMalloc((void **)&dOut, (size_t)n * 3 * sizeof(float));
    if (e == cudaSuccess) e = cudaMemcpy(dPool, pool.data(), pool.size() * sizeof(float), cudaMemcpyHostToDevice);
    if (e == cudaSuccess) e = cudaMemcpy(dSt, st, (size_t)n * 2 * sizeof(float), cudaMemcpyHostToDevice);
    if (e == cudaSuccess) e = cudaMemcpy(dDst, dst, (size_t)n * 4 * sizeof(float), cudaMemcpyHostToDevice);
    if (e == cudaSuccess) {
        k_texture_lookup<<<(unsigned)((n + 127) / 128), 128>>>(t, dPool, n, dSt, dDst, dOut);
        e = cudaGetLastError();
    }
    if (e == cudaSuccess) e = cudaMemcpy(out, dOut, (size_t)n * 3 * sizeof(float), cudaMemcpyDeviceToHost);
    cudaFree(dPool);
    cudaFree(dSt);
    cudaFree(dDst);
    cudaFree(dOut);
    if (e != cudaSuccess) return setError(PB2_ERR_CUDA, cudaGetErrorString(e));
    return PB2_OK;
}

static int buildEnvDistribution(const DTexture &tx, const float *pool, std::vector<float> *out) {
    const int width = 2 * tx.w, height = 2 * tx.h;
    if ((size_t)width * height > ((size_t)1 << 27)) return setError(PB2_ERR_UNSUPPORTED, "environment map too large for its sampling table");
    const size_t rowStride = 2 * (size_t)width + 2;
    std::vector<float> &table = *out;
    table.assign((size_t)height * rowStride + 2 * (size_t)height + 2, 0.f);
    const float fwidth = 0.5f / std::min(width, height);
    for (int v = 0; v < height; ++v) {
        const float vp = (v + .5f) / (float)height;
        const float sinTheta = std::sin(3.14159265358979323846f * (v + .5f) / height);
        float *row = table.data() + (size_t)v * rowStride;
        for (int u = 0; u < width; ++u) {
            const float up = (u + .5f) / (float)width;
            const V3 c = texLookupWidth(tx, pool, mk2(up, vp), fwidth);
            row[u] = 0.212671f * c.x + 0.715160f * c.y + 0.072169f * c.z;
            row[u] *= sinTheta;
        }
        finishVoxelDistribution(width, row);
    }
    float *marginal = table.data() + (size_t)height * rowStride;
    for (int v = 0; v < height; ++v) marginal[v] = table[(size_t)v * rowStride + 2 * (size_t)width + 1];
    finishVoxelDistribution(height, marginal);
    return PB2_OK;
}

extern "C" int pb2_env_distribution(const pb2_texture *texture, int32_t *nu, int32_t *nv, float *out) {
    if (!texture || !nu || !nv) return setError(PB2_ERR_INVALID, "null argument");
    std::vector<float> pool;
    texWeightLut(pool);
    DTexture t;
    int rc = buildTexturePyramid(*texture, pool, &t);
    if (rc) return rc;
    *nu = 2 * t.w;
    *nv = 2 * t.h;
    if (!out) return PB2_OK;
    std::vector<float> table;
    if ((rc = buildEnvDistribution(t, pool.data(), &table))) return rc;
    memcpy(out, table.data(), table.size() * sizeof(float));
    return PB2_OK;
}

static int createSceneOnCurrentDevice(const pb2_scene_desc *d, pb2_scene **out) {
    int rc = PB2_OK;
    if (d->n_prims <= 0 || d->n_nodes <= 0 || !d->nodes || !d->bvh_prims || !d->prim_type || !d->prim_index)
        return setError(PB2_ERR_INVALID, "scene has no primitives / BVH");
    if (d->n_prims > 0x7fffffffLL || d->n_nodes > 0x7fffffffLL) return setError(PB2_ERR_UNSUPPORTED, "more than 2^31 primitives/nodes");
    for (int i = 0; i < d->n_materials; ++i)
        if (d->materials[i].type < PB2_MAT_NONE || d->materials[i].type > PB2_MAT_UBER)
            return setError(PB2_ERR_UNSUPPORTED, "material type outside the path's scope (matte, plastic, substrate, metal, uber, mirror, glass)");
    for (int i = 0; i < d->n_materials; ++i)
        for (int k = 0; k < PB2_TEX_SLOTS; ++k) {
            const int id = d->materials[i].tex[k];
            if (!id) continue;
            if (id < 0 || id > d->n_textures || !d->textures) return setError(PB2_ERR_INVALID, "material texture index out of range");
            const bool spectrum = k == PB2_TEX_KD || k == PB2_TEX_KS || k == PB2_TEX_KR || k == PB2_TEX_KT || k == PB2_TEX_OPACITY ||
                                  k == PB2_TEX_METAL_ETA || k == PB2_TEX_METAL_K;
            if (d->textures[id - 1].channels != (spectrum ? 3 : 1))
                return setError(PB2_ERR_INVALID, "material texture has the wrong number of channels for its parameter");
        }
    bool hasAlpha = false;
    for (int i = 0; i < d->n_meshes; ++i)
        for (int id : {d->meshes[i].alpha_tex, d->meshes[i].shadow_alpha_tex}) {
            if (!id) continue;
            if (id < 0 || id > d->n_textures || !d->textures || d->textures[id - 1].channels != 1)
                return setError(PB2_ERR_INVALID, "mesh alpha texture: index out of range or not a one-channel texture");
            hasAlpha = true;
        }
    struct Guard {
        pb2_scene *s;
        ~Guard() { if (s) pb2_scene_destroy(s); }
    } guard{new pb2_scene()};
    pb2_scene *s = guard.s;
    s->devIndex = t_dev;
    for (int i = 0; i < d->n_materials; ++i)
        if (d->materials[i].type == PB2_MAT_MIRROR || d->materials[i].type == PB2_MAT_GLASS || d->materials[i].type == PB2_MAT_SUBSTRATE ||
            d->materials[i].type == PB2_MAT_METAL || d->materials[i].type == PB2_MAT_UBER)
            s->hasSpecular = true;
    DScene &sc = s->d;
    memset(&sc, 0, sizeof(sc));
    sc.nNodes = d->n_nodes;
    sc.nPrims = d->n_prims;
    sc.nTris = d->n_tris;
    sc.nLights = d->n_lights;
    s->nPrims = d->n_prims;
    s->nLights = d->n_lights;
    std::vector<pb2_bvh> bvhs;
    int64_t nBvhPrims = d->n_prims;
    if (d->n_bvhs >= 1) {
        if (!d->bvhs) return setError(PB2_ERR_INVALID, "n_bvhs > 0 but bvhs is null");
        bvhs.assign(d->bvhs, d->bvhs + d->n_bvhs);
        nBvhPrims = d->n_bvh_prims;
        if (nBvhPrims <= 0 || nBvhPrims > d->n_prims) return setError(PB2_ERR_INVALID, "bad n_bvh_prims");
    } else
        bvhs.push_back(pb2_bvh{0, d->n_nodes, 0, d->n_prims});
    if (d->n_instances < 0 || (d->n_instances > 0 && !d->instances)) return setError(PB2_ERR_INVALID, "bad instances");
    for (const pb2_bvh &b : bvhs)
        if (b.node_offset < 0 || b.n_nodes <= 0 || b.node_offset + b.n_nodes > d->n_nodes || b.prim_offset < 0 || b.n_prims <= 0 ||
            b.prim_offset + b.n_prims > nBvhPrims)
            return setError(PB2_ERR_INVALID, "BVH range out of bounds");
    std::vector<pb2_bvh_node> rebased;
    if (bvhs.size() > 1) rebased.assign(d->nodes, d->nodes + d->n_nodes);
    s->bvhDepth = 0;
    for (size_t k = 0; k < bvhs.size(); ++k) {
        const pb2_bvh &b = bvhs[k];
        std::vector<std::pair<int64_t, int>> todo{{0, 0}};
        int depth = 0;
        while (!todo.empty()) {
            std::pair<int64_t, int> nd = todo.back();
            todo.pop_back();
            if (nd.first < 0 || nd.first >= b.n_nodes) return setError(PB2_ERR_INVALID, "BVH child index out of range");
            depth = std::max(depth, nd.second);
            const pb2_bvh_node &node = d->nodes[b.node_offset + nd.first];
            if (node.n_prims == 0) {
                if (nd.second > 4096) return setError(PB2_ERR_INVALID, "BVH is not a tree");
                todo.push_back({nd.first + 1, nd.second + 1});
                todo.push_back({(int64_t)node.offset, nd.second + 1});
                if (!rebased.empty()) rebased[b.node_offset + nd.first].offset = (int32_t)(node.offset + b.node_offset);
            } else {
                if ((int64_t)node.offset + node.n_prims > b.n_prims || node.offset < 0)
                    return setError(PB2_ERR_INVALID, "BVH leaf range out of bounds");
                if (!rebased.empty()) rebased[b.node_offset + nd.first].offset = (int32_t)(node.offset + b.prim_offset);
            }
        }
        if (depth > 64) return setError(PB2_ERR_UNSUPPORTED, "BVH deeper than the reference's 64-entry traversal stack (bvh.cpp:671)");
        if (k == 0) s->bvhDepth = depth;
        else s->instDepth = std::max(s->instDepth, depth);
    }
    for (int64_t j = 0; j < nBvhPrims; ++j)
        if (d->bvh_prims[j] < 0 || d->bvh_prims[j] >= d->n_prims) return setError(PB2_ERR_INVALID, "bvh_prims entry out of range");
    for (int64_t i = 0; i < d->n_prims; ++i) {
        if (d->prim_type[i] == PB2_PRIM_INSTANCE) {
            if (d->prim_index[i] < 0 || d->prim_index[i] >= d->n_instances) return setError(PB2_ERR_INVALID, "instance index out of range");
        } else if (d->prim_type[i] != PB2_PRIM_TRIANGLE && d->prim_type[i] != PB2_PRIM_SPHERE)
            return setError(PB2_ERR_UNSUPPORTED, "primitive type outside the path's scope");
    }
    const pb2_bvh_node *nodes;
    if ((rc = upload(s, rebased.empty() ? d->nodes : rebased.data(), (size_t)d->n_nodes, &nodes))) return rc;
    sc.instances = nullptr;
    sc.nInstances = d->n_instances;
    std::vector<DInstance> inst((size_t)std::max(0, d->n_instances));
    if (d->n_instances > 0) {
        const float identity[16] = {1, 0, 0, 0, 0, 1, 0, 0, 0, 0, 1, 0, 0, 0, 0, 1};
        for (int i = 0; i < d->n_instances; ++i) {
            const pb2_instance &pi = d->instances[i];
            memcpy(inst[i].i2w.m, pi.instance_to_world, sizeof(float) * 16);
            memcpy(inst[i].w2i.m, pi.world_to_instance, sizeof(float) * 16);
            inst[i].identity = memcmp(pi.instance_to_world, identity, sizeof(identity)) == 0;
            inst[i].wroot = pi.bvh >= 0 ? pi.bvh : -1;
            inst[i].wroot4 = -1;
            if (pi.bvh >= 0) {
                if (pi.bvh == 0 || pi.bvh >= (int)bvhs.size()) return setError(PB2_ERR_INVALID, "instance BVH out of range");
                inst[i].root = (int)bvhs[pi.bvh].node_offset;
                inst[i].lone = -1;
            } else {
                if (pi.lone_prim < 0 || pi.lone_prim >= nBvhPrims) return setError(PB2_ERR_INVALID, "instance primitive out of range");
                if (d->prim_type[d->bvh_prims[pi.lone_prim]] == PB2_PRIM_INSTANCE) return setError(PB2_ERR_INVALID, "instance of an instance");
                inst[i].root = -1;
                inst[i].lone = pi.lone_prim;
            }
        }
        for (size_t k = 1; k < bvhs.size(); ++k)
            for (int64_t j = 0; j < bvhs[k].n_prims; ++j)
                if (d->prim_type[d->bvh_prims[bvhs[k].prim_offset + j]] == PB2_PRIM_INSTANCE)
                    return setError(PB2_ERR_INVALID, "instance inside an object BVH (api.cpp:1554-1557 forbids it)");
    }
    sc.nodes = reinterpret_cast<const float4 *>(nodes);
    sc.wide = nullptr;
    sc.wide4 = nullptr;
    if (d->n_nodes > 0 && d->n_prims < (int64_t)WIDE_MAX_PRIMS) {
        const pb2_bvh_node *src = rebased.empty() ? d->nodes : rebased.data();
        const int32_t nBvh = (int32_t)bvhs.size();
        std::vector<int32_t> wideOf((size_t)d->n_nodes, -1);
        int32_t nWide = nBvh;
        bool fits = true;
        for (int64_t i = 0; i < d->n_nodes; ++i) {
            if (src[i].n_prims == 0) wideOf[i] = nWide++;
            else if (src[i].n_prims > WIDE_MAX_LEAF) fits = false;
        }
        if (fits) {
            struct WideRec { float b[12]; uint32_t ref0, ref1, meta, pad; };
            static_assert(sizeof(WideRec) == 64, "wide record is 64 bytes");
            std::vector<WideRec> wide((size_t)nWide);
            auto childRef = [&](int64_t i) -> uint32_t {
                const pb2_bvh_node &n = src[i];
                return n.n_prims == 0 ? (uint32_t)wideOf[i] : (WIDE_LEAF | ((uint32_t)(n.n_prims - 1) << WIDE_LEAF_COUNT_SHIFT) | (uint32_t)n.offset);
            };
            auto putBox = [&](float *dst, const pb2_bvh_node &n) {
                dst[0] = n.bmin[0]; dst[1] = n.bmin[1]; dst[2] = n.bmin[2];
                dst[3] = n.bmax[0]; dst[4] = n.bmax[1]; dst[5] = n.bmax[2];
            };
            memset(wide.data(), 0, wide.size() * sizeof(WideRec));
            for (int32_t k = 0; k < nBvh; ++k) {
                const int64_t root = bvhs[(size_t)k].node_offset;
                putBox(wide[(size_t)k].b, src[root]);
                putBox(wide[(size_t)k].b + 6, src[root]);
                wide[(size_t)k].ref0 = wide[(size_t)k].ref1 = childRef(root);
                wide[(size_t)k].meta = WIDE_SINGLE;
            }
            for (int64_t i = 0; i < d->n_nodes; ++i) {
                const pb2_bvh_node &n = src[i];
                if (n.n_prims != 0) continue;
                WideRec &w = wide[(size_t)wideOf[i]];
                putBox(w.b, src[i + 1]);
                putBox(w.b + 6, src[n.offset]);
                w.ref0 = childRef(i + 1);
                w.ref1 = childRef(n.offset);
                w.meta = (uint32_t)n.axis & 3u;
            }
            const WideRec *dWide;
            if ((rc = upload(s, wide.data(), wide.size(), &dWide))) return rc;
            sc.wide = reinterpret_cast<const float4 *>(dWide);
            std::vector<int64_t> roots(bvhs.size());
            for (size_t k = 0; k < bvhs.size(); ++k) roots[k] = bvhs[k].node_offset;
            std::vector<int32_t> rootRecord(bvhs.size(), 0);
            const std::vector<float4> wide4 = buildWide4Records(src, roots.data(), roots.size(), rootRecord.data());
            const float4 *dWide4;
            if ((rc = upload(s, wide4.data(), wide4.size(), &dWide4))) return rc;
            sc.wide4 = dWide4;
            for (int i = 0; i < d->n_instances; ++i)
                inst[(size_t)i].wroot4 = d->instances[i].bvh >= 0 ? rootRecord[(size_t)d->instances[i].bvh] : -1;
        }
    }
    if (d->n_instances > 0) {
        const DInstance *dInst;
        if ((rc = upload(s, inst.data(), inst.size(), &dInst))) return rc;
        sc.instances = dInst;
    }
    if ((rc = upload(s, d->P, 3 * (size_t)d->n_vertices, &sc.P))) return rc;
    if ((rc = upload(s, d->N, d->N ? 3 * (size_t)d->n_vertices : 0, &sc.N))) return rc;
    if ((rc = upload(s, d->UV, d->UV ? 2 * (size_t)d->n_vertices : 0, &sc.UV))) return rc;
// ... 1240 lines not shown
```

### pbrt_v3_b200/csrc/pb2_wavefront.cuh

```cuda
#ifndef PB2_WAVEFRONT_CUH
#define PB2_WAVEFRONT_CUH

struct alignas(32) WfCtx {
    DLane ln;
    alignas(16) float4 hit;
    float tHit;
    int found;
    V2 pFilm;
};
static_assert(offsetof(WfCtx, ln) == 0 && offsetof(DLane, state) == 0 && offsetof(DLane, ray) == 4 && sizeof(DRay) == 28,
              "the trace kernels read the first 32 bytes of a context as {state, o, d, tMax}");
static_assert(offsetof(WfCtx, tHit) % 8 == 0 && offsetof(WfCtx, found) == offsetof(WfCtx, tHit) + 4, "tHit/found are stored as one float2");
static_assert(sizeof(DLane) == 192 && offsetof(WfCtx, hit) == 192 && offsetof(WfCtx, tHit) == 208 && offsetof(WfCtx, pFilm) == 216 &&
                  sizeof(WfCtx) == 224 && sizeof(WfCtx) % 32 == 0,
              "a context is seven whole 32-byte sectors: the lane (six), then hit, tHit / found and pFilm (one)");

struct WfSlot {
    DLane ln;
    float hit[4];
    float tHit;
    int found;
    V2 pFilm;
    int pad[2];
};
static_assert(offsetof(WfSlot, hit) == offsetof(WfCtx, hit) && offsetof(WfSlot, tHit) == offsetof(WfCtx, tHit) &&
                  offsetof(WfSlot, found) == offsetof(WfCtx, found) && offsetof(WfSlot, pFilm) == offsetof(WfCtx, pFilm) &&
                  sizeof(WfSlot) == 232 && alignof(WfSlot) == 8,
              "a slot holds a context's bytes at the context's offsets, 8-byte aligned, 58 words apart");

enum { WF_OUT_START = 96, WF_OUT_LIGHT = 128, WF_OUT_SHADE = (int)sizeof(DLane) };
static_assert(offsetof(DLane, lightNum) == 88 && offsetof(DLane, pick) == 92 && offsetof(DLane, ldSum) == 96 && offsetof(DLane, ldLight) == 108 &&
                  offsetof(DLane, bounces) < 96 && offsetof(DLane, misTerm) == 120,
              "the written-back prefixes above cover the fields their kernels change");

__device__ __forceinline__ int wfLaneId() {
    int lane;
    asm volatile("mov.u32 %0, %%laneid;" : "=r"(lane));
    return lane;
}

__device__ __forceinline__ void wfStageIn(const WfCtx *ctx, WfSlot *warpSlots, int c) {
    constexpr int CHUNKS = sizeof(WfCtx) / 16, BATCH = CHUNKS / 2;
    const int lane = wfLaneId();
    __syncwarp();
#pragma unroll
    for (int b = 0; b < 2; ++b) {
        uint4 v[BATCH];
        int cs[BATCH];
#pragma unroll
        for (int it = 0; it < BATCH; ++it) {
            const int q = (b * BATCH + it) * 32 + lane, j = q / CHUNKS, k = q % CHUNKS;
            cs[it] = __shfl_sync(0xffffffffu, c, j);
            if (cs[it] >= 0) v[it] = __ldcs(reinterpret_cast<const uint4 *>(ctx + cs[it]) + k);
        }
#pragma unroll
        for (int it = 0; it < BATCH; ++it) {
            const int q = (b * BATCH + it) * 32 + lane, j = q / CHUNKS, k = q % CHUNKS;
            if (cs[it] >= 0) {
                uint2 *s = reinterpret_cast<uint2 *>(reinterpret_cast<char *>(&warpSlots[j]) + 16 * k);
                s[0] = make_uint2(v[it].x, v[it].y);
                s[1] = make_uint2(v[it].z, v[it].w);
            }
        }
    }
    __syncwarp();
}

template <int BYTES>
__device__ __forceinline__ void wfStageOut(WfCtx *ctx, const WfSlot *warpSlots, int c) {
    static_assert(BYTES % 32 == 0 && BYTES <= (int)sizeof(DLane), "whole sectors of the lane");
    constexpr int CHUNKS = BYTES / 16;
    const int lane = wfLaneId();
    __syncwarp();
#pragma unroll
    for (int it = 0; it < CHUNKS; ++it) {
        const int q = it * 32 + lane, j = q / CHUNKS, k = q % CHUNKS;
        const int cj = __shfl_sync(0xffffffffu, c, j);
        if (cj >= 0) {
            const uint2 *s = reinterpret_cast<const uint2 *>(reinterpret_cast<const char *>(&warpSlots[j]) + 16 * k);
            const uint2 lo = s[0], hi = s[1];
            __stcs(reinterpret_cast<uint4 *>(ctx + cj) + k, make_uint4(lo.x, lo.y, hi.x, hi.y));
        }
    }
    __syncwarp();
}

enum { WQ_TRACE0 = 0, WQ_TRACE1 = 1, WQ_SHADE = 2, WQ_LIGHT = 3, WQ_FREE0 = 4, WQ_FREE1 = 5, WQ_CURSOR = 6, WQ_RETRY = 7, WQ_COUNT = 8 };
enum { WQ_FINISH = WQ_RETRY, WF_FINISH_WAIT = 1, WF_FINISH_GO = 2 };

struct WfPool {
    int capacity;
    WfCtx *ctx;
    int *queue[WQ_COUNT];
    unsigned *counts;
    unsigned long long *ctr;
    int2 *spill;
};

__device__ __forceinline__ int *wfQueue(const WfPool &pool, int q) {
    int *list = pool.queue[0];
#pragma unroll
    for (int k = 1; k < WQ_COUNT; ++k) {
        int *entry = pool.queue[k];
        asm("" : "+l"(entry));
        list = q == k ? entry : list;
    }
    return list;
}

__device__ __forceinline__ void wfPush(int *queue, unsigned *counter, int value, bool participate) {
    unsigned mask = __ballot_sync(0xffffffffu, participate);
    if (!mask) return;
    int lane = threadIdx.x & 31;
    int leader = __ffs(mask) - 1;
    unsigned base = 0;
    if (lane == leader) base = atomicAdd(counter, (unsigned)__popc(mask));
    base = __shfl_sync(0xffffffffu, base, leader);
    if (participate) queue[base + __popc(mask & ((1u << lane) - 1u))] = value;
}

__device__ __forceinline__ void wfCountRays(unsigned long long *counters, unsigned regular, unsigned shadow) {
    for (int o = 16; o > 0; o >>= 1) {
        regular += __shfl_down_sync(0xffffffffu, regular, o);
        shadow += __shfl_down_sync(0xffffffffu, shadow, o);
    }
    if ((threadIdx.x & 31) == 0) {
        if (regular) atomicAdd(&counters[CTR_REGULAR], (unsigned long long)regular);
        if (shadow) atomicAdd(&counters[CTR_SHADOW], (unsigned long long)shadow);
    }
}

struct WfChain {
    const DScene *sc;
    const DRenderParams *rp;
    float4 *film;
    int freeQ;
    int pad;
};

template <bool SPH>
__device__ __noinline__ int wfChainLight(const WfChain &ch, WfCtx *cx, bool found) {
    DLane &ln = cx->ln;
    const float4 h4 = cx->hit;
    const int foundCode = cx->found;
    DHit hit;
    hit.leaf = __float_as_int(h4.x);
    hit.b0 = h4.y;
    hit.b1 = h4.z;
    hit.b2 = h4.w;
    hit.inst = foundCode >= 2 ? foundCode - 2 : -1;
    lightAdvance<SPH>(*ch.sc, ln, found, hit, cx->tHit);
    if (ln.state == LS_IDLE) addSample(*ch.rp, ch.film, cx->pFilm, guardRadiance(ln.L));
    return ln.state;
}

template <bool GENERAL>
__device__ __forceinline__ bool wfStartSample(const DRenderParams &rp, const WfPool &pool, WfSlot &slot, bool want, unsigned *cameraRays) {
    bool started = false;
    while (__any_sync(0xffffffffu, want && !started)) {
        const bool draw = want && !started;
        const unsigned mask = __ballot_sync(0xffffffffu, draw);
        const int lane = threadIdx.x & 31, leader = __ffs(mask) - 1;
        unsigned long long w0 = 0;
        if (lane == leader) w0 = atomicAdd(&pool.ctr[CTR_WORK], (unsigned long long)__popc(mask));
        w0 = __shfl_sync(0xffffffffu, w0, leader);
        if (draw) {
            const long long item = (long long)w0 + __popc(mask & ((1u << lane) - 1u));
            if (item >= rp.nWorkItems) {
                want = false;
            } else {
                int px, py, sample;
                if (decodeWork(rp, item, &px, &py, &sample)) {
                    DSampler smp;
                    smp.index = sampleIndex<GENERAL>(rp.halton, px, py, sample);
                    smp.dim = 0;
                    V2 pFilm;
                    DRay ray = generateCameraRay<GENERAL>(rp.cam, rp.halton, smp, px, py, &pFilm);
                    laneStartPath(slot.ln, ray, smp);
                    slot.pFilm = pFilm;
                    ++*cameraRays;
                    started = true;
                }
            }
        }
    }
    return started;
}

template <bool GENERAL>
__global__ void __launch_bounds__(128) k_wf_gen(const DRenderParams *__restrict__ rpp, WfPool pool, int freeQ, int traceQ) {
    __shared__ WfSlot stage[128];
    WfSlot &slot = stage[threadIdx.x];
    WfSlot *warpSlots = stage + (threadIdx.x & ~31u);
    const DRenderParams &rp = *rpp;
    const int *freeList = wfQueue(pool, freeQ);
    int *traceList = wfQueue(pool, traceQ);
    const unsigned n = pool.counts[freeQ];
    unsigned stride = gridDim.x * blockDim.x;
    unsigned cameraRays = 0;
    for (unsigned base = blockIdx.x * blockDim.x; base < n; base += stride) {
        unsigned i = base + threadIdx.x;
        const bool have = i < n;
        const int c = have ? freeList[i] : -1;
        const bool started = wfStartSample<GENERAL>(rp, pool, slot, have, &cameraRays);
        if (started) {
            slot.ln.lightNum = 0;
            slot.ln.pick = 0;
            __stcs(reinterpret_cast<float2 *>(&pool.ctx[c].pFilm), make_float2(slot.pFilm.x, slot.pFilm.y));
        }
        wfStageOut<WF_OUT_START>(pool.ctx, warpSlots, started ? c : -1);
// ... 703 lines not shown
                    state = (fl & 1) ? LS_SHADOW : __ldcs(&cx.ln.state);
                    __stcs(reinterpret_cast<float2 *>(&cx.tHit), make_float2(pw.f[6][s], __int_as_float((fl & 2) ? 1 : 0)));
                }
                wfPush(pool.queue[WQ_SHADE], &pool.counts[WQ_SHADE], c, flush && state == LS_PATH);
                wfPush(pool.queue[WQ_LIGHT], &pool.counts[WQ_LIGHT], c, flush && state != LS_PATH);
                bool want = (flush || mode == PL_EMPTY) && !exhausted;
                const unsigned wantMask = __ballot_sync(FULL, want);
                int newFlags = 0;
                if (wantMask) {
                    const int leader = __ffs(wantMask) - 1;
                    unsigned base = 0;
                    if (lane == leader) base = atomicAdd(&pool.counts[WQ_CURSOR], (unsigned)__popc(wantMask));
                    base = __shfl_sync(FULL, base, leader);
                    const unsigned idx = base + __popc(wantMask & ltMask);
                    if (want && idx < n) {
                        c = pool.queue[traceQ][idx];
                        const float4 *p = reinterpret_cast<const float4 *>(&pool.ctx[c]);
                        const float4 ra = __ldcs(p), rb = __ldcs(p + 1);
                        const DRaySetup rs = setupRay(mk3(ra.y, ra.z, ra.w), mk3(rb.x, rb.y, rb.z));
                        pw.f[0][s] = rs.o.x; pw.f[1][s] = rs.o.y; pw.f[2][s] = rs.o.z;
                        pw.f[3][s] = rs.invDir.x; pw.f[4][s] = rs.invDir.y; pw.f[5][s] = rs.invDir.z;
                        pw.f[6][s] = rb.w;
                        pw.f[7][s] = rs.Sx; pw.f[8][s] = rs.Sy; pw.f[9][s] = rs.Sz;
                        pw.i[0][s] = 0;
                        pw.i[1][s] = 0;
                        pw.i[2][s] = c;
                        newFlags = ((__float_as_int(ra.x) == LS_SHADOW) ? 1 : 0) | (rs.neg0 << 2) | (rs.neg1 << 3) | (rs.neg2 << 4) | (rs.kx << 5) |
                                   (rs.ky << 7) | (rs.kz << 9) | (rs.slow << 11) | (PL_NODE << 12);
                    }
                    if (__any_sync(FULL, want && idx >= n)) exhausted = true;
                }
                if (flush || want) pw.i[3][s] = newFlags;
            }
            __syncwarp();
            continue;
        }

        const unsigned b0 = phase == PL_NODE ? bN0 : bL0, b1 = phase == PL_NODE ? bN1 : bL1;
        const int c0 = __popc(b0);
        if (b0 & (1u << lane)) pw.list[__popc(b0 & ltMask)] = lane;
        if (b1 & (1u << lane)) pw.list[c0 + __popc(b1 & ltMask)] = lane + 32;
        __syncwarp();
        const int nSel = min(c0 + __popc(b1), 32);
        const bool active = lane < nSel;
        const int s = active ? pw.list[lane] : 0;
        __syncwarp();

        if (phase == PL_NODE) {
            DRaySetup rs;
            rs.o = mk3(pw.f[0][s], pw.f[1][s], pw.f[2][s]);
            rs.invDir = mk3(pw.f[3][s], pw.f[4][s], pw.f[5][s]);
            float tMax = pw.f[6][s];
            int cur = pw.i[0][s], sp = pw.i[1][s];
            int fl = pw.i[3][s];
            rs.neg0 = (fl >> 2) & 1; rs.neg1 = (fl >> 3) & 1; rs.neg2 = (fl >> 4) & 1;
            rs.kx = rs.ky = rs.kz = 0;
            rs.Sx = rs.Sy = rs.Sz = 0;
            rs.slow = (fl >> 11) & 1;
            int mode = active ? (int)PL_NODE : (int)PL_EMPTY;
            int leafFirst = 0, leafN = 0;
            const bool warpSlow = __any_sync(FULL, active && rs.slow != 0);
#pragma unroll
            for (int sub = 0; sub < NSUB; ++sub) {
                {
                    const bool need = (mode == PL_NODE) & (cur < 0);
                    const bool empty = need & (sp == 0);
                    const bool pop = need & !empty;
                    int2 e = make_int2(0, 0);
                    if (pop) e = stGet(s, sp - 1);
                    sp = pop ? sp - 1 : sp;
                    const bool take = pop & (__int_as_float(e.y) < tMax);
                    const bool leafRef = take & (e.x < 0);
                    leafFirst = leafRef ? (e.x & (int)WIDE_LEAF_OFFSET_MASK) : leafFirst;
                    leafN = leafRef ? (((e.x >> WIDE_LEAF_COUNT_SHIFT) & 0xf) + 1) : leafN;
                    cur = (take & !leafRef) ? e.x : cur;
                    mode = leafRef ? (int)PL_LEAF : mode;
                    if (empty) mode = PL_DONE;
                }
                if (mode == PL_NODE && cur >= 0) {
                    const float4 *w = &sc.wide[4 * (size_t)cur];
                    float4 q0, q1, q2, q3;
                    ldg256(w, q0, q1);
                    ldg256(w + 2, q2, q3);
                    float t0, t1;
                    bool p0, p1;
                    if (warpSlow) slabTestPair(q0, q1, q2, rs, tMax, &p0, &p1, &t0, &t1);
                    else slabTestPairFast(q0, q1, q2, rs, tMax, &p0, &p1, &t0, &t1);
                    const uint32_t meta = floatBits(q3.z);
                    if (meta & WIDE_SINGLE) p1 = false;
                    const int axis = (int)(meta & 3u);
                    const bool isNeg = (axis == 0 ? rs.neg0 : (axis == 1 ? rs.neg1 : rs.neg2)) != 0;
                    const int ref0 = asInt(q3.x), ref1 = asInt(q3.y);
                    const bool both = p0 & p1;
                    if (both) stPut(s, sp, make_int2(isNeg ? ref0 : ref1, __float_as_int(isNeg ? t0 : t1)));
                    sp += both ? 1 : 0;
                    const int ref = (both ? isNeg : !p0) ? ref1 : ref0;
                    const bool have = p0 | p1;
                    const bool isLeaf = have & (ref < 0);
                    leafFirst = isLeaf ? (ref & (int)WIDE_LEAF_OFFSET_MASK) : leafFirst;
                    leafN = isLeaf ? (((ref >> WIDE_LEAF_COUNT_SHIFT) & 0xf) + 1) : leafN;
                    mode = isLeaf ? (int)PL_LEAF : (int)PL_NODE;
                    cur = (have & !isLeaf) ? ref : -1;
                }
            }
            if (active) {
                pw.i[0][s] = cur;
                pw.i[1][s] = sp;
                pw.i[3][s] = (fl & 0xfff) | (mode << 12);
                pw.i[4][s] = leafFirst;
                pw.i[5][s] = leafN;
            }
        } else {
            if (active) {
                DRaySetup rs;
                rs.o = mk3(pw.f[0][s], pw.f[1][s], pw.f[2][s]);
                rs.invDir = mk3(0, 0, 0);
                float tMax = pw.f[6][s];
                rs.Sx = pw.f[7][s]; rs.Sy = pw.f[8][s]; rs.Sz = pw.f[9][s];
                int fl = pw.i[3][s];
                rs.neg0 = rs.neg1 = rs.neg2 = 0;
                rs.kx = (fl >> 5) & 3; rs.ky = (fl >> 7) & 3; rs.kz = (fl >> 9) & 3;
                rs.slow = 0;
                const int c = pw.i[2][s];
                int leafFirst = pw.i[4][s], leafN = pw.i[5][s];
                const bool any = (fl & 1) != 0;
                bool finished = false;
                while (leafN > 0) {
                    const int idx = leafFirst;
                    ++leafFirst;
                    --leafN;
                    const float4 *rec = &sc.leafPrims[3 * (size_t)idx];
                    const float4 a = ldg4(rec), b = ldg4(rec + 1), c4 = ldg4(rec + 2);
                    const uint32_t pf = floatBits(b.w);
                    float t, b0, b1, b2;
                    if (triangleTest(mk3(a.x, a.y, a.z), mk3(b.x, b.y, b.z), mk3(c4.x, c4.y, c4.z), rs, tMax, &t, &b0, &b1, &b2)) {
                        if (any) { fl |= 2; finished = true; break; }
                        if (pf & LEAF_DEGENERATE) continue;
                        fl |= 2;
                        tMax = t;
                        __stcs(reinterpret_cast<float4 *>(&pool.ctx[c].hit), make_float4(__int_as_float(idx), b0, b1, b2));
                    }
                }
                const int sp = pw.i[1][s];
                const int mode = (finished || sp == 0) ? (int)PL_DONE : (int)PL_NODE;
                pw.f[6][s] = tMax;
                pw.i[0][s] = -1;
                pw.i[3][s] = (fl & 0xfff) | (mode << 12);
            }
        }
        __syncwarp();
    }
}

template <bool SHADE, bool SPH, int MINB, bool SPEC = false, bool LAZY = false, bool TEX = false>
__global__ void __launch_bounds__(128, MINB) k_wf_advance(const DScene *__restrict__ scp, const DRenderParams *__restrict__ rpp, WfPool pool,
                                                          int srcQ, int traceQ, int freeQ, float4 *film, unsigned long long *counters) {
    __shared__ WfSlot stage[128];
    __shared__ float sampleRows[SHADE ? 128 * (kSampleBatch + 1) : 1];
    WfSlot &slot = stage[threadIdx.x];
    WfSlot *warpSlots = stage + (threadIdx.x & ~31u);
    float *u = sampleRows + (SHADE ? threadIdx.x * (kSampleBatch + 1) : 0);
    const DScene &sc = *scp;
    const DRenderParams &rp = *rpp;
    const int *srcList = wfQueue(pool, srcQ);
    int *traceList = wfQueue(pool, traceQ), *freeList = wfQueue(pool, freeQ);
    unsigned n = pool.counts[srcQ];
    unsigned stride = gridDim.x * blockDim.x;
    unsigned regular = 0, shadow = 0;
    for (unsigned base = blockIdx.x * blockDim.x; base < n; base += stride) {
        unsigned i = base + threadIdx.x;
        bool have = i < n;
        int c = have ? srcList[i] : 0;
        bool ended = false, deferred = false;
        wfStageIn(pool.ctx, warpSlots, have ? c : -1);
        if (have) {
            DLane &ln = slot.ln;
            const int foundCode = slot.found;
            DHit hit;
            hit.leaf = __float_as_int(slot.hit[0]);
            hit.b0 = slot.hit[1];
            hit.b1 = slot.hit[2];
            hit.b2 = slot.hit[3];
            hit.inst = foundCode >= 2 ? foundCode - 2 : -1;
            bool found = foundCode != 0;
            float tHit = slot.tHit;
            if (SHADE && TEX) {
                DTexCtx tc;
                tc.cam = &rp.cam;
                tc.pFilm = slot.pFilm;
                tc.diffScale = rp.diffScale;
                shadeVertex<SPH, SPEC, LAZY, true>(sc, rp.halton, rp.path, ln, found, hit, tHit, u, &tc);
            } else if (SHADE) shadeVertex<SPH, SPEC, LAZY>(sc, rp.halton, rp.path, ln, found, hit, tHit, u);
            else lightAdvance<SPH>(sc, ln, found, hit, tHit);
            if (SHADE && LAZY && ln.state == LS_DEFER) {
                ln.state = LS_PATH;
                deferred = true;
            } else {
                ended = ln.state == LS_IDLE;
                if (ended) addSample(rp, film, slot.pFilm, guardRadiance(ln.L));
                else if (ln.state == LS_SHADOW) shadow++;
                else regular++;
            }
        }
        wfStageOut<SHADE ? WF_OUT_SHADE : WF_OUT_LIGHT>(pool.ctx, warpSlots, have && !ended ? c : -1);
        if (SHADE && LAZY) wfPush(pool.queue[WQ_RETRY], &pool.counts[WQ_RETRY], c, deferred);
        wfPush(traceList, &pool.counts[traceQ], c, have && !ended && !deferred);
        wfPush(freeList, &pool.counts[freeQ], c, have && ended);
    }
    wfCountRays(counters, regular, shadow);
}

__device__ __forceinline__ bool wfFinishNow(const DRenderParams &rp, const WfPool &pool, int traceQ, unsigned threshold) {
    const unsigned n = pool.counts[traceQ];
    return n > 0 && n <= threshold && (long long)pool.ctr[CTR_WORK] >= rp.nWorkItems;
}

template <bool SPH, bool SPEC>
__global__ void __launch_bounds__(128) k_wf_finish(const DScene *__restrict__ scp, const DRenderParams *__restrict__ rpp, WfPool pool, int traceQ,
                                                   unsigned threshold, float4 *film) {
    const DScene &sc = *scp;
    const DRenderParams &rp = *rpp;
    __shared__ bool sGo;
    if (threadIdx.x == 0) {
        const unsigned mine = wfFinishNow(rp, pool, traceQ, threshold) ? WF_FINISH_GO : WF_FINISH_WAIT;
        const unsigned first = atomicCAS(&pool.counts[WQ_FINISH], 0u, mine);
        sGo = (first ? first : mine) == WF_FINISH_GO;
    }
    __syncthreads();
    if (!sGo) return;
    const unsigned n = pool.counts[traceQ];
    const int *traceList = wfQueue(pool, traceQ);
    unsigned regular = 0, shadow = 0;
    for (unsigned i = blockIdx.x * blockDim.x + threadIdx.x; i < n; i += gridDim.x * blockDim.x) {
        WfCtx &cx = pool.ctx[traceList[i]];
        DLane &ln = cx.ln;
        while (ln.state != LS_IDLE) {
            DHit hit;
            float tMax;
            const bool found = traceLane(sc, ln, &tMax, &hit, nullptr);
            laneAdvance<SPH, SPEC>(sc, rp.halton, rp.path, ln, found, hit, tMax);
            if (ln.state == LS_DEFER) break;
            if (ln.state == LS_SHADOW) shadow++;
            else if (ln.state != LS_IDLE) regular++;
        }
        addSample(rp, film, cx.pFilm, guardRadiance(ln.L));
    }
    wfCountRays(pool.ctr, regular, shadow);
}

__global__ void __launch_bounds__(128) k_lightdist_build(DScene sc, DHalton h) {
    const DLightDist &ld = sc.lightDist;
    const int nReq = ld.counters[0];
    __shared__ int sRecord;
    for (int r = blockIdx.x; r < nReq; r += gridDim.x) {
        const int voxel = ld.requests[r];
        if (threadIdx.x == 0) {
            int k = atomicAdd(&ld.counters[1], 1);
            if (k >= ld.poolRecords) {
                ld.counters[2] = 1;
                k = -1;
            }
            sRecord = k;
        }
        __syncthreads();
        const int k = sRecord;
        if (k >= 0) {
            float *rec = const_cast<float *>(ld.table) + (size_t)k * ld.stride;
            const int pz = voxel % ld.nVoxels[2], py = (voxel / ld.nVoxels[2]) % ld.nVoxels[1], px = voxel / (ld.nVoxels[2] * ld.nVoxels[1]);
            const DVoxelBounds vb = voxelBounds(ld, px, py, pz);
            for (int j = threadIdx.x; j < sc.nLights; j += blockDim.x) rec[j] = voxelLightContribution(sc, h, vb, j);
            __syncthreads();
            if (threadIdx.x == 0) {
                finishVoxelDistribution(sc.nLights, rec);
                __threadfence();
                ld.slots[voxel] = k;
            }
        }
        __syncthreads();
    }
}
__global__ void k_lightdist_done(DScene sc) {
    if (threadIdx.x == 0 && blockIdx.x == 0) sc.lightDist.counters[0] = 0;
}

__global__ void k_wf_init(WfPool pool) {
    unsigned i = blockIdx.x * blockDim.x + threadIdx.x;
    if (i < (unsigned)pool.capacity) pool.queue[WQ_FREE0][i] = (int)i;
    if (i < WQ_COUNT) pool.counts[i] = (i == WQ_FREE0) ? (unsigned)pool.capacity : 0u;
}

__global__ void k_wf_reset(WfPool pool, int a, int b, int traceNext, unsigned threshold) {
    if (threadIdx.x == 0) {
        if (threshold && pool.counts[WQ_FINISH] == WF_FINISH_GO) pool.counts[traceNext] = 0;
        pool.counts[WQ_RETRY] = 0;
        pool.counts[WQ_CURSOR] = 0;
        pool.counts[WQ_SHADE] = 0;
        pool.counts[WQ_LIGHT] = 0;
        pool.counts[a] = 0;
        pool.counts[b] = 0;
    }
}

#endif
```

Before: 193.4.

## Specialize wavefront shading kernels for Lambertian area-light scenes and stage fewer context sectors

Measured after the change: 223.0, median of 6. 15.3% higher.

```diff
diff --git a/include/pb2.h b/include/pb2.h
--- a/include/pb2.h
+++ b/include/pb2.h
@@ -271,6 +271,7 @@
 
 int pb2_scene_create(const pb2_scene_desc *desc, pb2_scene **out);
 int pb2_scene_destroy(pb2_scene *scene);
+int pb2_shade_class(const pb2_scene_desc *desc, int32_t *out);
 
 int pb2_intersect(pb2_scene *scene, const pb2_ray *rays, int64_t n, pb2_hit *hits);
 int pb2_intersect_p(pb2_scene *scene, const pb2_ray *rays, int64_t n, uint8_t *occluded);
diff --git a/pbrt_v3_b200/csrc/device/pb2_path.cuh b/pbrt_v3_b200/csrc/device/pb2_path.cuh
--- a/pbrt_v3_b200/csrc/device/pb2_path.cuh
+++ b/pbrt_v3_b200/csrc/device/pb2_path.cuh
@@ -71,7 +71,7 @@
     float diffScale;
 };
 
-template <bool SPH, bool SPEC = true, bool LAZY = true, bool TEX = false>
+template <bool SPH, bool SPEC = true, bool LAZY = true, bool TEX = false, int FC = SHADE_ALL>
 PB2_HD void shadeVertex(const DScene &sc, const DHalton &h, const DPathParams &pp, DLane &ln, bool found, const DHit &hit,
                         float tMax, float *u, const DTexCtx *tc = nullptr) {
     const int dim0 = ln.smp.dim;
@@ -111,8 +111,9 @@
         if (found) {
             if (li >= 0) ln.L = ln.L + ln.beta * lightL(sc.lights[li], isect.n, -ln.ray.d);
         } else {
-            for (int k = 0; k < sc.nInfinite; ++k)
-                ln.L = ln.L + ln.beta * infiniteLe(sc, sc.lights[sc.infinite[k]], sc.deltaLights[sc.infinite[k]], ln.ray.d);
+            if (FC & SHADE_NON_AREA)
+                for (int k = 0; k < sc.nInfinite; ++k)
+                    ln.L = ln.L + ln.beta * infiniteLe(sc, sc.lights[sc.infinite[k]], sc.deltaLights[sc.infinite[k]], ln.ray.d);
         }
     }
     if (!found || ln.bounces >= pp.maxDepth) {
@@ -121,7 +122,7 @@
     }
     if (TEX) ln.camRay = false;
     DBsdf bsdf;
-    if (!makeBsdf<SPEC, TEX>(sc, isect, &bsdf, TEX ? &uvDiff : nullptr)) {
+    if (!makeBsdf<SPEC, TEX, FC>(sc, isect, &bsdf, TEX ? &uvDiff : nullptr)) {
         ln.ray = spawnRay(isect, ln.ray.d);
         return;
     }
@@ -146,11 +147,11 @@
             const TriRec lightRec = loadTriRec(sc.lightRecs, (size_t)lightNum);
             V2 uLight = get2D<TEX>(h, smp, u, dim0);
             V2 uScattering = get2D<TEX>(h, smp, u, dim0);
-            DLightSample ls = sampleLight<SPH>(sc, lightNum, light, lightRec, isect, uLight);
+            DLightSample ls = sampleLight<SPH, FC>(sc, lightNum, light, lightRec, isect, uLight);
             float lightPdf = ls.pdf, scatteringPdf = 0;
             if (lightPdf > 0 && !isBlack(ls.Li)) {
-                V3 f = bsdfF<SPEC>(bsdf, isect.wo, ls.wi) * absDot(ls.wi, isect.ns);
-                scatteringPdf = bsdfPdf<SPEC>(bsdf, isect.wo, ls.wi);
+                V3 f = bsdfF<SPEC, FC>(bsdf, isect.wo, ls.wi) * absDot(ls.wi, isect.ns);
+                scatteringPdf = bsdfPdf<SPEC, FC>(bsdf, isect.wo, ls.wi);
                 if (!isBlack(f)) {
                     shadow = spawnRayTo(isect, ls.p, ls.pError, ls.n);
                     hasShadow = true;
@@ -162,16 +163,16 @@
             V3 wi;
             V3 f = mk3(0, 0, 0);
             if (!ls.delta) {
-                f = bsdfSampleF<SPEC>(bsdf, isect.wo, &wi, uScattering, &scatteringPdf, nullptr, true);
+                f = bsdfSampleF<SPEC, FC>(bsdf, isect.wo, &wi, uScattering, &scatteringPdf, nullptr, true);
                 if (scatteringPdf != 0) f = f * absDot(wi, isect.ns);
                 else f = mk3(0, 0, 0);
             }
             if (!isBlack(f) && scatteringPdf > 0) {
-                lightPdf = lightPdfLi<SPH>(sc, light, lightRec, isect, wi, lightNum);
+                lightPdf = lightPdfLi<SPH, FC>(sc, light, lightRec, isect, wi, lightNum);
                 if (lightPdf != 0) {
                     float weight = powerHeuristic(scatteringPdf, lightPdf);
                     V3 Lmis = mk3(light.L[0], light.L[1], light.L[2]);
-                    if (sc.deltaLights && light.type == PB2_LIGHT_INFINITE) Lmis = infiniteLe(sc, light, sc.deltaLights[lightNum], wi);
+                    if ((FC & SHADE_NON_AREA) && sc.deltaLights && light.type == PB2_LIGHT_INFINITE) Lmis = infiniteLe(sc, light, sc.deltaLights[lightNum], wi);
                     V3 fl = f * Lmis * weight;
                     ln.misTerm = mk3(fl.x / scatteringPdf, fl.y / scatteringPdf, fl.z / scatteringPdf);
                     DRay mr = spawnRay(isect, wi);
@@ -188,7 +189,7 @@
         V3 wo = -ln.ray.d, wi;
         float pdf;
         int sampled = 0;
-        V3 f = bsdfSampleF<SPEC>(bsdf, wo, &wi, get2D<TEX>(h, smp, u, dim0), &pdf, &sampled);
+        V3 f = bsdfSampleF<SPEC, FC>(bsdf, wo, &wi, get2D<TEX>(h, smp, u, dim0), &pdf, &sampled);
         if (!(isBlack(f) || pdf == 0.f)) {
             V3 s = f * absDot(wi, isect.ns);
             V3 beta = ln.beta * mk3(s.x / pdf, s.y / pdf, s.z / pdf);
@@ -224,15 +225,16 @@
         startMisOrFinish(ln);
 }
 
-template <bool SPH>
+template <bool SPH, int FC = SHADE_ALL>
 PB2_HD void lightAdvance(const DScene &sc, DLane &ln, bool found, const DHit &hit, float tMax) {
+    const bool nonArea = (FC & SHADE_NON_AREA) && sc.deltaLights;
     if (ln.state == LS_SHADOW) {
         if (!found) ln.ldSum = ln.ldSum + ln.ldLight;
         startMisOrFinish(ln);
     } else {
         if (!found) {
-            if (sc.deltaLights && sc.lights[ln.lightNum].type == PB2_LIGHT_INFINITE) ln.ldSum = ln.ldSum + ln.misTerm;
-        } else if (!(sc.deltaLights && sc.lights[ln.lightNum].type == PB2_LIGHT_INFINITE)) {
+            if (nonArea && sc.lights[ln.lightNum].type == PB2_LIGHT_INFINITE) ln.ldSum = ln.ldSum + ln.misTerm;
+        } else if (!(nonArea && sc.lights[ln.lightNum].type == PB2_LIGHT_INFINITE)) {
             float4 b = ldg4(&sc.leafPrims[3 * (size_t)hit.leaf + 1]), c = ldg4(&sc.leafPrims[3 * (size_t)hit.leaf + 2]);
             int hitLight = asInt(c.w);
             if (SPH && (floatBits(b.w) & LEAF_SPHERE)) hitLight = sc.primLight[asInt(ldg4(&sc.leafPrims[3 * (size_t)hit.leaf]).w)];
@@ -249,14 +251,14 @@
     }
 }
 
-template <bool SPH, bool SPEC = true, bool TEX = false>
+template <bool SPH, bool SPEC = true, bool TEX = false, int FC = SHADE_ALL>
 PB2_HD bool laneAdvance(const DScene &sc, const DHalton &h, const DPathParams &pp, DLane &ln, bool found, const DHit &hit,
                         float tMax, const DTexCtx *tc = nullptr) {
     if (ln.state == LS_PATH) {
         float u[kSampleBatch];
-        shadeVertex<SPH, SPEC, true, TEX>(sc, h, pp, ln, found, hit, tMax, u, tc);
-    } else
-        lightAdvance<SPH>(sc, ln, found, hit, tMax);
+        shadeVertex<SPH, SPEC, true, TEX, FC>(sc, h, pp, ln, found, hit, tMax, u, tc);
+    } else
+        lightAdvance<SPH, FC>(sc, ln, found, hit, tMax);
     return ln.state == LS_IDLE;
 }
 
diff --git a/pbrt_v3_b200/csrc/device/pb2_shade.cuh b/pbrt_v3_b200/csrc/device/pb2_shade.cuh
--- a/pbrt_v3_b200/csrc/device/pb2_shade.cuh
+++ b/pbrt_v3_b200/csrc/device/pb2_shade.cuh
@@ -245,6 +245,7 @@
     float e;
 };
 enum { BSDF_SAMPLED_SPECULAR = 1, BSDF_SAMPLED_TRANSMISSION = 2 };
+enum { SHADE_OREN_NAYAR = 1, SHADE_MICROFACET = 2, SHADE_NON_AREA = 4, SHADE_ALL = 7, SHADE_LAMBERT_AREA = 0 };
 enum { GEN_OPACITY = 1, GEN_LAMBERT = 2, GEN_MICROFACET = 4, GEN_SPEC_REFLECTION = 8, GEN_SPEC_TRANSMISSION = 16,
        GEN_MICRO_TRANSMISSION = 32,
        GEN_LOBES = 6, GEN_NON_SPECULAR = GEN_LAMBERT | GEN_MICROFACET | GEN_MICRO_TRANSMISSION };
@@ -301,7 +302,7 @@
     it->dpdus = dpdu;
 }
 
-template <bool SPEC = true, bool TEX = false>
+template <bool SPEC = true, bool TEX = false, int FC = SHADE_ALL>
 PB2_HD bool makeBsdf(const DScene &sc, const DInteraction &it, DBsdf *bsdf, const DUvDiff *uvDiff = nullptr) {
     int m = sc.primMaterial[it.prim];
     if (m < 0) return false;
@@ -450,7 +451,7 @@
         float sig = clampf(mat.sigma, 0.f, 90.f);
         if (!isBlack(kd)) {
             bsdf->R = kd;
-            if (sig == 0)
+            if (!(FC & SHADE_OREN_NAYAR) || sig == 0)
                 bsdf->diffuseKind = 1;
             else {
                 bsdf->diffuseKind = 2;
@@ -468,7 +469,7 @@
             bsdf->nLobes++;
         }
         V3 ks = clampSpectrum(mat.ks);
-        if (!isBlack(ks)) {
+        if ((FC & SHADE_MICROFACET) && !isBlack(ks)) {
             float rough = mat.roughness;
             if (mat.remap_roughness) rough = roughnessToAlpha(rough);
             bsdf->Ks = ks;
@@ -636,8 +637,9 @@
     return .5f * (absCosTheta(wi) * kInvPi + pdf_wh / (4 * dot(wo, wh)));
 }
 
+template <int FC = SHADE_ALL>
 PB2_HD V3 diffuseF(const DBsdf &b, V3 wo, V3 wi) {
-    if (b.diffuseKind == 1) return b.R * kInvPi;
+    if (!(FC & SHADE_OREN_NAYAR) || b.diffuseKind == 1) return b.R * kInvPi;
     float sinThetaI = sinTheta(wi), sinThetaO = sinTheta(wo);
     float maxCos = 0;
     if ((double)sinThetaI > 1e-4 && (double)sinThetaO > 1e-4) {
@@ -754,7 +756,7 @@
     return f;
 }
 
-template <bool SPEC = true>
+template <bool SPEC = true, int FC = SHADE_ALL>
 PB2_HD V3 bsdfF(const DBsdf &b, V3 woW, V3 wiW) {
     V3 wi = worldToLocal(b, wiW), wo = worldToLocal(b, woW);
     if (wo.z == 0) return mk3(0, 0, 0);
@@ -763,12 +765,12 @@
     if (SPEC && b.blend) return reflect ? blendF(b, wo, wi) : f;
     if (SPEC && b.general) return genF(b, wo, wi, reflect);
     if (reflect) {
-        if (b.diffuseKind) f = f + diffuseF(b, wo, wi);
-        if (b.hasMicrofacet) f = f + microfacetF(b, wo, wi);
+        if (b.diffuseKind) f = f + diffuseF<FC>(b, wo, wi);
+        if ((FC & SHADE_MICROFACET) && b.hasMicrofacet) f = f + microfacetF(b, wo, wi);
     }
     return f;
 }
-template <bool SPEC = true>
+template <bool SPEC = true, int FC = SHADE_ALL>
 PB2_HD float bsdfPdf(const DBsdf &b, V3 woW, V3 wiW) {
     if (b.nLobes == 0) return 0.f;
     V3 wo = worldToLocal(b, woW), wi = worldToLocal(b, wiW);
@@ -783,7 +785,7 @@
     }
     float pdf = 0.f;
     if (b.diffuseKind) pdf += diffusePdf(wo, wi);
-    if (b.hasMicrofacet) pdf += microfacetPdf(b, wo, wi);
+    if ((FC & SHADE_MICROFACET) && b.hasMicrofacet) pdf += microfacetPdf(b, wo, wi);
     return pdf / b.nLobes;
 }
 PB2_HD bool refract(V3 wi, V3 n, float eta, V3 *wt) {
@@ -873,7 +875,7 @@
     return f;
 }
 
-template <bool SPEC = true>
+template <bool SPEC = true, int FC = SHADE_ALL>
 PB2_HD V3 bsdfSampleF(const DBsdf &b, V3 woW, V3 *wiW, V2 u, float *pdf, int *sampledFlags = nullptr, bool nonSpecularOnly = false) {
     *pdf = 0;
     if (sampledFlags) *sampledFlags = 0;
@@ -938,7 +940,7 @@
     }
     int comp = (int)floorf(u.x * matching);
     if (comp > matching - 1) comp = matching - 1;
-    bool sampleMicro = b.hasMicrofacet && (comp == matching - 1) && !(b.diffuseKind && comp == 0);
+    bool sampleMicro = (FC & SHADE_MICROFACET) && b.hasMicrofacet && (comp == matching - 1) && !(b.diffuseKind && comp == 0);
     V2 uRemapped = mk2(pmin(u.x * matching - comp, kOneMinusEpsilon), u.y);
     V3 wo = worldToLocal(b, woW), wi;
     if (wo.z == 0) return mk3(0, 0, 0);
@@ -947,7 +949,7 @@
         wi = cosineSampleHemisphere(uRemapped);
         if (wo.z < 0) wi.z *= -1;
         *pdf = diffusePdf(wo, wi);
-        f = diffuseF(b, wo, wi);
+        f = diffuseF<FC>(b, wo, wi);
     } else {
         V3 wh = trSampleWh(b.alpha, wo, uRemapped);
         if (dot(wo, wh) < 0) return mk3(0, 0, 0);
@@ -958,7 +960,7 @@
     }
     if (*pdf == 0) return mk3(0, 0, 0);
     *wiW = localToWorld(b, wi);
-    if (matching > 1) {
+    if ((FC & SHADE_MICROFACET) && matching > 1) {
         if (sampleMicro) *pdf += diffusePdf(wo, wi);
         else *pdf += microfacetPdf(b, wo, wi);
         *pdf /= matching;
@@ -966,8 +968,8 @@
     bool reflect = dot(*wiW, b.ng) * dot(woW, b.ng) > 0;
     f = mk3(0, 0, 0);
     if (reflect) {
-        if (b.diffuseKind) f = f + diffuseF(b, wo, wi);
-        if (b.hasMicrofacet) f = f + microfacetF(b, wo, wi);
+        if (b.diffuseKind) f = f + diffuseF<FC>(b, wo, wi);
+        if ((FC & SHADE_MICROFACET) && b.hasMicrofacet) f = f + microfacetF(b, wo, wi);
     }
     return f;
 }
@@ -1247,10 +1249,11 @@
     return (dl.dist[6 * iv + iu] / dl.dist[12 + 5]) / (2 * kPi * kPi * sinTheta);
 }
 
-template <bool SPH = true>
+template <bool SPH = true, int FC = SHADE_ALL>
 PB2_HD DLightSample sampleLight(const DScene &sc, int lightNum, const pb2_light &l, const TriRec &rec, const DInteraction &ref, V2 u) {
-    if (sc.deltaLights && l.type == PB2_LIGHT_INFINITE) return sampleInfiniteLight(sc, l, sc.deltaLights[lightNum], ref.p, u);
-    if (sc.deltaLights && l.type != PB2_LIGHT_AREA) return sampleDeltaLight(l, sc.deltaLights[lightNum], ref.p);
+    const bool nonArea = (FC & SHADE_NON_AREA) && sc.deltaLights;
+    if (nonArea && l.type == PB2_LIGHT_INFINITE) return sampleInfiniteLight(sc, l, sc.deltaLights[lightNum], ref.p, u);
+    if (nonArea && l.type != PB2_LIGHT_AREA) return sampleDeltaLight(l, sc.deltaLights[lightNum], ref.p);
     DLightSample s;
     if (SPH && (rec.flags & LEAF_SPHERE)) s = sampleSphereLight(sc, l, ref, u);
     else s = sampleTriangleLight(sc, l, rec, ref.p, u);
@@ -1258,9 +1261,9 @@
     return s;
 }
 
-template <bool SPH = true>
+template <bool SPH = true, int FC = SHADE_ALL>
 PB2_HD float lightPdfLi(const DScene &sc, const pb2_light &l, const TriRec &rec, const DInteraction &ref, V3 wi, int lightNum = -1) {
-    if (sc.deltaLights && l.type == PB2_LIGHT_INFINITE) return infinitePdfLi(sc.deltaLights[lightNum], wi);
+    if ((FC & SHADE_NON_AREA) && sc.deltaLights && l.type == PB2_LIGHT_INFINITE) return infinitePdfLi(sc.deltaLights[lightNum], wi);
     if (SPH && (rec.flags & LEAF_SPHERE)) return sphereLightPdf(sc, l, ref, wi);
     DRay ray = spawnRay(ref, wi);
     const TriVerts t = rec.tv;
diff --git a/pbrt_v3_b200/csrc/pb2_cuda.cu b/pbrt_v3_b200/csrc/pb2_cuda.cu
--- a/pbrt_v3_b200/csrc/pb2_cuda.cu
+++ b/pbrt_v3_b200/csrc/pb2_cuda.cu
@@ -348,6 +348,7 @@
     int bvhDepth = 0;
     int instDepth = 0;
     bool hasSpecular = false;
+    int shadeClass = SHADE_ALL;
     int devIndex = 0;
     std::vector<pb2_scene *> replicas;
     bool lazyLightDist = false;
@@ -926,6 +927,8 @@
     return pool;
 }
 
+constexpr int kShadeLambertAreaMinBlocks = 4;
+
 static int renderWavefront(pb2_scene *scene, const DRenderParams &rp, float4 *film, cudaStream_t stream, int flags,
                            bool timeTrace, unsigned long long *launches, double *traceMs) {
     const bool lazyLights = scene->lazyLightDist;
@@ -949,7 +952,12 @@
         chain.film = film;
     }
     const bool spheres = scene->d.spheres != nullptr;
+    const bool sobol = rp.halton.sobol != nullptr;
+    const bool textured = scene->d.nTextures > 0 || sobol;
+    const bool lambertArea = scene->shadeClass == SHADE_LAMBERT_AREA && !scene->hasSpecular && !spheres;
+    const bool narrowShade = lambertArea && !scene->lazyLightDist && !textured;
     AdvanceKernel advLight = spheres ? k_wf_advance<false, true, 7> : k_wf_advance<false, false, 7>;
+    if (lambertArea) advLight = k_wf_advance<false, false, 7, false, false, false, SHADE_LAMBERT_AREA>;
     AdvanceKernel advShade = scene->hasSpecular ? (spheres ? k_wf_advance<true, true, 4, true> : k_wf_advance<true, false, 4, true>)
                              : spheres ? k_wf_advance<true, true, 4>
                                        : k_wf_advance<true, false, 4>;
@@ -957,12 +965,12 @@
         advShade = scene->hasSpecular ? (spheres ? k_wf_advance<true, true, 4, true, true> : k_wf_advance<true, false, 4, true, true>)
                    : spheres ? k_wf_advance<true, true, 4, false, true>
                              : k_wf_advance<true, false, 4, false, true>;
-    const bool sobol = rp.halton.sobol != nullptr;
-    const bool textured = scene->d.nTextures > 0 || sobol;
     if (textured) advShade = k_wf_advance<true, true, 3, true, true, true>;
+    if (narrowShade) advShade = k_wf_advance<true, false, kShadeLambertAreaMinBlocks, false, false, false, SHADE_LAMBERT_AREA>;
     typedef void (*FinishKernel)(const DScene *, const DRenderParams *, WfPool, int, unsigned, float4 *);
     FinishKernel finish = scene->hasSpecular ? (spheres ? k_wf_finish<true, true> : k_wf_finish<false, true>)
                                              : (spheres ? k_wf_finish<true, false> : k_wf_finish<false, false>);
+    if (lambertArea) finish = k_wf_finish<false, false, SHADE_LAMBERT_AREA>;
     static const int finishPerSM = envInt("PB2_FINISH", 256);
     const unsigned finishThreshold = ((flags & PB2_FLAG_COUNT_TRAVERSAL) || lazyLights || textured) ? 0u : (unsigned)(g_numSMs * std::max(0, finishPerSM));
     const int finishBlocks = std::max(1, (int)((finishThreshold + 127) / 128));
@@ -1360,6 +1368,15 @@
         return rc;
     }
     *out = primary;
+    return PB2_OK;
+}
+
+static int shadeFeatureClass(const pb2_scene_desc *d);
+int pb2_shade_class(const pb2_scene_desc *d, int32_t *out) {
+    if (!d || !out) return setError(PB2_ERR_INVALID, "null argument");
+    if (d->n_materials < 0 || (d->n_materials > 0 && !d->materials) || d->n_lights < 0 || (d->n_lights > 0 && !d->lights))
+        return setError(PB2_ERR_INVALID, "bad material or light records");
+    *out = shadeFeatureClass(d);
     return PB2_OK;
 }
 
@@ -1663,6 +1680,25 @@
     return PB2_OK;
 }
 
+static int shadeFeatureClass(const pb2_scene_desc *d) {
+    static const bool forceGeneral = envInt("PB2_SHADE_GENERAL", 0) != 0;
+    if (forceGeneral) return SHADE_ALL;
+    int fc = 0;
+    for (int i = 0; i < d->n_materials; ++i) {
+        const pb2_material &m = d->materials[i];
+        if (m.type == PB2_MAT_NONE) continue;
+        if (m.type == PB2_MAT_MATTE) {
+            if (m.tex[PB2_TEX_SIGMA] || !(m.sigma <= 0.f)) fc |= SHADE_OREN_NAYAR;
+        } else if (m.type == PB2_MAT_PLASTIC)
+            fc |= SHADE_MICROFACET;
+        else
+            return SHADE_ALL;
+    }
+    for (int i = 0; i < d->n_lights; ++i)
+        if (d->lights[i].type != PB2_LIGHT_AREA) fc |= SHADE_NON_AREA;
+    return fc;
+}
+
 static int createSceneOnCurrentDevice(const pb2_scene_desc *d, pb2_scene **out) {
     int rc = PB2_OK;
     if (d->n_prims <= 0 || d->n_nodes <= 0 || !d->nodes || !d->bvh_prims || !d->prim_type || !d->prim_index)
@@ -1699,6 +1735,7 @@
         if (d->materials[i].type == PB2_MAT_MIRROR || d->materials[i].type == PB2_MAT_GLASS || d->materials[i].type == PB2_MAT_SUBSTRATE ||
             d->materials[i].type == PB2_MAT_METAL || d->materials[i].type == PB2_MAT_UBER)
             s->hasSpecular = true;
+    s->shadeClass = shadeFeatureClass(d);
     DScene &sc = s->d;
     memset(&sc, 0, sizeof(sc));
     sc.nNodes = d->n_nodes;
diff --git a/pbrt_v3_b200/csrc/pb2_wavefront.cuh b/pbrt_v3_b200/csrc/pb2_wavefront.cuh
--- a/pbrt_v3_b200/csrc/pb2_wavefront.cuh
+++ b/pbrt_v3_b200/csrc/pb2_wavefront.cuh
@@ -39,8 +39,32 @@
     return lane;
 }
 
+enum { WF_IN_ALL = 0x7f, WF_IN_SHADE = 0x47 };
+static_assert(offsetof(DLane, etaScale) + sizeof(float) <= 96 && offsetof(DLane, smp) + sizeof(DSampler) <= 96 &&
+                  offsetof(DLane, ldSum) == 96 && offsetof(DLane, betaNext) + sizeof(V3) <= 192 && offsetof(WfCtx, hit) == 192 &&
+                  offsetof(WfCtx, pFilm) + sizeof(V2) <= 224,
+              "WF_IN_SHADE: the fields shadeVertex reads on entry lie in sectors 0-2 and 6, the dead ones in sectors 3-5");
+
+template <unsigned SECTORS>
+__device__ __forceinline__ int wfStagedChunk(int kk) {
+    if (SECTORS == WF_IN_ALL) return kk;
+    const int n = kk >> 1;
+    int s = 0, seen = 0;
+#pragma unroll
+    for (int t = 0; t < 7; ++t)
+        if ((SECTORS >> t) & 1u) {
+            s = n == seen ? t : s;
+            ++seen;
+        }
+    return 2 * s + (kk & 1);
+}
+
+template <unsigned SECTORS = WF_IN_ALL>
 __device__ __forceinline__ void wfStageIn(const WfCtx *ctx, WfSlot *warpSlots, int c) {
-    constexpr int CHUNKS = sizeof(WfCtx) / 16, BATCH = CHUNKS / 2;
+    constexpr int NSECT = ((SECTORS >> 0) & 1) + ((SECTORS >> 1) & 1) + ((SECTORS >> 2) & 1) + ((SECTORS >> 3) & 1) +
+                          ((SECTORS >> 4) & 1) + ((SECTORS >> 5) & 1) + ((SECTORS >> 6) & 1);
+    static_assert(SECTORS <= WF_IN_ALL && NSECT > 0, "sectors of a 224-byte context");
+    constexpr int CHUNKS = 2 * NSECT, BATCH = NSECT;
     const int lane = wfLaneId();
     __syncwarp();
 #pragma unroll
@@ -49,13 +73,15 @@
         int cs[BATCH];
 #pragma unroll
         for (int it = 0; it < BATCH; ++it) {
-            const int q = (b * BATCH + it) * 32 + lane, j = q / CHUNKS, k = q % CHUNKS;
+            const int q = (b * BATCH + it) * 32 + lane, j = q / CHUNKS, kk = q % CHUNKS;
+            const int k = wfStagedChunk<SECTORS>(kk);
             cs[it] = __shfl_sync(0xffffffffu, c, j);
             if (cs[it] >= 0) v[it] = __ldcs(reinterpret_cast<const uint4 *>(ctx + cs[it]) + k);
         }
 #pragma unroll
         for (int it = 0; it < BATCH; ++it) {
-            const int q = (b * BATCH + it) * 32 + lane, j = q / CHUNKS, k = q % CHUNKS;
+            const int q = (b * BATCH + it) * 32 + lane, j = q / CHUNKS, kk = q % CHUNKS;
+            const int k = wfStagedChunk<SECTORS>(kk);
             if (cs[it] >= 0) {
                 uint2 *s = reinterpret_cast<uint2 *>(reinterpret_cast<char *>(&warpSlots[j]) + 16 * k);
                 s[0] = make_uint2(v[it].x, v[it].y);
@@ -1065,7 +1091,7 @@
     }
 }
 
-template <bool SHADE, bool SPH, int MINB, bool SPEC = false, bool LAZY = false, bool TEX = false>
+template <bool SHADE, bool SPH, int MINB, bool SPEC = false, bool LAZY = false, bool TEX = false, int FC = SHADE_ALL>
 __global__ void __launch_bounds__(128, MINB) k_wf_advance(const DScene *__restrict__ scp, const DRenderParams *__restrict__ rpp, WfPool pool,
                                                           int srcQ, int traceQ, int freeQ, float4 *film, unsigned long long *counters) {
     __shared__ WfSlot stage[128];
@@ -1085,7 +1111,7 @@
         bool have = i < n;
         int c = have ? srcList[i] : 0;
         bool ended = false, deferred = false;
-        wfStageIn(pool.ctx, warpSlots, have ? c : -1);
+        wfStageIn<SHADE ? WF_IN_SHADE : WF_IN_ALL>(pool.ctx, warpSlots, have ? c : -1);
         if (have) {
             DLane &ln = slot.ln;
             const int foundCode = slot.found;
@@ -1103,8 +1129,8 @@
                 tc.pFilm = slot.pFilm;
                 tc.diffScale = rp.diffScale;
                 shadeVertex<SPH, SPEC, LAZY, true>(sc, rp.halton, rp.path, ln, found, hit, tHit, u, &tc);
-            } else if (SHADE) shadeVertex<SPH, SPEC, LAZY>(sc, rp.halton, rp.path, ln, found, hit, tHit, u);
-            else lightAdvance<SPH>(sc, ln, found, hit, tHit);
+            } else if (SHADE) shadeVertex<SPH, SPEC, LAZY, false, FC>(sc, rp.halton, rp.path, ln, found, hit, tHit, u);
+            else lightAdvance<SPH, FC>(sc, ln, found, hit, tHit);
             if (SHADE && LAZY && ln.state == LS_DEFER) {
                 ln.state = LS_PATH;
                 deferred = true;
@@ -1128,7 +1154,7 @@
     return n > 0 && n <= threshold && (long long)pool.ctr[CTR_WORK] >= rp.nWorkItems;
 }
 
-template <bool SPH, bool SPEC>
+template <bool SPH, bool SPEC, int FC = SHADE_ALL>
 __global__ void __launch_bounds__(128) k_wf_finish(const DScene *__restrict__ scp, const DRenderParams *__restrict__ rpp, WfPool pool, int traceQ,
                                                    unsigned threshold, float4 *film) {
     const DScene &sc = *scp;
@@ -1151,7 +1177,7 @@
             DHit hit;
             float tMax;
             const bool found = traceLane(sc, ln, &tMax, &hit, nullptr);
-            laneAdvance<SPH, SPEC>(sc, rp.halton, rp.path, ln, found, hit, tMax);
+            laneAdvance<SPH, SPEC, false, FC>(sc, rp.halton, rp.path, ln, found, hit, tMax);
             if (ln.state == LS_DEFER) break;
             if (ln.state == LS_SHADOW) shadow++;
             else if (ln.state != LS_IDLE) regular++;
```
